# mmp/pbrt-v1

Hardware: AMD Instinct MI355X
Metric: Mrays/s (primary+secondary: every Scene::Intersect + Scene::IntersectP) (higher is better)
Workload: dtype f32

## Files before the change

### include/pbrt_hip.h

```cpp
#ifndef PBRT_HIP_H
#define PBRT_HIP_H
#include <stdint.h>
#include <stddef.h>
#ifdef __cplusplus
extern "C" {
#endif

#define RT_OK 0
#define RT_EINVAL (-1)
#define RT_EDEVICE (-2)
#define RT_ESTATE (-3)
#define RT_ENOMEM (-4)

typedef struct RtScene RtScene;

enum { RT_MAT_MATTE = 0, RT_MAT_MIRROR = 1, RT_MAT_GLASS = 2, RT_MAT_PLASTIC = 3, RT_MAT_UBER = 4, RT_MAT_SHINYMETAL = 5, RT_MAT_TRANSLUCENT = 6 };
typedef struct RtMaterial {
    int32_t type;
    float kd[3];
    float kt[3];
    float sigma;
    float ior;
    float ks[3];
    float roughness;
// ... 130 lines not shown
typedef struct RtAccelInfo {
    uint32_t n_nodes, n_leaf_refs, max_depth, n_tris;
    float bounds[6];
    double build_seconds;
    int32_t kind;
    int32_t grid_nvoxels[3];
    float grid_width[3], grid_inv_width[3];
} RtAccelInfo;

const char *rt_last_error(void);
int rt_device_count(int *count);

int rt_scene_create(const RtSceneDesc *desc, int device, RtScene **out);
typedef struct RtPrebuiltAccel {
    int32_t kind;
    uint32_t n_nodes, n_leaf_refs, max_depth;
    const uint32_t *nodes;
    const uint32_t *leaf_refs;
    float bounds[6];
    int32_t grid_nvoxels[3]; float grid_width[3], grid_inv_width[3];
} RtPrebuiltAccel;
int rt_scene_create_prebuilt(const RtSceneDesc *desc, int device, const RtPrebuiltAccel *accel, RtScene **out);
int rt_scene_set_density(RtScene *s, const RtDensityRegion *region);
int rt_scene_set_light_transforms(RtScene *s, const float *light_to_world, uint32_t n_lights);
struct RtTexture; struct RtMaterialTextures;
int rt_scene_set_textures(RtScene *s, const struct RtTexture *nodes, uint32_t n_nodes, const struct RtMaterialTextures *mats, uint32_t n_mats);
int rt_scene_destroy(RtScene *s);
int rt_scene_set_stream(RtScene *s, void *hip_stream);
int rt_scene_accel_info(const RtScene *s, RtAccelInfo *info);
int rt_scene_accel_copy(const RtScene *s, uint32_t *nodes, uint32_t *leaf_refs);

typedef struct RtKdTree RtAccel;
int rt_accel_build(const float *tri_verts, uint32_t n_tris, const RtAccelParams *params, RtAccel **out);
int rt_accel_info(const RtAccel *t, RtAccelInfo *info);
int rt_accel_copy(const RtAccel *t, uint32_t *nodes, uint32_t *leaf_refs);
typedef struct RtLeafLayoutInfo { uint64_t n_nodes, n_slots, n_entries; uint32_t stride, pad; } RtLeafLayoutInfo;
int rt_accel_leaf_layout(const RtAccel *t, int runs, int copies, uint32_t *tnodes, uint32_t *slot_prim, uint32_t *entries, RtLeafLayoutInfo *info);
int rt_accel_destroy(RtAccel *t);
typedef struct RtKdTree RtKdTree;
int rt_kdtree_build(const float *tri_verts, uint32_t n_tris, const RtAccelParams *params, RtKdTree **out);
int rt_kdtree_info(const RtKdTree *t, RtAccelInfo *info);
int rt_kdtree_copy(const RtKdTree *t, uint32_t *nodes, uint32_t *leaf_refs);
int rt_kdtree_destroy(RtKdTree *t);

int rt_camera_rays(RtScene *s, const RtRenderDesc *rd, uint64_t first, uint32_t count, RtRay *rays_out);
int rt_trace_closest(RtScene *s, const RtRay *rays, uint32_t n, RtHit *hits_out);
int rt_trace_any(RtScene *s, const RtRay *rays, uint32_t n, uint8_t *occluded_out);

int rt_trace_closest_device(RtScene *s, const RtRay *dev_rays, uint32_t n, RtHit *dev_hits);
int rt_trace_any_device(RtScene *s, const RtRay *dev_rays, uint32_t n, uint8_t *dev_occluded);
typedef struct RtHitGeometry {
    float   *p;
    float   *ng;
    float   *ns;
    float   *uv;
    int32_t *material;
    int32_t *light;
} RtHitGeometry;
int rt_hit_geometry_device(RtScene *s, const RtRay *dev_rays, const RtHit *dev_hits, uint32_t n, const RtHitGeometry *out);
int rt_camera_rays_device(RtScene *s, const RtRenderDesc *rd, uint64_t first, uint32_t count, RtRay *dev_rays);
int rt_scene_get_stream(RtScene *s, void **hip_stream_out);

int rt_film_bind(RtScene *s, void *device_accum, int32_t x_pixel_count, int32_t y_pixel_count);
int rt_film_clear(RtScene *s);
int rt_film_read(RtScene *s, float *host_accum);
int rt_film_resolve(RtScene *s, int premultiply_alpha, float *rgb_out, float *alpha_out);

int rt_render(RtScene *s, const RtRenderDesc *rd);
int rt_sync(RtScene *s);
int rt_samples_read(RtScene *s, uint64_t first, uint64_t count, float *out);
int rt_counters(RtScene *s, RtCounters *out);
int rt_counters_reset(RtScene *s);
int rt_set_counting(RtScene *s, int enabled);
int rt_last_render_ms(RtScene *s, float *total_ms, float *kernel_ms);
typedef struct RtRenderStats {
    float total_ms, render_ms, trace_ms, gather_ms;
    int32_t pipeline, iterations, timed_iterations;
    uint32_t slots;
    float shade_ms;
    int32_t bands;
    float march_ms;
    uint64_t weighted_points;
    float weighted_ms[5];
} RtRenderStats;
int rt_film_resolve_device(RtScene *s, const float *dev_accum, uint64_t n, int premultiply, float *dev_rgb, float *dev_alpha);
int rt_film_resolve_device_rgba(RtScene *s, const float *dev_accum, uint64_t n, int premultiply, float *dev_rgba);
int rt_film_pack_parts(RtScene *s, const float *dev_accum, int32_t w, int32_t h, int32_t world, int32_t rows, float *dev_parts);
int rt_last_render_stats(RtScene *s, RtRenderStats *out);

#ifdef __cplusplus
}
#endif
#endif
```

### pbrt-v1_amd/__init__.py

```python
from __future__ import annotations

import ctypes as C
import os
import subprocess
import numpy as np

_HERE = os.path.dirname(os.path.abspath(__file__))
LIB_DIR = os.path.join(_HERE, "lib")
HIP_LIB = os.path.join(LIB_DIR, "libpbrt_hip.so")
if os.environ.get("PBRT_HIP_TUNE") and os.environ.get("PBRT_HIP_LIB_PATH"):
    HIP_LIB = os.environ["PBRT_HIP_LIB_PATH"]
HOST_LIB = os.path.join(LIB_DIR, "libpbrt_host.so")
CSRC = os.path.join(_HERE, "csrc")

HIPCC_FLAGS = ["--offload-arch=gfx950", "-O3", "-std=c++17", "-ffp-contract=off", "-fno-slp-vectorize", "-fPIC", "-shared",
               "-Wno-unused-value"]
HOST_FLAGS = ["-O2", "-std=c++17", "-fPIC", "-shared", "-msse2", "-mfpmath=sse", "-fvisibility=hidden", "-fvisibility-inlines-hidden"]


HIP_UNITS = ("rt_kernels.hip", "rt_scene.hip", "rt_film.hip", "rt_trace.hip", "rt_mega_w.hip", "rt_mega_d.hip", "rt_mega_dw.hip", "rt_mega_p.hip", "rt_mega_b.hip", "rt_mega_g.hip", "rt_pipe_w.hip", "rt_pipe_d.hip",
             "rt_pipe_p.hip", "rt_pipe_v.hip", "rt_march.hip", "rt_rays.hip", "kd_build.cpp", "grid_build.cpp", "leaf_layout.cpp")


def _include_closure(path, seen=None):
    import re
    seen = set() if seen is None else seen
    if path in seen or not os.path.exists(path):
        return seen
    seen.add(path)
    for inc in re.findall(r'^\s*#\s*include\s+"([^"]+)"', open(path).read(), re.M):
        _include_closure(os.path.normpath(os.path.join(os.path.dirname(path), inc)), seen)
    return seen


def _compile_unit(cmd, verbose=False):
    if verbose:
        print(" ".join(cmd))
    if not cmd[-3].endswith(".hip"):
        subprocess.check_call(cmd)
        return
    r = subprocess.run(cmd + ["-Rpass-analysis=kernel-resource-usage"], capture_output=True, text=True)
    keep = [ln for ln in r.stderr.splitlines() if "remark:" in ln and any(k in ln for k in ("Function Name", " VGPRs:", "VGPRs Spill", "Occupancy", "ScratchSize", "LDS Size"))]
    open(cmd[-1][:-2] + ".resources.txt", "w").write("\n".join(keep) + "\n")
    if r.returncode != 0:
        raise RuntimeError("hipcc failed:\n" + r.stderr[-4000:])


def build(force: bool = False, verbose: bool = False, defines=(), jobs: int | None = None) -> None:
    from concurrent.futures import ThreadPoolExecutor
    os.makedirs(LIB_DIR, exist_ok=True)
    obj_dir = os.path.join(LIB_DIR, "obj")
    os.makedirs(obj_dir, exist_ok=True)
    hip_dir = os.path.join(CSRC, "hip")
    hip_dep = [os.path.join(hip_dir, f) for f in os.listdir(hip_dir)] + [os.path.join(_HERE, "..", "include", "pbrt_hip.h")]
    headers = [d for d in hip_dep if d.endswith((".h", ".inc"))]
    host_src = [os.path.join(CSRC, "host", "scene_api.cpp")]
    host_dep = [os.path.join(CSRC, "host", f) for f in os.listdir(os.path.join(CSRC, "host"))] + \
               [os.path.join(_HERE, "..", "include", f) for f in ("pbrt_hip.h", "pbrt_hip_desc.h", "pbrt_hip_plugin.h", "pbrt_hip_material.h", "pbrt_hip_texture.h")]

    def stale(out, deps):
        return force or not os.path.exists(out) or any(os.path.getmtime(d) > os.path.getmtime(out) for d in deps)

    stamp = os.path.join(obj_dir, "defines.txt")
    dtext = " ".join(HIPCC_FLAGS) + " | " + " ".join(HOST_FLAGS) + " | " + " ".join(defines)
    if (open(stamp).read() if os.path.exists(stamp) else "") != dtext:
        force = True
    todo = []
    for u in HIP_UNITS:
        obj = os.path.join(obj_dir, u.rsplit(".", 1)[0] + ".o")
        if stale(obj, sorted(_include_closure(os.path.join(hip_dir, u)))):
            todo.append(["hipcc"] + [f for f in HIPCC_FLAGS if f != "-shared"] + list(defines) + ["-c", os.path.join(hip_dir, u), "-o", obj])
    if todo:
        run = lambda cmd: _compile_unit(cmd, verbose)
        with ThreadPoolExecutor(max_workers=jobs or min(len(todo), os.cpu_count() or 4)) as ex:
            list(ex.map(run, todo))
        open(stamp, "w").write(dtext)
    objs = [os.path.join(obj_dir, u.rsplit(".", 1)[0] + ".o") for u in HIP_UNITS]
    if stale(HIP_LIB, objs):
        cmd = ["hipcc", "--offload-arch=gfx950", "-shared", "-fPIC"] + objs + ["-o", HIP_LIB]
        if verbose:
            print(" ".join(cmd))
        subprocess.check_call(cmd)
    if stale(HOST_LIB, host_dep):
        cmd = ["g++"] + HOST_FLAGS + host_src + ["-Wl,--version-script=" + os.path.join(CSRC, "host", "exports.map"), "-ldl", "-o", HOST_LIB]
        if verbose:
            print(" ".join(cmd))
        subprocess.check_call(cmd)


def build_variant(name: str, defines=(), units=None, arch: str | None = None, verbose: bool = False) -> str:
    from concurrent.futures import ThreadPoolExecutor
    units = list(HIP_UNITS if units is None else units)
    if len(units) < len(HIP_UNITS):
        build()
    obj_dir = os.path.join(LIB_DIR, "obj_" + name)
    os.makedirs(obj_dir, exist_ok=True)
    hip_dir = os.path.join(CSRC, "hip")
    flags = [f for f in HIPCC_FLAGS if f != "-shared"]
    if arch:
        flags = ["--offload-arch=" + arch if f.startswith("--offload-arch=") else f for f in flags]
    out = os.path.join(LIB_DIR, "libpbrt_hip_%s.so" % name)
    stamp = os.path.join(obj_dir, "defines.txt")
    dtext = " ".join(flags) + " | " + " ".join(defines) + " | " + " ".join(units)
    lib_ok = os.path.exists(out) and (open(stamp).read() if os.path.exists(stamp) else "") == dtext
    obj_of = lambda d, u: os.path.join(d, u.rsplit(".", 1)[0] + ".o")

    def stale(u):
        obj = obj_of(obj_dir, u)
        if not lib_ok:
            return True
        t = os.path.getmtime(obj if os.path.exists(obj) else out)
        return any(os.path.getmtime(d) > t for d in _include_closure(os.path.join(hip_dir, u)))
    todo = [u for u in units if stale(u)]
    borrowed = [obj_of(os.path.join(LIB_DIR, "obj"), u) for u in HIP_UNITS if u not in units]
    if not todo and lib_ok and not any(os.path.getmtime(o) > os.path.getmtime(out) for o in borrowed):
        return out
    todo += [u for u in units if u not in todo and not os.path.exists(obj_of(obj_dir, u))]
    cmds = [["hipcc"] + flags + list(defines) + ["-c", os.path.join(hip_dir, u), "-o", obj_of(obj_dir, u)] for u in todo]
    if cmds:
        with ThreadPoolExecutor(max_workers=min(len(cmds), os.cpu_count() or 4)) as ex:
            list(ex.map(lambda cmd: _compile_unit(cmd, verbose), cmds))
    objs = [obj_of(obj_dir if u in units else os.path.join(LIB_DIR, "obj"), u) for u in HIP_UNITS]
    subprocess.check_call(["hipcc", "--offload-arch=" + (arch or "gfx950"), "-shared", "-fPIC"] + objs + ["-o", out])
    open(stamp, "w").write(dtext)
    return out


class RtCounters(C.Structure):
    _fields_ = [(n, C.c_uint64) for n in ("camera_rays", "closest_rays", "any_rays", "nodes_visited", "leaf_refs",
                                          "tri_tests", "bad_samples", "stack_overflows")]

    def as_dict(self):
        return {n: int(getattr(self, n)) for n, _ in self._fields_}


class RtAccelInfo(C.Structure):
    _fields_ = [("n_nodes", C.c_uint32), ("n_leaf_refs", C.c_uint32), ("max_depth", C.c_uint32), ("n_tris", C.c_uint32),
                ("bounds", C.c_float * 6), ("build_seconds", C.c_double), ("kind", C.c_int32),
                ("grid_nvoxels", C.c_int32 * 3), ("grid_width", C.c_float * 3), ("grid_inv_width", C.c_float * 3)]


class RtLeafLayoutInfo(C.Structure):
    _fields_ = [("n_nodes", C.c_uint64), ("n_slots", C.c_uint64), ("n_entries", C.c_uint64), ("stride", C.c_uint32), ("pad", C.c_uint32)]


class RtPrebuiltAccel(C.Structure):
    _fields_ = [("kind", C.c_int32), ("n_nodes", C.c_uint32), ("n_leaf_refs", C.c_uint32), ("max_depth", C.c_uint32),
                ("nodes", C.c_void_p), ("leaf_refs", C.c_void_p), ("bounds", C.c_float * 6),
                ("grid_nvoxels", C.c_int32 * 3), ("grid_width", C.c_float * 3), ("grid_inv_width", C.c_float * 3)]


class RtRenderStats(C.Structure):
    _fields_ = [("total_ms", C.c_float), ("render_ms", C.c_float), ("trace_ms", C.c_float), ("gather_ms", C.c_float),
                ("pipeline", C.c_int32), ("iterations", C.c_int32), ("timed_iterations", C.c_int32), ("slots", C.c_uint32), ("shade_ms", C.c_float), ("bands", C.c_int32), ("march_ms", C.c_float),
                ("weighted_points", C.c_uint64), ("weighted_ms", C.c_float * 5)]

    def as_dict(self):
        return {n: (list(getattr(self, n)) if n == "weighted_ms" else getattr(self, n)) for n, _ in self._fields_}


class RtVolume(C.Structure):
    _fields_ = [("present", C.c_int32), ("world_to_volume", C.c_float * 16), ("p0", C.c_float * 3), ("p1", C.c_float * 3),
                ("sigma_a", C.c_float * 3), ("sigma_s", C.c_float * 3), ("le", C.c_float * 3), ("g", C.c_float)]


class RtDensityRegion(C.Structure):
    _fields_ = [("kind", C.c_int32), ("a", C.c_float), ("b", C.c_float), ("updir", C.c_float * 3),
                ("nx", C.c_int32), ("ny", C.c_int32), ("nz", C.c_int32), ("density", C.POINTER(C.c_float))]


RT_MATERIAL_NAMES = ("matte", "mirror", "glass", "plastic", "uber", "shinymetal", "translucent")


class RtMaterial(C.Structure):
    _fields_ = [("type", C.c_int32), ("kd", C.c_float * 3), ("kt", C.c_float * 3), ("sigma", C.c_float), ("ior", C.c_float),
                ("ks", C.c_float * 3), ("roughness", C.c_float), ("kr", C.c_float * 3)]


class RtMaterialLobes(C.Structure):
    _fields_ = [(n, C.c_float * 3) for n in ("eta_ks", "eta_kr", "r_kd", "t_kd", "r_ks", "t_ks")] + \
               [(n, C.c_int32) for n in ("has_dr", "has_dt", "has_gr", "has_gt")]


class RtMaterialParams(C.Structure):
    _fields_ = [("type", C.c_int32), ("c", (C.c_float * 3) * 4), ("f", C.c_float)]


class RtMaterialTextures(C.Structure):
    _fields_ = [("raw", RtMaterialParams), ("tex", C.c_int32 * 5)]


class RtMaterialResolved(C.Structure):
    _fields_ = [("type", C.c_int32), ("r", C.c_float * 3), ("t", C.c_float * 3), ("on_a", C.c_float), ("on_b", C.c_float), ("ior", C.c_float),
                ("has_r", C.c_int32), ("has_t", C.c_int32), ("ks", C.c_float * 3), ("exponent", C.c_float), ("kr", C.c_float * 3),
                ("has_g", C.c_int32), ("has_kr", C.c_int32)]


class RtTexture(C.Structure):
    _fields_ = [("kind", C.c_int32), ("is_color", C.c_int32), ("mapping", C.c_int32), ("child", C.c_int32 * 3), ("value", C.c_float * 12),
                ("map", C.c_float * 8), ("world_to_texture", C.c_float * 16)]


RT_TEXTURE_NAMES = ("constant", "scale", "mix", "bilerp", "uv", "checkerboard")
RT_TEXMAP_NAMES = ("uv", "spherical", "cylindrical", "planar")
RT_MATERIAL_SLOTS = {"matte": ("Kd", None, None, None, "sigma"), "mirror": ("Kr", None, None, None, None), "glass": ("Kr", "Kt", None, None, "index"),
                     "plastic": ("Kd", "Ks", None, None, "roughness"), "uber": ("Kd", "Ks", "Kr", "opacity", "roughness"),
                     "shinymetal": (None, "Ks", "Kr", None, "roughness"), "translucent": ("Kd", "Ks", "reflect", "transmit", "roughness")}

RT_DENSITY_NAMES = {1: "exponential", 2: "volumegrid"}

RT_LIGHT_NAMES = ("point", "area", "spot", "distant", "infinite")

RT_INTEGRATOR_DEBUG = 0x100
RT_DEBUG_NAMES = ("u", "v", "nx", "ny", "nz", "snx", "sny", "snz", "one", "zero", "hit")
(RT_DEBUG_U, RT_DEBUG_V, RT_DEBUG_NX, RT_DEBUG_NY, RT_DEBUG_NZ, RT_DEBUG_SNX, RT_DEBUG_SNY, RT_DEBUG_SNZ,
 RT_DEBUG_ONE, RT_DEBUG_ZERO, RT_DEBUG_HIT) = range(11)


class RtLight(C.Structure):
    _fields_ = [("type", C.c_int32), ("color", C.c_float * 3), ("pos", C.c_float * 3), ("n_samples", C.c_int32), ("first_tri", C.c_uint32),
                ("n_tris", C.c_uint32), ("reverse_orientation", C.c_int32), ("flip_normal", C.c_int32), ("dir", C.c_float * 3),
                ("world_to_light", C.c_float * 9), ("cos_total_width", C.c_float), ("cos_falloff_start", C.c_float), ("quadric_plus1", C.c_int32)]

class RtRenderDesc(C.Structure):
    _fields_ = [(n, C.c_int32) for n in ("integrator", "max_depth", "strategy", "volume_integrator")] + [("step_size", C.c_float)] + \
               [(n, C.c_int32) for n in ("sampler", "x_samples", "y_samples", "jitter", "pixel_samples")] + [("seed", C.c_uint32)] + \
               [(n, C.c_int32) for n in ("x_res", "y_res", "x_pixel_start", "y_pixel_start", "x_pixel_count", "y_pixel_count", "x_start", "x_end", "y_start", "y_end")] + \
               [("filter_x_width", C.c_float), ("filter_y_width", C.c_float), ("filter_table", C.c_float * 256)] + \
               [(n, C.c_int32) for n in ("shard_index", "shard_count", "tile_pixels")]


class RtHitGeometry(C.Structure):
    _fields_ = [(n, C.c_void_p) for n in ("p", "ng", "ns", "uv", "material", "light")]


HIT_FIELDS = ("p", "ng", "ns", "uv", "material", "light")
_HIT_FIELD_SHAPE = {"p": (3, False), "ng": (3, False), "ns": (3, False), "uv": (2, False), "material": (0, True), "light": (0, True)}

# ... 796 lines not shown
```

### pbrt-v1_amd/csrc/hip/rt_host.h

```cpp
#pragma once
#include "rt_flavour.h"
#include "rt_render_kernel.h"
#include "rt_pipeline.h"
#include "rt_pipe_vertex.h"
#include "rt_pipe_march.h"
#include "rt_bidir.h"
#include "rt_internal.h"
#include "rt_devbuf.h"
#include <cstdio>
#include <cstdlib>
#include <cstring>
#include <string>
#include <vector>
#include <cmath>
#include <chrono>
#include <atomic>
#include <thread>
#include <type_traits>

namespace rt {
const char *knob(const char *name);
int fail(int code, const std::string &msg);
const char *last_error();
void hip_warn(hipError_t e, const char *what);
}
using namespace rt;
#define HIPCHK(expr)                                                                                   \
    do {                                                                                               \
        hipError_t e_ = (expr);                                                                        \
        if (e_ != hipSuccess)                                                                          \
            return rt::fail(RT_EDEVICE, std::string(#expr) + ": " + hipGetErrorString(e_));            \
    } while (0)
#define HIPWARN(expr) rt::hip_warn((expr), #expr)

namespace rt {
extern const flavour::Table<RenderKernelFn, flavour::Mega> g_render_kernels_whitted, g_render_kernels_direct, g_render_kernels_path;
extern const flavour::Table<RenderKernelFn, flavour::Weighted> g_render_kernels_weighted;
extern const flavour::Table<RenderKernelFn, flavour::Bidir> g_render_kernels_bidir;
extern const flavour::Table<RenderKernelFn, flavour::Debug> g_render_kernels_debug;
extern const flavour::Table<PipeShadeFn, flavour::Shade> g_pipe_shade_whitted, g_pipe_shade_direct, g_pipe_shade_path;
extern const flavour::Table<PipeShadeFn, flavour::Vertex> g_pipe_vertex;
extern const flavour::Table<PipeTraceFn, flavour::Trace> g_pipe_trace;
extern const flavour::Table<PipeMarchFn, flavour::March> g_pipe_march;
}
static const flavour::Table<RenderKernelFn, flavour::Mega> *const g_render_kernels[RT_INTEGRATOR_PATH + 1] = {&g_render_kernels_whitted, &g_render_kernels_direct, &g_render_kernels_path};
static const flavour::Table<PipeShadeFn, flavour::Shade> *const g_pipe_shade[RT_INTEGRATOR_PATH + 1] = {&g_pipe_shade_whitted, &g_pipe_shade_direct, &g_pipe_shade_path};
struct ResidentGrids {
    flavour::Table<unsigned, flavour::Mega> mega[RT_INTEGRATOR_PATH + 1];
    flavour::Table<unsigned, flavour::Weighted> weighted;
    flavour::Table<unsigned, flavour::Bidir> bidir;
    flavour::Table<unsigned, flavour::Debug> debug;
    flavour::Table<unsigned, flavour::Trace> trace;
    flavour::Table<unsigned, flavour::March> march;
};

namespace rt { void host_free(void *p); void event_free(void *e); void stream_free(void *st); }
template <class T> using Pinned = rt::DevBuf<T, rt::host_free>;
using Event = rt::DevBuf<std::remove_pointer_t<hipEvent_t>, rt::event_free>;
using OwnedStream = rt::DevBuf<std::remove_pointer_t<hipStream_t>, rt::stream_free>;

struct PipePlanes {
    DevBuf<float4> state, ray_o, hit, q_o; DevBuf<unsigned> q_slot;
    template <class F> void each(F &&f) { f(state, size_t(RT_PIPE_VEC)); f(ray_o, size_t(2)); f(hit, size_t(3)); f(q_o, size_t(4)); f(q_slot, size_t(3)); }
};

struct RtScene {
    int device = 0;
    hipStream_t stream = nullptr;
    OwnedStream own_stream;
    Event ev0, ev1, ev2;
    Event wt_ev[6];
    std::vector<Event> pipe_ev;
    std::vector<Event> pipe_fence;
    KdTree tree;
    GridAccelData gridacc;
    int accel_kind = RT_ACCEL_KDTREE;
    double per_leaf = -1.0;
    bool has_ext = false;
    DevScene dev{};
    std::vector<DevBuf<char>> allocs;
    float *accum = nullptr; DevBuf<float> own_accum; int film_w = 0, film_h = 0;
    DevBuf<float> filter_dev;
    DevBuf<unsigned long long> work_counter, counters;
    DevBuf<uint2> spill;
    DevBuf<float> frames;
    unsigned grid = 0, n_threads = 0;
    ResidentGrids grids{};
    DevBuf<DimReq> light_dims;
    std::vector<DimReq> light_dims_host;
    const unsigned *light_draw_flags = nullptr; unsigned n_drawing_lights = 0;
    DevBuf<unsigned> wt_recbase;
    unsigned n_infinite = 0;
    int light_draws = 0;
    DevBuf<unsigned> wt_base; DevBuf<float> wt_rec; DevBuf<float2> wt_pick;
    DevBuf<unsigned long long> wt_sums;
    Pinned<unsigned long long> wt_total;
    unsigned long long wt_points = 0; bool last_weighted = false;
    DevBuf<DevScene> dev_scene; DevBuf<DevFrame> dev_frame;
    DevBuf<float4> samples;
    int samples_spp = 1;
    unsigned long long samples_last = 0;
    DevBuf<float> resolve_buf;
    DevBuf<float> vol_buf;
    RtVolume volume{};
    int density_kind = RT_DENSITY_NONE;
    double vol_world[6] = {0, 0, 0, 0, 0, 0};
    bool rendered = false;
    std::vector<DevMaterial> materials_host;
    std::vector<DevLight> lights_host;
    std::vector<int> tex_uv_idx_host; std::vector<float> tex_uv_host;
    bool has_textures = false;
    DevBuf<DevMaterial> mat_buf;
    int spill_depth = 0;
    bool have_timing = false;
    bool counting = true;
    uint32_t n_tris = 0;
    PipePlanes pool; DevBuf<unsigned> q_count; DevBuf<unsigned long long> wave_work; DevBuf<PipePool> dev_pool;
    Pinned<unsigned> h_qcount;
    bool last_pipeline = false, last_marches = false; int pipe_iters = 0, pipe_timed = 0; unsigned pipe_slots = 0;
    DevBuf<float4> trace_buf;
    int n_cus = 0;
    DevBuf<unsigned> trace_qc;
    DevBuf<float4> ray_planes, any_hits;
};
#define RT_PIPE_QN 4096
#define RT_PIPE_TIMED 256
#define RT_PIPE_BATCH 4

static inline int scene_alloc(RtScene *s, size_t bytes, void **p) {
    DevBuf<char> b;
    if (int rc = b.grow(bytes)) return rc;
    *p = b.p; s->allocs.push_back(std::move(b));
    return RT_OK;
}
template <class T>
static inline int upload(RtScene *s, const T *host, size_t n, const T **dev) {
    void *p = nullptr;
    if (int rc = scene_alloc(s, (n ? n : 1) * sizeof(T), &p)) return rc;
    if (n) HIPCHK(hipMemcpy(p, host, n * sizeof(T), hipMemcpyHostToDevice));
    *dev = static_cast<const T *>(p);
    return RT_OK;
}

int upload_tex_uv(RtScene *s);
int ensure_material_pool(RtScene *s, rt::DevFrame &fr, size_t levels, size_t n_slots);

template <class T>
static inline int ensure(RtScene *s, DevBuf<T> &b, size_t need) {
    if (need <= b.cap) return RT_OK;
    if (b.p) HIPCHK(hipStreamSynchronize(s->stream));
    return b.grow(need);
}

template <class F> static inline int guarded(const char *what, F &&f) {
    try { return f(); }
    catch (const std::bad_alloc &) { return rt::fail(RT_ENOMEM, std::string(what) + ": out of host memory"); }
    catch (const std::exception &e) { return rt::fail(RT_ESTATE, std::string(what) + ": " + e.what()); }
}

struct FilmGather { int which = 0, grx = 0, gry = 0, cols = 0, rows = 0, slot_ncs = 0; size_t slot_lds = 0, col_bytes = 0; };
int film_gather_plan(RtScene *s, const rt::DevFrame &fr, FilmGather &g);
int film_gather_launch(RtScene *s, const rt::DevFrame &fr, const FilmGather &g, const rt::DevFrame *dfr, int row0, int row_end);
```

### pbrt-v1_amd/csrc/hip/rt_integrate.h

```cpp
#pragma once
#include "rt_shade.h"
#include "rt_texture.h"

namespace rt {

enum Stage {
    ST_FETCH = 0, ST_VERTEX, ST_DIRECT_NEXT, ST_SHADOW_DONE, ST_MIS_DONE, ST_ED_BSDF, ST_ED_DONE,
    ST_BOUNCE, ST_SPECULAR, ST_SPEC_TRANS, ST_RETURN, ST_VOL_BEGIN, ST_VOL_STEP, ST_POP, ST_FINISH, ST_EXIT
};

struct Rng {
    uint32_t base, ctr;
    RT_DEV float next_float() { return rng_f32(base, ctr++); }
    RT_DEV uint32_t next_u32() { return rng_u32(base, ctr++); }
};

#define RT_FRAME_WORDS 25

struct Lane {
    uint32_t sample_index;
    uint32_t work;
    float image_x, image_y;
    uint32_t dim_base;
    Rng rng;
    V3 L;
    V3 thr;
    float alpha;
    int depth;
    int fsp;
    bool specular;
    Vertex v;
    int li, lj;
    int cur_light;
    V3 Ld;
    V3 Ld_light;
    V3 L_all;
    V3 pend;
    float bs1, bs2, bcs;
    uint32_t ord;
    uint32_t ctr0;
    float wt_w;
    unsigned vf;
    V3 dM, dB;
    V3 pendS, pendM, thr_old;
    int stage;
    bool has_ray;
    Trav tv;
};

RT_DEV float lhs_value(const Lane &ln, const DimReq &r, int j, int d) {
    const uint32_t fb = ln.dim_base + r.f_base, ub = ln.dim_base + r.u_base;
    if (r.n == 1) return (0 + rng_f32(ln.rng.base, fb + d)) * 1.f;
    int pos = j;
    const int n = r.n;
    for (int k = n - 1; k >= 0; --k) {
        int other = int(rng_u32(ln.rng.base, ub + d * n + k) % uint32_t(n));
        if (pos == k) pos = other; else if (pos == other) pos = k;
    }
    float delta = 1.f / n;
    return (pos + rng_f32(ln.rng.base, fb + pos * r.dims + d)) * delta;
}

RT_DEV float van_der_corput(uint32_t n, uint32_t scramble) {
    n = (n << 16) | (n >> 16);
    n = ((n & 0x00ff00ffu) << 8) | ((n & 0xff00ff00u) >> 8);
    n = ((n & 0x0f0f0f0fu) << 4) | ((n & 0xf0f0f0f0u) >> 4);
    n = ((n & 0x33333333u) << 2) | ((n & 0xccccccccu) >> 2);
    n = ((n & 0x55555555u) << 1) | ((n & 0xaaaaaaaau) >> 1);
    n ^= scramble;
    return (float)n / (float)0x100000000LL;
}
RT_DEV float sobol2(uint32_t n, uint32_t scramble) {
    for (uint32_t v = 1u << 31; n != 0; n >>= 1, v ^= v >> 1)
        if (n & 0x1) scramble ^= v;
    return (float)scramble / (float)0x100000000LL;
}
RT_DEV int shuffle_origin(uint32_t base, uint32_t off, int count, int pos) {
    for (int k = count - 1; k >= 0; --k) {
        const int other = int(rng_u32(base, off + k) % uint32_t(count));
        if (pos == k) pos = other; else if (pos == other) pos = k;
    }
    return pos;
}
RT_DEV uint32_t pixel_stream(const DevFrame &fr, const Lane &ln) {
    const uint32_t n0 = ln.sample_index - (ln.work % uint32_t(fr.spp));
    if (n0 == 0 && fr.sampler != RT_SAMPLER_LOWDISCREPANCY) return rng_base(0xFFFFFFFFu, fr.seed);
    return rng_base(n0, fr.seed);
}
RT_DEV float dim_value(const DevFrame &fr, const Lane &ln, const DimReq &r, int j, int d) {
    if (fr.sampler == RT_SAMPLER_STRATIFIED) return lhs_value(ln, r, j, d);
    if (fr.sampler == RT_SAMPLER_RANDOM) return rng_f32(ln.rng.base, ln.dim_base + r.f_base + j * r.dims + d);
    const uint32_t pb = pixel_stream(fr, ln);
    const int P = fr.spp, n = r.n, s = int(ln.work % uint32_t(P));
    const uint32_t nscr = r.dims;
    const int blk = shuffle_origin(pb, r.f_base + nscr + uint32_t(n) * P, P, s);
    const int jb = (n == 1) ? 0 : shuffle_origin(pb, r.f_base + nscr + uint32_t(blk) * n, n, j);
    const uint32_t idx = uint32_t(blk) * n + jb;
    if (r.dims == 1) return van_der_corput(idx, rng_u32(pb, r.f_base));
    return d == 0 ? van_der_corput(idx, rng_u32(pb, r.f_base)) : sobol2(idx, rng_u32(pb, r.f_base + 1));
}

#ifndef RT_SAMPLE_NT
#define RT_SAMPLE_NT 1
#endif
RT_DEV void sample_write(const DevFrame &fr, const Lane &ln, V3 Ls, float alpha, unsigned &bad) {
    const float y = lum_y(Ls);
    if (Ls.x != Ls.x || Ls.y != Ls.y || Ls.z != Ls.z) { Ls = mk3(0.f); ++bad; }
    else if (y < -1e-5) { Ls = mk3(0.f); ++bad; }
    else if (isinf(y)) { Ls = mk3(0.f); ++bad; }
    const uint32_t lp = fastdiv(ln.work, fr.div.spp);
    float4 RT_G *rec = RT_GPTR(float4, fr.samples) + sample_slot(lp, ln.work - lp * uint32_t(fr.spp), fr.spp);
#if RT_SAMPLE_NT
    typedef float nt_f4 __attribute__((ext_vector_type(4)));
    const nt_f4 r0 = {Ls.x, Ls.y, Ls.z, alpha}, r1 = {ln.image_x, ln.image_y, 0.f, 0.f};
    __builtin_nontemporal_store(r0, (nt_f4 RT_G *)rec);
    __builtin_nontemporal_store(r1, (nt_f4 RT_G *)(rec + RT_SAMPLE_XY));
#else
    rec[0] = make_float4(Ls.x, Ls.y, Ls.z, alpha);
    rec[RT_SAMPLE_XY] = make_float4(ln.image_x, ln.image_y, 0.f, 0.f);
#endif
}

RT_DEV void stratified_camera_sample(const DevFrame &fr, uint32_t pixel_index, int s, int px, int py,
                                     uint32_t pix_base, float &ix, float &iy, float &lu, float &lv, bool need_lens) {
    const int n = fr.spp;
    const int sy = int(fastdiv(unsigned(s), fr.div.xs)), sx = s - sy * fr.xs;
    const float dx = 1.f / fr.xs, dy = 1.f / fr.ys;
    float jx = 0.5f, jy = 0.5f;
    if (fr.jitter) { jx = rng_f32(pix_base, 2 * s); jy = rng_f32(pix_base, 2 * s + 1); }
    ix = (sx + jx) * dx; iy = (sy + jy) * dy;
    ix += px; iy += py;
    lu = lv = 0.5f;
    if (need_lens) {
        const uint32_t ub = fr.jitter ? 5u * n : 0u;
        int pos = s;
        for (int k = n - 1; k >= 0; --k) {
            int other = int(rng_u32(pix_base, ub + k) % uint32_t(n));
            if (pos == k) pos = other; else if (pos == other) pos = k;
        }
        const int lx = pos % fr.xs, ly = pos / fr.xs;
        float kx = 0.5f, ky = 0.5f;
        if (fr.jitter) { kx = rng_f32(pix_base, 2 * n + 2 * pos); ky = rng_f32(pix_base, 2 * n + 2 * pos + 1); }
        lu = (lx + kx) * dx; lv = (ly + ky) * dy;
    }
    (void)pixel_index;
}

RT_DEV Ray camera_ray(const RtCamera &cam, float ix, float iy, float lensU, float lensV) {
    Ray r;
    if (cam.type == RT_CAMERA_ENVIRONMENT) {
        r.o = xform_point(cam.camera_to_world, mk3(0.f, 0.f, 0.f));
        const float theta = RT_PI * iy / cam.y_res;
        const float phi = 2 * RT_PI * ix / cam.x_res;
        const V3 dir = mk3(rt_sinf(theta) * rt_cosf(phi), rt_cosf(theta), rt_sinf(theta) * rt_sinf(phi));
        r.d = xform_vector(cam.camera_to_world, dir);
        r.mint = cam.hither; r.maxt = cam.yon;
        return r;
    }
    V3 Pcamera = xform_point(cam.raster_to_camera, mk3(ix, iy, 0.f));
    r.o = Pcamera;
    r.d = cam.type == RT_CAMERA_ORTHOGRAPHIC ? mk3(0.f, 0.f, 1.f) : Pcamera;
    if (cam.lens_radius > 0.f) {
        float lu, lv; concentric_disk(lensU, lensV, lu, lv);
        lu *= cam.lens_radius; lv *= cam.lens_radius;
        float ft = (cam.focal_distance - cam.hither) / r.d.z;
        V3 Pfocus = r.o + r.d * ft;
        r.o.x += lu * (cam.focal_distance - cam.hither) / cam.focal_distance;
        r.o.y += lv * (cam.focal_distance - cam.hither) / cam.focal_distance;
        r.d = Pfocus - r.o;
    }
    r.d = normalize3(r.d);
    r.mint = 0.f;
    r.maxt = cam.type == RT_CAMERA_ORTHOGRAPHIC ? cam.yon - cam.hither : (cam.yon - cam.hither) / r.d.z;
    r.o = xform_point(cam.camera_to_world, r.o);
    r.d = xform_vector(cam.camera_to_world, r.d);
    return r;
}

RT_DEV bool work_to_sample(const DevFrame &fr, unsigned long long w, unsigned long long &pixel, int &s) {
    const unsigned long long per_tile = (unsigned long long)fr.tile_pixels * fr.spp;
    if (fr.tile_w > 0) {
        const unsigned w32 = unsigned(w), pt = unsigned(per_tile);
        const unsigned lt = fastdiv(w32, fr.div.per_tile), rem = w32 - lt * pt;
        const unsigned tile = lt * unsigned(fr.shard_count) + unsigned(fr.shard_index);
        const unsigned q = fastdiv(rem, fr.div.spp);
        s = int(rem - q * unsigned(fr.spp));
        const unsigned ty = fastdiv(tile, fr.div.tiles_x), tx = tile - ty * unsigned(fr.tiles_x);
        const unsigned qy = fastdiv(q, fr.div.tile_w), qx = q - qy * unsigned(fr.tile_w);
        const unsigned px = tx * unsigned(fr.tile_w) + qx, py = ty * unsigned(fr.tile_h) + qy;
        const unsigned ew = unsigned(fr.x_end - fr.x_start), eh = unsigned(fr.y_end - fr.y_start);
        pixel = (unsigned long long)py * ew + px;
        return px < ew && py < eh;
    }
    if (fr.total_work <= 0xffffffffull && per_tile <= 0xffffffffull) {
        const unsigned w32 = unsigned(w), pt = unsigned(per_tile);
        const unsigned lt = fastdiv(w32, fr.div.per_tile), rem = w32 - lt * pt;
        const unsigned long long tile = (unsigned long long)lt * unsigned(fr.shard_count) + unsigned(fr.shard_index);
        const unsigned q = fastdiv(rem, fr.div.spp);
        pixel = tile * unsigned(fr.tile_pixels) + q;
        s = int(rem - q * unsigned(fr.spp));
        return pixel < fr.total_pixels;
    }
    const unsigned long long lt = w / per_tile, rem = w % per_tile;
    const unsigned long long tile = lt * fr.shard_count + fr.shard_index;
    pixel = tile * fr.tile_pixels + rem / fr.spp;
    s = int(rem % fr.spp);
    return pixel < fr.total_pixels;
}

RT_DEV void tile_order_to_sample(const DevFrame &fr, unsigned w, unsigned &pixel, int &s) {
    const unsigned spp = unsigned(fr.spp), T = unsigned(fr.mega_tile);
    const unsigned W = unsigned(fr.x_end - fr.x_start), H = unsigned(fr.y_end - fr.y_start);
    const FrameDiv &dv = fr.div;
    const unsigned wp = fastdiv(w, dv.spp); s = int(w - wp * spp);
    const unsigned row_px = W * T, ty = fastdiv(wp, dv.row_px), rem = wp - ty * row_px;
    const unsigned h_t = min(T, H - ty * T), full = T * h_t, tiles_x = dv.blocks_x;
    const FastDiv &df = h_t < T ? dv.block[1] : dv.block[0];
    unsigned tx = fastdiv(rem, df); tx = tx < tiles_x ? tx : tiles_x - 1u;
    const unsigned rem2 = rem - tx * full, w_t = min(T, W - tx * T);
    const FastDiv &dw = w_t < T ? dv.block_w[1] : dv.block_w[0];
    const unsigned qy = fastdiv(rem2, dw), qx = rem2 - qy * w_t;
    pixel = (ty * T + qy) * W + tx * T + qx;
}

RT_DEV void setup_sample(const DevScene &sc, const DevFrame &fr, Lane &ln, unsigned long long pixel, int s, Ray &ray) {
    const int w = fr.x_end - fr.x_start;
    int px, py;
    if (fr.total_pixels <= 0xffffffffull) { const unsigned row = fastdiv(unsigned(pixel), fr.div.width); px = fr.x_start + int(unsigned(pixel) - row * unsigned(w)); py = fr.y_start + int(row); }
    else { px = fr.x_start + int(pixel % w); py = fr.y_start + int(pixel / w); }
    const uint32_t n0 = uint32_t(pixel * fr.spp);
    ln.sample_index = n0 + uint32_t(s);
    ln.rng.base = rng_base(ln.sample_index, fr.seed);
    float lu = 0.5f, lv = 0.5f;
    const bool need_lens = sc.cam.lens_radius > 0.f;
    if (fr.sampler == RT_SAMPLER_STRATIFIED) {
        const uint32_t pix_base = (pixel == 0) ? rng_base(0xFFFFFFFFu, fr.seed) : rng_base(n0, fr.seed);
        ln.dim_base = (s == 0 && pixel != 0) ? fr.pixgen_draws : 0u;
        stratified_camera_sample(fr, uint32_t(pixel), s, px, py, pix_base, ln.image_x, ln.image_y, lu, lv, need_lens);
    } else if (fr.sampler == RT_SAMPLER_RANDOM) {
        const uint32_t pix_base = (pixel == 0) ? rng_base(0xFFFFFFFFu, fr.seed) : rng_base(n0, fr.seed);
        ln.dim_base = (s == 0 && pixel != 0) ? fr.pixgen_draws : 0u;
        ln.image_x = rng_f32(pix_base, 2 * s); ln.image_y = rng_f32(pix_base, 2 * s + 1);
        ln.image_x += px; ln.image_y += py;
        if (need_lens) { lu = rng_f32(pix_base, 2 * fr.spp + 2 * s); lv = rng_f32(pix_base, 2 * fr.spp + 2 * s + 1); }
    } else {
        const uint32_t pix_base = rng_base(n0, fr.seed);
        const uint32_t P = uint32_t(fr.spp);
        ln.dim_base = (s == 0) ? fr.pixgen_draws : 0u;
        const int pos = shuffle_origin(pix_base, 2 + P, int(P), s);
        ln.image_x = px + van_der_corput(uint32_t(pos), rng_u32(pix_base, 0));
        ln.image_y = py + sobol2(uint32_t(pos), rng_u32(pix_base, 1));
        if (need_lens) {
            const uint32_t lb = 2 + 2 * P;
            const int lp = shuffle_origin(pix_base, lb + 2 + P, int(P), s);
            lu = van_der_corput(uint32_t(lp), rng_u32(pix_base, lb)); lv = sobol2(uint32_t(lp), rng_u32(pix_base, lb + 1));
        }
    }
    ln.rng.ctr = ln.dim_base + ((fr.sampler == RT_SAMPLER_LOWDISCREPANCY) ? 0u : fr.lhs_total);
    ray = camera_ray(sc.cam, ln.image_x, ln.image_y, lu, lv);
    ln.image_x = (ln.image_x + 1.f) - 1.f; ln.image_y = (ln.image_y + 1.f) - 1.f;
}

RT_DEV float RT_G *frame_ptr(const DevFrame &fr, int frame, unsigned gtid) {
    return RT_GPTR(float, fr.frames) + (size_t(frame) * RT_FRAME_WORDS) * fr.n_threads + gtid;
}
template <bool EXT>
RT_DEV void frame_push(const DevFrame &fr, Lane &ln, unsigned gtid, V3 f, float absdot, int after) {
    float RT_G *q = frame_ptr(fr, ln.fsp, gtid); const size_t st = fr.n_threads;
    q[0 * st] = ln.L.x; q[1 * st] = ln.L.y; q[2 * st] = ln.L.z;
    q[3 * st] = f.x; q[4 * st] = f.y; q[5 * st] = f.z; q[6 * st] = absdot;
    q[7 * st] = __int_as_float(after); q[8 * st] = __int_as_float(ln.depth);
    q[9 * st] = ln.v.p.x; q[10 * st] = ln.v.p.y; q[11 * st] = ln.v.p.z;
    q[12 * st] = ln.v.nn.x; q[13 * st] = ln.v.nn.y; q[14 * st] = ln.v.nn.z;
    q[15 * st] = ln.v.sn.x; q[16 * st] = ln.v.sn.y; q[17 * st] = ln.v.sn.z;
    q[18 * st] = ln.v.wo.x; q[19 * st] = ln.v.wo.y; q[20 * st] = ln.v.wo.z;
    q[21 * st] = __int_as_float(ln.v.mat);
    if (EXT) { q[22 * st] = ln.v.ng.x; q[23 * st] = ln.v.ng.y; q[24 * st] = ln.v.ng.z; }
    ++ln.fsp;
}
template <bool EXT>
RT_DEV int frame_pop(const DevFrame &fr, Lane &ln, unsigned gtid, V3 child) {
    --ln.fsp;
    const float RT_G *q = frame_ptr(fr, ln.fsp, gtid); const size_t st = fr.n_threads;
    V3 Lp = mk3(q[0 * st], q[1 * st], q[2 * st]);
    V3 f = mk3(q[3 * st], q[4 * st], q[5 * st]);
    float absdot = q[6 * st];
    ln.L = Lp + (child * f) * absdot;
    int after = __float_as_int(q[7 * st]);
    ln.depth = __float_as_int(q[8 * st]);
    ln.v.p = mk3(q[9 * st], q[10 * st], q[11 * st]);
    ln.v.nn = mk3(q[12 * st], q[13 * st], q[14 * st]);
    ln.v.sn = mk3(q[15 * st], q[16 * st], q[17 * st]);
    ln.v.tn = cross3(ln.v.nn, ln.v.sn);
    ln.v.wo = mk3(q[18 * st], q[19 * st], q[20 * st]);
    ln.v.mat = __float_as_int(q[21 * st]);
    if (EXT) ln.v.ng = mk3(q[22 * st], q[23 * st], q[24 * st]);
    return after;
}

RT_DEV void all_lights_done(Lane &ln) {
    ln.L = ln.L + ln.L_all;
    ln.stage = ST_SPECULAR;
}

template <bool DEFER = false>
RT_DEV void launch_ray(Lane &ln, const DevScene &sc, V3 o, V3 d, float mint, float maxt, bool any, int next_stage) {
    Ray r; r.o = o; r.d = d; r.mint = mint; r.maxt = maxt;
    if (DEFER) { ln.tv.o = o; ln.tv.d = d; ln.tv.mint = mint; ln.tv.maxt = maxt; ln.tv.any = any; ln.tv.hit_prim = -1; ln.tv.b1 = 0.f; ln.tv.b2 = 0.f; }
    else if (sc.accel_kind == RT_ACCEL_GRID) grid_begin(ln.tv, sc, r, any); else trav_begin(ln.tv, sc, r, any);
    ln.has_ray = true;
    ln.stage = next_stage;
}

RT_DEV float RT_G *vol_ray_ptr(const DevFrame &fr, int level, unsigned gtid) { return RT_GPTR(float, fr.vol_rays) + size_t(level) * 8 * fr.n_threads + gtid; }
RT_DEV void vol_store_ray(const DevFrame &fr, int level, unsigned gtid, const Ray &r) {
    float RT_G *q = vol_ray_ptr(fr, level, gtid); const size_t st = fr.n_threads;
    q[0] = r.o.x; q[st] = r.o.y; q[2 * st] = r.o.z; q[3 * st] = r.d.x; q[4 * st] = r.d.y; q[5 * st] = r.d.z; q[6 * st] = r.mint; q[7 * st] = r.maxt;
}
RT_DEV Ray vol_load_ray(const DevFrame &fr, int level, unsigned gtid) {
    const float RT_G *q = vol_ray_ptr(fr, level, gtid); const size_t st = fr.n_threads;
    Ray r; r.o = mk3(q[0], q[st], q[2 * st]); r.d = mk3(q[3 * st], q[4 * st], q[5 * st]); r.mint = q[6 * st]; r.maxt = q[7 * st];
    return r;
}
RT_DEV bool vol_intersect(const RtVolume &v, V3 o, V3 d, float mint, float maxt, float &t0, float &t1) {
    const V3 vo = xform_point(v.world_to_volume, o), vd = xform_vector(v.world_to_volume, d);
    float a = mint, b = maxt; bool ok = true;
#pragma unroll
    for (int i = 0; i < 3; ++i) {
        float invRayDir = 1.f / comp(vd, i);
        float tNear = (v.p0[i] - comp(vo, i)) * invRayDir, tFar = (v.p1[i] - comp(vo, i)) * invRayDir;
        if (tNear > tFar) { float tmp = tNear; tNear = tFar; tFar = tmp; }
        a = tNear > a ? tNear : a; b = tFar < b ? tFar : b;
        if (a > b) ok = false;
    }
    t0 = a; t1 = b; return ok;
}
RT_DEV bool vol_inside(const RtVolume &v, V3 p) {
    const V3 q = xform_point(v.world_to_volume, p);
    return q.x >= v.p0[0] && q.x <= v.p1[0] && q.y >= v.p0[1] && q.y <= v.p1[1] && q.z >= v.p0[2] && q.z <= v.p1[2];
}
RT_DEV V3 vol_transmittance(const RtVolume &v, V3 o, V3 d, float mint, float maxt) {
    float t0, t1;
// ... 194 lines not shown
            const V3 ss = dens ? D * mat_color(vol.sigma_s) : (in ? mat_color(vol.sigma_s) : mk3(0.f));
            const int nLights = int(sc.n_lights);
            if (!is_black(ss) && nLights > 0) {
                const float r0 = have_row ? m.s0 : samp[size_t(3 * i) * st], u1 = have_row ? m.s1 : samp[size_t(3 * i + 1) * st], u2 = have_row ? m.s2 : samp[size_t(3 * i + 2) * st];
                const int lightNum = min(int(floorf(r0 * nLights)), nLights - 1);
                LightRef Lt = RT_LIGHT(sc, lightNum);
                V3 wo, L, sd; float pdf, smax;
                if (light_is_delta<EXT>(Lt)) { L = delta_light_sample(Lt, p, wo, sd, smax); pdf = 1.f; }
                else if constexpr (EXT) {
                    if (light_is_infinite<EXT>(Lt)) { wo = infinite_sample_sphere(u1, u2, pdf); L = mat_color(Lt.color); sd = wo; smax = RT_INF; }
                    else {
                        V3 ns; V3 ps = area_sample_point<EXT>(sc, Lt, p, u1, u2, ln.rng, ns);
                        wo = normalize3(ps - p); pdf = area_light_pdf<EXT>(sc, Lt, p, wo); L = area_L(Lt, ns, -wo);
                        sd = ps - p; smax = 1.f - RT_RAY_EPSILON;
                    }
                } else {
                    V3 ns; V3 ps = area_sample_point<EXT>(sc, Lt, p, u1, u2, ln.rng, ns);
                    wo = normalize3(ps - p); pdf = area_light_pdf<EXT>(sc, Lt, p, wo); L = area_L(Lt, ns, -wo);
                    sd = ps - p; smax = 1.f - RT_RAY_EPSILON;
                }
                if (!is_black(L) && pdf > 0.f) {
                    const float costheta = dot3(w, -wo);
                    const float phase = in ? 1.f / (4.f * RT_PI) * (1.f - vol.g * vol.g) / rt_powf(1.f + vol.g * vol.g - 2.f * vol.g * costheta, 1.5f) : 0.f;
                    ln.pend = div_s((((Tr * ss) * phase) * L) * float(nLights), pdf);
                    m.i = i; m.t0 = t0; m.Tr = Tr; m.p = p; m.Lv = Lv;
                    if (PREFETCH) {
                        const int j = i + 1 < N ? i + 1 : i;
                        m.s0 = samp[size_t(3 * j) * st]; m.s1 = samp[size_t(3 * j + 1) * st]; m.s2 = samp[size_t(3 * j + 2) * st];
                    }
                    launch_ray<DEFER>(ln, sc, p, sd, RT_RAY_EPSILON, smax, true, ST_VOL_STEP);
                    return true;
                }
            }
        }
        ++i; t0 += step; have_row = false;
    }
    Lv = Lv * step;
    if (EXT && sc.dens_kind != RT_DENSITY_NONE) ln.L = ln.L + Lv;
    else {
        const V3 T = vol_transmittance(vol, ray.o, ray.d, ray.mint, ray.maxt);
        ln.L = T * ln.L + Lv;
    }
    ln.stage = ST_POP;
    return false;
}

RT_DEV float debug_value(int code, bool hit, float u, float v, V3 ng, V3 ns) {
    switch (code) {
        case RT_DEBUG_U: return u;
        case RT_DEBUG_V: return v;
        case RT_DEBUG_NX: return fabsf(ng.x);
        case RT_DEBUG_NY: return fabsf(ng.y);
        case RT_DEBUG_NZ: return fabsf(ng.z);
        case RT_DEBUG_SNX: return fabsf(ns.x);
        case RT_DEBUG_SNY: return fabsf(ns.y);
        case RT_DEBUG_SNZ: return fabsf(ns.z);
        case RT_DEBUG_ONE: return 1.f;
        case RT_DEBUG_HIT: return hit ? 1.f : 0.f;
        default: return 0.f;
    }
}
template <bool COUNT, bool VOL>
RT_DEV void debug_vertex(const DevScene &sc, const DevFrame &fr, Lane &ln, unsigned gtid, unsigned *c_closest) {
    if (COUNT) ++*c_closest;
    const bool hit = ln.tv.hit_prim >= 0;
    const int cr = fr.strategy & 0xff, cg = (fr.strategy >> 8) & 0xff, cb = (fr.strategy >> 16) & 0xff;
    const bool want_uv = cr <= RT_DEBUG_V || cg <= RT_DEBUG_V || cb <= RT_DEBUG_V;
    const bool want_n = (cr >= RT_DEBUG_NX && cr <= RT_DEBUG_SNZ) || (cg >= RT_DEBUG_NX && cg <= RT_DEBUG_SNZ) || (cb >= RT_DEBUG_NX && cb <= RT_DEBUG_SNZ);
    float u = 0.f, v = 0.f; V3 ng = mk3(0.f), ns = mk3(0.f);
    if (hit) {
        if (want_uv) {
            RtTexHit h;
            hit_point_uv(sc, ln.tv, __float_as_uint(RT_GPTR(const float4, sc.tri_shade)[size_t(2) * unsigned(ln.tv.hit_prim)].w), h);
            u = h.u; v = h.v;
        }
        if (want_n) { make_vertex<true>(sc, ln.tv, ln.v); ng = ln.v.ng; ns = ln.v.nn; }
        if (VOL) vol_ray_ptr(fr, 0, gtid)[7 * size_t(fr.n_threads)] = ln.tv.maxt;
    }
    ln.L = mk3(debug_value(cr, hit, u, v, ng, ns), debug_value(cg, hit, u, v, ng, ns), debug_value(cb, hit, u, v, ng, ns));
    ln.alpha = 1.f;
    ln.stage = ST_RETURN;
}

template <bool COUNT, int INTEG_, bool VOL, bool EXT, int STAGE, bool DEFER = false, bool PARK = false>
RT_DEV void stage_body(const DevScene &sc, const DevFrame &fr, Lane &ln, unsigned gtid,
                       unsigned *c_closest, unsigned *c_any, unsigned *c_bad) {
    constexpr bool WEIGHTED = INTEG_ == RT_INTEG_DIRECT_WEIGHTED;
    constexpr int INTEG = WEIGHTED ? int(RT_INTEGRATOR_DIRECT) : INTEG_;
    if constexpr (STAGE == ST_VERTEX && INTEG_ == RT_INTEGRATOR_DEBUG) {
        debug_vertex<COUNT, VOL>(sc, fr, ln, gtid, c_closest);
        return;
    } else if constexpr (STAGE == ST_VERTEX) {
        if (COUNT) ++*c_closest;
        const bool hit = ln.tv.hit_prim >= 0;
        if (INTEG == RT_INTEGRATOR_PATH) {
            if (!hit) {
                if (EXT && ln.depth == 0) ln.L = infinite_le_sum(sc, ln.L, mk3(1.f), false);
                if (ln.depth == 0) ln.alpha = (ln.L.x != 0.f || ln.L.y != 0.f || ln.L.z != 0.f) ? 1.f : 0.f;
                else if (EXT && ln.specular) ln.L = infinite_le_sum(sc, ln.L, ln.thr, true);
                ln.stage = ST_RETURN; return;
            }
            int resolved = -1;
            if constexpr (EXT) resolved = resolve_hit_material(sc, fr, ln.tv, 0, gtid);
            make_vertex<EXT>(sc, ln.tv, ln.v);
            if (EXT && resolved >= 0) ln.v.mat = resolved;
#ifdef RT_DEBUG_PIXEL
            if (int(floorf(ln.image_x)) == fr.dbg_x && int(floorf(ln.image_y)) == fr.dbg_y)
                printf("DEV depth %d prim %d t %.9g o %.9g %.9g %.9g d %.9g %.9g %.9g p %.9g %.9g %.9g nn %.9g %.9g %.9g sn %.9g %.9g %.9g\n", ln.depth, ln.tv.hit_prim, ln.tv.maxt,
                       ln.tv.o.x, ln.tv.o.y, ln.tv.o.z, ln.tv.d.x, ln.tv.d.y, ln.tv.d.z, ln.v.p.x, ln.v.p.y, ln.v.p.z, ln.v.nn.x, ln.v.nn.y, ln.v.nn.z, ln.v.sn.x, ln.v.sn.y, ln.v.sn.z);
#endif
            if (ln.depth == 0) { ln.alpha = 1.f; if (VOL) vol_ray_ptr(fr, 0, gtid)[7 * size_t(fr.n_threads)] = ln.tv.maxt; }
            else if (VOL) ln.thr = ln.thr * scene_transmittance<VOL, EXT>(sc, fr, ln, ln.tv.o, ln.tv.d, ln.tv.mint, ln.tv.maxt);
            if ((ln.depth == 0 || ln.specular) && ln.v.light >= 0)
                ln.L = ln.L + ln.thr * area_L(RT_LIGHT(sc, ln.v.light), vertex_ng<EXT>(ln.v), ln.v.wo);
        } else {
            if (!hit) {
                ln.L = mk3(0.f);
                if (ln.depth == 0) ln.alpha = 0.f;
                if (EXT) {
                    ln.L = infinite_le_sum(sc, ln.L, mk3(1.f), false);
                    if (ln.depth == 0 && !is_black(ln.L)) ln.alpha = 1.f;
                }
                ln.stage = ST_RETURN; return;
            }
            int resolved = -1;
            if constexpr (EXT) resolved = resolve_hit_material(sc, fr, ln.tv, ln.fsp, gtid);
            make_vertex<EXT>(sc, ln.tv, ln.v);
            if (EXT && resolved >= 0) ln.v.mat = resolved;
            if (ln.depth == 0) ln.alpha = 1.f;
            if (VOL) vol_ray_ptr(fr, ln.fsp, gtid)[7 * size_t(fr.n_threads)] = ln.tv.maxt;
            ln.L = mk3(0.f);
            if (ln.v.light >= 0) ln.L = ln.L + area_L(RT_LIGHT(sc, ln.v.light), vertex_ng<EXT>(ln.v), ln.v.wo);
        }
        ln.li = 0; ln.lj = 0; ln.L_all = mk3(0.f); ln.Ld_light = mk3(0.f);
        ln.stage = ST_DIRECT_NEXT;
        return;
    }
    if constexpr (STAGE == ST_DIRECT_NEXT) {
        const int nLights = int(sc.n_lights);
        if constexpr (WEIGHTED) {
            if (nLights == 0) { ln.stage = ST_SPECULAR; return; }
            if (fr.weighted_phase == 1) { ++ln.ord; ln.stage = ST_SPECULAR; return; }
            if (fr.weighted_phase == 3 && ln.li > 0) { ln.stage = ST_SPECULAR; return; }
            if (fr.weighted_phase == 2 && fr.wt_mixed) {
                if (ln.li == 0 && ln.lj == 0) { ln.ctr0 = ln.rng.ctr; ln.wt_w = __uint_as_float(1u); }
                if (ln.li >= nLights) { ++ln.ord; ln.rng.ctr = ln.ctr0; ln.lj = 0; ln.stage = ST_SPECULAR; return; }
                ln.rng.ctr = ln.ctr0 + uint32_t(ln.lj);
            } else if (fr.weighted_phase == 2) {
                if (ln.li == 0) ln.ctr0 = ln.rng.ctr;
                if (ln.li >= nLights) { ++ln.ord; ln.stage = ST_SPECULAR; return; }
                ln.rng.ctr = ln.ctr0;
            }
            const float ls1 = dim_value(fr, ln, fr.two_d[0], 0, 0), ls2 = dim_value(fr, ln, fr.two_d[0], 0, 1);
            ln.bs1 = dim_value(fr, ln, fr.two_d[1], 0, 0); ln.bs2 = dim_value(fr, ln, fr.two_d[1], 0, 1);
            ln.bcs = dim_value(fr, ln, fr.one_d[1], 0, 0);
            if (fr.weighted_phase == 2) {
                if (ln.li == 0 && ln.lj == 0) RT_GPTR(float, fr.wt_rec)[weighted_record(fr, ln, nLights)] = dim_value(fr, ln, fr.one_d[0], 0, 0);
                estimate_direct_begin<EXT, DEFER>(sc, ln, ln.li, ls1, ls2);
            } else {
                const float2 pick = RT_GPTR(const float2, fr.wt_pick)[ln.ord++];
                ln.li = 1; ln.wt_w = pick.y;
                estimate_direct_begin<EXT, DEFER>(sc, ln, __float_as_int(pick.x), ls1, ls2);
            }
            return;
        }
        if (INTEG == RT_INTEGRATOR_PATH || (INTEG == RT_INTEGRATOR_DIRECT && fr.strategy == RT_STRATEGY_ONE)) {
            if (nLights == 0 || ln.li > 0) { ln.stage = (INTEG == RT_INTEGRATOR_PATH) ? ST_BOUNCE : ST_SPECULAR; return; }
            ln.li = 1;
            const int k = (INTEG == RT_INTEGRATOR_PATH) ? ln.depth : 0;
            const bool from_sampler = (INTEG == RT_INTEGRATOR_DIRECT) || k < 3;
            float un, ls1, ls2;
            if (from_sampler) {
                const int i1 = (INTEG == RT_INTEGRATOR_PATH) ? 3 * k : 0;
                const int i2 = (INTEG == RT_INTEGRATOR_PATH) ? 3 * k : 0;
                un = dim_value(fr, ln, fr.one_d[i1], 0, 0);
                ls1 = dim_value(fr, ln, fr.two_d[i2], 0, 0); ls2 = dim_value(fr, ln, fr.two_d[i2], 0, 1);
                ln.bs1 = dim_value(fr, ln, fr.two_d[i2 + 1], 0, 0); ln.bs2 = dim_value(fr, ln, fr.two_d[i2 + 1], 0, 1);
                ln.bcs = dim_value(fr, ln, fr.one_d[i1 + 1], 0, 0);
            } else {
                un = ln.rng.next_float();
                ls1 = ln.rng.next_float(); ls2 = ln.rng.next_float();
                ln.bs1 = ln.rng.next_float(); ln.bs2 = ln.rng.next_float(); ln.bcs = ln.rng.next_float();
            }
            int lightNum = min(int(floorf(un * nLights)), nLights - 1);
            estimate_direct_begin<EXT, DEFER>(sc, ln, lightNum, ls1, ls2);
            return;
        }
        if (INTEG == RT_INTEGRATOR_DIRECT) {
            if (ln.li >= nLights) { all_lights_done(ln); return; }
            const DimReq RT_G *ld = RT_GPTR(const DimReq, fr.light_dims) + 3 * ln.li;
            const DimReq rl = ld[0], rb = ld[1], rc = ld[2];
            if (ln.lj == 0) ln.Ld_light = mk3(0.f);
            const float ls1 = dim_value(fr, ln, rl, ln.lj, 0), ls2 = dim_value(fr, ln, rl, ln.lj, 1);
            ln.bs1 = dim_value(fr, ln, rb, ln.lj, 0); ln.bs2 = dim_value(fr, ln, rb, ln.lj, 1);
            ln.bcs = dim_value(fr, ln, rc, ln.lj, 0);
            estimate_direct_begin<EXT, DEFER>(sc, ln, ln.li, ls1, ls2);
            return;
        }
        if (ln.li >= nLights) { ln.stage = ST_SPECULAR; return; }
        {
            LightRef Lt = RT_LIGHT(sc, ln.li);
            MatRef m = RT_MAT(sc, ln.v.mat);
            const int cur = ln.li++;
            V3 wi, Li, sd; float smax;
            if (light_is_delta<EXT>(Lt)) Li = delta_light_sample(Lt, ln.v.p, wi, sd, smax);
            else if constexpr (EXT) {
                if (light_is_infinite<EXT>(Lt)) {
                    float u2 = ln.rng.next_float();
                    float u1 = ln.rng.next_float();
                    float pdf; wi = infinite_sample_sphere(u1, u2, pdf);
                    Li = (pdf == 0.f) ? mk3(0.f) : div_s(mat_color(Lt.color), pdf);
                    sd = wi; smax = RT_INF;
                } else {
                    float u2 = ln.rng.next_float();
                    float u1 = ln.rng.next_float();
                    V3 ns; V3 ps = area_sample_point<EXT>(sc, Lt, ln.v.p, u1, u2, ln.rng, ns);
                    wi = normalize3(ps - ln.v.p);
                    float pdf = area_light_pdf<EXT>(sc, Lt, ln.v.p, wi);
                    Li = (pdf == 0.f) ? mk3(0.f) : div_s(area_L(Lt, ns, -wi), pdf);
                    sd = ps - ln.v.p; smax = 1.f - RT_RAY_EPSILON;
                }
            } else {
                float u2 = ln.rng.next_float();
                float u1 = ln.rng.next_float();
                V3 ns; V3 ps = area_sample_point<EXT>(sc, Lt, ln.v.p, u1, u2, ln.rng, ns);
                wi = normalize3(ps - ln.v.p);
                float pdf = area_light_pdf<EXT>(sc, Lt, ln.v.p, wi);
                Li = (pdf == 0.f) ? mk3(0.f) : div_s(area_L(Lt, ns, -wi), pdf);
                sd = ps - ln.v.p; smax = 1.f - RT_RAY_EPSILON;
            }
            (void)cur;
            if (is_black(Li)) return;
            V3 f = bsdf_f<EXT>(m, ln.v, ln.v.wo, wi);
            if (is_black(f)) return;
            ln.pend = (f * Li) * absdot3(wi, ln.v.nn);
            launch_ray<DEFER>(ln, sc, ln.v.p, sd, RT_RAY_EPSILON, smax, true, ST_SHADOW_DONE);
        }
        return;
    }
    if constexpr (STAGE == ST_SHADOW_DONE) {
        if (COUNT) ++*c_any;
        const bool occluded = ln.tv.hit_prim >= 0;
        if (INTEG == RT_INTEGRATOR_WHITTED) {
            if (!occluded) ln.L = ln.L + ln.pend * scene_transmittance<VOL, EXT>(sc, fr, ln, ln.tv.o, ln.tv.d, ln.tv.mint, ln.tv.maxt);
            ln.stage = ST_DIRECT_NEXT;
            return;
        }
        if (!occluded) ln.Ld = ln.Ld + ln.pend * scene_transmittance<VOL, EXT>(sc, fr, ln, ln.tv.o, ln.tv.d, ln.tv.mint, ln.tv.maxt);
        ln.stage = ST_ED_BSDF;
        return;
    }
    if constexpr (STAGE == ST_ED_BSDF) {
        estimate_direct_bsdf<EXT, DEFER>(sc, ln);
        return;
    }
    if constexpr (STAGE == ST_MIS_DONE) {
        if (COUNT) ++*c_closest;
        if (ln.tv.hit_prim >= 0) {
            V3 nh; int light;
            prim_normal_light<EXT>(sc, ln.tv, nh, light);
            if (light == ln.cur_light) {
                if (dot3(nh, -ln.tv.d) > 0)
                    ln.Ld = ln.Ld + ln.pend * scene_transmittance<VOL, EXT>(sc, fr, ln, ln.tv.o, ln.tv.d, ln.tv.mint, ln.tv.maxt);
            }
        } else if (EXT) {
            LightRef Lt = RT_LIGHT(sc, ln.cur_light);
            if (Lt.type == RT_LIGHT_INFINITE && !is_black(mat_color(Lt.color)))
                ln.Ld = ln.Ld + ln.pend * scene_transmittance<VOL, EXT>(sc, fr, ln, ln.tv.o, ln.tv.d, ln.tv.mint, ln.tv.maxt);
        }
        ln.stage = ST_ED_DONE;
        return;
    }
    if constexpr (STAGE == ST_ED_DONE) {
        const int nLights = int(sc.n_lights);
        if constexpr (WEIGHTED) {
            if (fr.weighted_phase == 2) {
                const unsigned at = fr.wt_mixed ? __float_as_uint(ln.wt_w) : 1u + 2u * unsigned(ln.li);
                float RT_G *rec = RT_GPTR(float, fr.wt_rec) + weighted_record(fr, ln, nLights) + at;
                rec[0] = lum_y(ln.Ld);
                rec[1] = lum_y(ln.Ld * float(nLights));
                if (fr.wt_mixed) {
                    ln.wt_w = __uint_as_float(at + 2u);
                    const unsigned j = ln.ord - RT_GPTR(const unsigned, fr.wt_base)[ln.work];
                    if (light_draws_rng(RT_LIGHT(sc, ln.li)) && unsigned(ln.lj) < j) ++ln.lj; else { ln.lj = 0; ++ln.li; }
                } else ++ln.li;
                ln.stage = ST_DIRECT_NEXT;
            } else {
                if (ln.wt_w == 0.f) ln.L = ln.L + ln.Ld * float(nLights);
                else ln.L = ln.L + div_s(ln.Ld, ln.wt_w);
                ln.stage = ST_SPECULAR;
            }
            return;
        }
        if (INTEG == RT_INTEGRATOR_PATH) {
            ln.L = ln.L + ln.thr * (ln.Ld * float(nLights));
            ln.stage = ST_BOUNCE;
        } else if (fr.strategy == RT_STRATEGY_ONE) {
            ln.L = ln.L + ln.Ld * float(nLights);
            ln.stage = ST_SPECULAR;
        } else {
            ln.Ld_light = ln.Ld_light + ln.Ld;
            const int ns = RT_GPTR(const DimReq, fr.light_dims)[3 * ln.li].n;
            if (++ln.lj >= ns) {
                ln.L_all = ln.L_all + ln.Ld_light * (1.f / float(ns));
                ln.lj = 0; ++ln.li;
            }
            ln.stage = ST_DIRECT_NEXT;
            if (ln.li >= nLights) all_lights_done(ln);
        }
        return;
    }
    if constexpr (STAGE == ST_BOUNCE) {
        MatRef m = RT_MAT(sc, ln.v.mat);
        const int k = ln.depth;
        float bs1, bs2, bcs;
        if (k < 3) {
            bs1 = dim_value(fr, ln, fr.two_d[3 * k + 2], 0, 0); bs2 = dim_value(fr, ln, fr.two_d[3 * k + 2], 0, 1);
            bcs = dim_value(fr, ln, fr.one_d[3 * k + 2], 0, 0);
        } else { bs1 = ln.rng.next_float(); bs2 = ln.rng.next_float(); bcs = ln.rng.next_float(); }
        V3 wi; float pdf; int flags;
        V3 f = bsdf_sample_f<EXT>(m, ln.v, ln.v.wo, wi, bs1, bs2, bcs, pdf, BX_ALL, flags);
        if (is_black(f) || pdf == 0.f) { ln.stage = ST_RETURN; return; }
        ln.specular = (flags & BX_SPECULAR) != 0;
        ln.thr = ln.thr * div_s(f * absdot3(wi, ln.v.nn), pdf);
        if (k > 3) {
            if (ln.rng.next_float() > .5f) { ln.stage = ST_RETURN; return; }
            ln.thr = div_s(ln.thr, .5f);
        }
        if (k == fr.max_depth) { ln.stage = ST_RETURN; return; }
        ++ln.depth;
        launch_ray<DEFER>(ln, sc, ln.v.p, wi, RT_RAY_EPSILON, RT_INF, false, ST_VERTEX);
        return;
    }
    if constexpr (STAGE == ST_SPECULAR) {
        if (!(ln.depth < fr.max_depth)) { ln.stage = ST_RETURN; return; }
        MatRef m = RT_MAT(sc, ln.v.mat);
        float u3 = ln.rng.next_float(), u2 = ln.rng.next_float(), u1 = ln.rng.next_float();
        V3 wi; float pdf; int flags;
        V3 f = bsdf_sample_f<EXT>(m, ln.v, ln.v.wo, wi, u1, u2, u3, pdf, BX_REFLECTION | BX_SPECULAR, flags);
        if (!is_black(f) && pdf > 0.f) f = div_s(f, pdf);
        const float ad = absdot3(wi, ln.v.nn);
        if (!is_black(f) && ad > 0.f) {
            frame_push<EXT>(fr, ln, gtid, f, ad, ST_SPEC_TRANS);
            ++ln.depth;
            launch_ray<DEFER>(ln, sc, ln.v.p, wi, RT_RAY_EPSILON, RT_INF, false, ST_VERTEX);
            if (VOL) { Ray cr; cr.o = ln.v.p; cr.d = wi; cr.mint = RT_RAY_EPSILON; cr.maxt = RT_INF; vol_store_ray(fr, ln.fsp, gtid, cr); }
            return;
        }
        ln.stage = ST_SPEC_TRANS;
        return;
    }
    if constexpr (STAGE == ST_SPEC_TRANS) {
        MatRef m = RT_MAT(sc, ln.v.mat);
        float u3 = ln.rng.next_float(), u2 = ln.rng.next_float(), u1 = ln.rng.next_float();
        V3 wi; float pdf; int flags;
        V3 f = bsdf_sample_f<EXT>(m, ln.v, ln.v.wo, wi, u1, u2, u3, pdf, BX_TRANSMISSION | BX_SPECULAR, flags);
        if (!is_black(f) && pdf > 0.f) f = div_s(f, pdf);
        const float ad = absdot3(wi, ln.v.nn);
        if (!is_black(f) && ad > 0.f) {
            frame_push<EXT>(fr, ln, gtid, f, ad, ST_RETURN);
            ++ln.depth;
            launch_ray<DEFER>(ln, sc, ln.v.p, wi, RT_RAY_EPSILON, RT_INF, false, ST_VERTEX);
            if (VOL) { Ray cr; cr.o = ln.v.p; cr.d = wi; cr.mint = RT_RAY_EPSILON; cr.maxt = RT_INF; vol_store_ray(fr, ln.fsp, gtid, cr); }
            return;
        }
        ln.stage = ST_RETURN;
        return;
    }
    if constexpr (STAGE == ST_RETURN) {
        ln.stage = VOL ? ST_VOL_BEGIN : ST_POP;
        return;
    }
    if constexpr (VOL && (STAGE == ST_VOL_BEGIN || STAGE == ST_VOL_STEP)) {
        const Ray ray = vol_load_ray(fr, ln.fsp, gtid);
        const size_t st = fr.n_threads;
        float RT_G *vs = RT_GPTR(float, fr.vol_state) + gtid;
        float RT_G *samp = RT_GPTR(float, fr.vol_samp) + gtid;
        March m;
        bool park;
        if (STAGE == ST_VOL_BEGIN) {
            march_begin<EXT>(sc, fr, ln, ray, m, samp, st);
            if (PARK) { ln.stage = ST_VOL_STEP; park = true; }
            else park = march_steps<COUNT, EXT, DEFER>(sc, fr, ln, ray, m, samp, st, false, c_any);
        } else {
            m.i = __float_as_int(vs[0]); m.N = __float_as_int(vs[st]); m.t0 = vs[2 * st]; m.step = vs[3 * st];
            m.Tr = mk3(vs[4 * st], vs[5 * st], vs[6 * st]); m.p = mk3(vs[7 * st], vs[8 * st], vs[9 * st]); m.Lv = mk3(vs[10 * st], vs[11 * st], vs[12 * st]);
            park = march_steps<COUNT, EXT, DEFER>(sc, fr, ln, ray, m, samp, st, true, c_any);
        }
        if (park) {
            vs[0] = __int_as_float(m.i); vs[st] = __int_as_float(m.N); vs[2 * st] = m.t0; vs[3 * st] = m.step;
            vs[4 * st] = m.Tr.x; vs[5 * st] = m.Tr.y; vs[6 * st] = m.Tr.z; vs[7 * st] = m.p.x; vs[8 * st] = m.p.y; vs[9 * st] = m.p.z;
            vs[10 * st] = m.Lv.x; vs[11 * st] = m.Lv.y; vs[12 * st] = m.Lv.z;
        }
        return;
    }
    if constexpr (STAGE == ST_POP) {
        if (ln.fsp == 0) { ln.stage = ST_FINISH; return; }
        ln.stage = frame_pop<EXT>(fr, ln, gtid, ln.L);
        return;
    }
    if constexpr (STAGE == ST_FINISH) {
        if (WEIGHTED && fr.weighted_phase == 1) RT_GPTR(unsigned, fr.wt_base)[ln.work] = ln.ord;
        if (!WEIGHTED || fr.weighted_phase == 3) sample_write(fr, ln, ln.L, ln.alpha, *c_bad);
        ln.stage = ST_FETCH;
        return;
    }
    (void)gtid; (void)c_closest; (void)c_any; (void)c_bad;
}

enum { BV_S = 1u, BV_M = 2u, BV_B = 4u, BV_ED = 8u,
       BV_QM = 16u, BV_QB = 32u,
       BV_CUR_S = 64u, BV_CUR_M = 128u, BV_CUR_B = 256u,
       BV_S_CLEAR = 512u, BV_M_LIT = 1024u };
template <bool COUNT, bool EXT>
RT_DEV void byv_ray_result(const DevScene &sc, Lane &ln, unsigned *c_closest, unsigned *c_any) {
    if (ln.vf & BV_CUR_S) {
        if (COUNT) ++*c_any;
        if (ln.tv.hit_prim < 0) ln.vf |= BV_S_CLEAR;
    } else if (ln.vf & BV_CUR_M) {
        if (COUNT) ++*c_closest;
        if (ln.tv.hit_prim >= 0) {
            V3 nh; int light;
            prim_normal_light<EXT>(sc, ln.tv, nh, light);
            if (light == ln.cur_light && dot3(nh, -ln.tv.d) > 0) ln.vf |= BV_M_LIT;
        }
    }
    ln.vf &= ~(BV_CUR_S | BV_CUR_M | BV_CUR_B);
}
template <bool COUNT, int ACCEL, bool EXT>
RT_DEV void byv_ray_advance(const DevScene &sc, Lane &ln, unsigned *c_closest, unsigned *c_any) {
    byv_ray_result<COUNT, EXT>(sc, ln, c_closest, c_any);
    Ray r; r.o = ln.tv.o; r.mint = RT_RAY_EPSILON; r.maxt = RT_INF;
    if (ln.vf & BV_QM) { r.d = ln.dM; ln.vf = (ln.vf & ~BV_QM) | BV_CUR_M; }
    else { r.d = ln.dB; ln.vf = (ln.vf & ~BV_QB) | BV_CUR_B; }
    if (ACCEL == RT_ACCEL_GRID) grid_begin(ln.tv, sc, r, false); else trav_begin(ln.tv, sc, r, false);
}
template <bool COUNT, int ACCEL, bool EXT>
RT_DEV void advance_pass_byv(const DevScene &sc, const DevFrame &fr, Lane &ln, unsigned gtid, unsigned *c_closest, unsigned *c_any, unsigned *c_bad) {
    constexpr int INTEG = RT_INTEGRATOR_PATH;
#define RT_BV_BODY(S) stage_body<COUNT, INTEG, false, EXT, S, true>(sc, fr, ln, gtid, c_closest, c_any, c_bad)
    const int nLights = int(sc.n_lights);
    if (!ln.has_ray && (ln.stage == ST_VERTEX || ln.stage == ST_ED_DONE)) {
        byv_ray_result<COUNT, EXT>(sc, ln, c_closest, c_any);
        if (ln.vf & BV_ED) {
            V3 Ld = mk3(0.f);
            if (ln.vf & BV_S_CLEAR) Ld = Ld + ln.pendS * mk3(1.f);
            if (ln.vf & BV_M_LIT) Ld = Ld + ln.pendM * mk3(1.f);
            ln.L = ln.L + ln.thr_old * (Ld * float(nLights));
        }
        ln.vf = 0u;
        if (ln.stage == ST_ED_DONE) ln.stage = ST_RETURN;
    }
    unsigned flags = 0;
    V3 o = mk3(0.f), dS = mk3(0.f); float maxtS = 0.f;
    if (!ln.has_ray && ln.stage == ST_VERTEX) RT_BV_BODY(ST_VERTEX);
    if (!ln.has_ray && ln.stage == ST_DIRECT_NEXT) {
        RT_BV_BODY(ST_DIRECT_NEXT);
        if (ln.has_ray) { ln.has_ray = false; ln.stage = ST_ED_BSDF; flags |= BV_S; ln.pendS = ln.pend; o = ln.tv.o; dS = ln.tv.d; maxtS = ln.tv.maxt; }
        if (ln.stage == ST_ED_BSDF) {
            RT_BV_BODY(ST_ED_BSDF);
            if (ln.has_ray) { ln.has_ray = false; flags |= BV_M | BV_QM; ln.pendM = ln.pend; o = ln.tv.o; ln.dM = ln.tv.d; }
            if (flags & (BV_S | BV_M)) { flags |= BV_ED; ln.thr_old = ln.thr; }
            else { ln.stage = ST_ED_DONE; RT_BV_BODY(ST_ED_DONE); }
            ln.stage = ST_BOUNCE;
        }
    }
    if (!ln.has_ray && ln.stage == ST_BOUNCE) {
        RT_BV_BODY(ST_BOUNCE);
        if (ln.has_ray) { ln.has_ray = false; flags |= BV_B | BV_QB; o = ln.tv.o; ln.dB = ln.tv.d; }
    }
    if (!ln.has_ray && ln.stage == ST_RETURN && !(flags & BV_ED)) { RT_BV_BODY(ST_RETURN); RT_BV_BODY(ST_POP); RT_BV_BODY(ST_FINISH); }
    if (flags & (BV_S | BV_M | BV_B)) {
        Ray r; r.o = o; r.mint = RT_RAY_EPSILON;
        bool any = false;
        if (flags & BV_S) { r.d = dS; r.maxt = maxtS; any = true; flags |= BV_CUR_S; }
        else if (flags & BV_M) { r.d = ln.dM; r.maxt = RT_INF; flags = (flags & ~BV_QM) | BV_CUR_M; }
        else { r.d = ln.dB; r.maxt = RT_INF; flags = (flags & ~BV_QB) | BV_CUR_B; }
        if (ACCEL == RT_ACCEL_GRID) grid_begin(ln.tv, sc, r, any); else trav_begin(ln.tv, sc, r, any);
        ln.vf = flags;
        ln.has_ray = true;
        ln.stage = (flags & BV_B) ? ST_VERTEX : ST_ED_DONE;
    }
#undef RT_BV_BODY
}


RT_DEV bool stage_in_phase(int stage, int phase) {
    if (stage == ST_EXIT) return false;
    if (phase < 0) return true;
    const bool first = stage == ST_VERTEX || stage == ST_DIRECT_NEXT;
    return phase == 0 ? first : !first;
}
template <bool COUNT, int INTEG_, bool VOL, bool EXT, bool DEFER = false, bool PARK = false>
RT_DEV void advance_pass(const DevScene &sc, const DevFrame &fr, Lane &ln, unsigned gtid,
                         unsigned *c_closest, unsigned *c_any, unsigned *c_bad, int phase) {
    constexpr int INTEG = INTEG_ == RT_INTEG_DIRECT_WEIGHTED ? int(RT_INTEGRATOR_DIRECT) : INTEG_;
#ifdef RT_PROFILE_STAGES
#define RT_RUN(S) { const unsigned long long m_ = __ballot(!ln.has_ray && ln.stage == S); if (m_) { const unsigned long long t_ = __builtin_readcyclecounter(); \
        if (!ln.has_ray && ln.stage == S) stage_body<COUNT, INTEG_, VOL, EXT, S, DEFER, PARK>(sc, fr, ln, gtid, c_closest, c_any, c_bad); \
        if (__lane_id() == 0) { atomicAdd(fr.counters + 24 + 2 * S, __builtin_readcyclecounter() - t_); atomicAdd(fr.counters + 24 + 2 * S + 1, (unsigned long long)__popcll(m_) | (1ull << 40)); } } }
#else
#define RT_RUN(S) if (!ln.has_ray && ln.stage == S) stage_body<COUNT, INTEG_, VOL, EXT, S, DEFER, PARK>(sc, fr, ln, gtid, c_closest, c_any, c_bad)
#endif
    if constexpr (INTEG_ == RT_INTEGRATOR_DEBUG) {
        RT_RUN(ST_VERTEX);
        RT_RUN(ST_RETURN);
        if (VOL) { RT_RUN(ST_VOL_STEP); RT_RUN(ST_VOL_BEGIN); }
        RT_RUN(ST_POP);
        RT_RUN(ST_FINISH);
    } else {
    if (phase != 0) {
        RT_RUN(ST_MIS_DONE);
        RT_RUN(ST_SHADOW_DONE);
    }
    if (phase != 1) {
        RT_RUN(ST_VERTEX);
        RT_RUN(ST_DIRECT_NEXT);
    }
    if (phase != 0) {
        if (INTEG != RT_INTEGRATOR_WHITTED) { RT_RUN(ST_ED_BSDF); RT_RUN(ST_ED_DONE); }
        if (INTEG == RT_INTEGRATOR_PATH) { RT_RUN(ST_BOUNCE); }
        else { RT_RUN(ST_SPECULAR); RT_RUN(ST_SPEC_TRANS); }
        RT_RUN(ST_RETURN);
        if (VOL) { if (!PARK) RT_RUN(ST_VOL_STEP); RT_RUN(ST_VOL_BEGIN); }
        RT_RUN(ST_POP);
        RT_RUN(ST_FINISH);
    }
    }
#undef RT_RUN
}

}
```

### pbrt-v1_amd/csrc/hip/rt_kernels.hip

```cpp
#include "rt_host.h"
#include "rt_weighted.h"

namespace rt {
__global__ void camera_kernel(DevScene sc, DevFrame fr, unsigned long long first, unsigned count, RtRay *out) {
    const unsigned i = blockIdx.x * blockDim.x + threadIdx.x;
    if (i >= count) return;
    const unsigned long long n = first + i;
    Lane ln; Ray r;
    setup_sample(sc, fr, ln, n / fr.spp, int(n % fr.spp), r);
    out[i].o[0] = r.o.x; out[i].o[1] = r.o.y; out[i].o[2] = r.o.z;
    out[i].d[0] = r.d.x; out[i].d[1] = r.d.y; out[i].d[2] = r.d.z;
    out[i].mint = r.mint; out[i].maxt = r.maxt;
}

}

namespace rt {
const char *knob(const char *name) {
#ifdef RT_NO_TUNABLES
    (void)name; return nullptr;
#else
    static const bool on = std::getenv("PBRT_HIP_TUNE") != nullptr;
    return on ? std::getenv(name) : nullptr;
#endif
// ... 78 lines not shown
        s->pipe_ev.resize(6 * RT_PIPE_TIMED); s->pipe_fence.resize(RT_PIPE_QN / RT_PIPE_BATCH);
        for (auto &e : s->pipe_ev) HIPCHK(hipEventCreate(&e.p));
        for (auto &e : s->pipe_fence) HIPCHK(hipEventCreateWithFlags(&e.p, hipEventDisableTiming));
    }
    const flavour::Request rq = request_of(s, rd, &fr);
    const PipeShadeFn shade = by_vertex ? g_pipe_vertex[flavour::Vertex::index(rq)] : (*g_pipe_shade[integ])[flavour::Shade::index(rq)];
    const int tk = flavour::Trace::index(rq);
    const PipeTraceFn trace = g_pipe_trace[tk];
    const unsigned trace_grid = s->grids.trace[tk];
    const bool marches = s->volume.present;
    const int mk = flavour::March::index(rq);
    const unsigned march_grid = s->grids.march[mk];
    HIPCHK(hipMemcpyAsync(s->dev_frame, &fr, sizeof(DevFrame), hipMemcpyHostToDevice, s->stream));
    HIPCHK(hipMemcpyAsync(s->dev_pool, &pl, sizeof(PipePool), hipMemcpyHostToDevice, s->stream));
    HIPCHK(hipMemsetAsync(s->work_counter, 0, sizeof(unsigned long long), s->stream));
    HIPCHK(hipMemsetAsync(pl.state + n_slots, 0, size_t(n_slots) * sizeof(float4), s->stream));
    HIPCHK(hipMemsetAsync(pl.wave_work, 0, size_t(n_slots / 64 + 1) * 2 * sizeof(unsigned long long), s->stream));
    HIPCHK(hipEventRecord(s->ev0, s->stream));
    int iter = 0, checked = 0, batch = 0;
    bool done = false;
    const int max_iters = 1 << 20;
    while (!done) {
        for (int k = 0; k < RT_PIPE_BATCH; ++k, ++iter) {
            const unsigned qi = unsigned(iter % RT_PIPE_QN);
            PipeLaunch pk{}; pk.qi = qi; pk.slot_base = 0; pk.q_base = 0;
            HIPCHK(hipMemsetAsync(pl.q_count + size_t(RT_QC_STRIDE) * qi, 0, RT_QC_STRIDE * sizeof(unsigned), s->stream));
            if (iter < RT_PIPE_TIMED) HIPCHK(hipEventRecord(s->pipe_ev[6 * iter + 2], s->stream));
            hipLaunchKernelGGL(shade, dim3(n_slots / RT_BLOCK), dim3(RT_BLOCK), 0, s->stream, (const DevScene *)s->dev_scene,
                               (const DevFrame *)s->dev_frame, (const PipePool *)s->dev_pool, pk);
            if (iter < RT_PIPE_TIMED) HIPCHK(hipEventRecord(s->pipe_ev[6 * iter + 3], s->stream));
            TraceJob job{};
            job.q_o = pl.q_o; job.q_d = pl.q_d; job.q_slot = pl.q_slot; job.q_count = pl.q_count + size_t(RT_QC_STRIDE) * qi; job.hit = pl.hit;
            job.n_slots = n_slots; job.q_base = pk.q_base; job.spill = s->spill; job.n_threads = s->n_threads; job.counters = s->counters;
            if (by_vertex) { job.by_slot = 1; job.q_o = pl.ray_o; job.q_d = pl.ray_d; }
            if (iter < RT_PIPE_TIMED) HIPCHK(hipEventRecord(s->pipe_ev[6 * iter], s->stream));
            hipLaunchKernelGGL(trace, dim3(trace_grid), dim3(RT_BLOCK), 0, s->stream, (const DevScene *)s->dev_scene, job);
            if (iter < RT_PIPE_TIMED) HIPCHK(hipEventRecord(s->pipe_ev[6 * iter + 1], s->stream));
            if (marches) {
                MarchJob mj{};
                mj.q_march = pl.q_march; mj.q_count = pl.q_count + size_t(RT_QC_STRIDE) * qi;
                mj.spill = s->spill; mj.n_threads = s->n_threads; mj.counters = s->counters;
                if (iter < RT_PIPE_TIMED) HIPCHK(hipEventRecord(s->pipe_ev[6 * iter + 4], s->stream));
                hipLaunchKernelGGL(g_pipe_march[mk], dim3(march_grid), dim3(RT_BLOCK), 0, s->stream, (const DevScene *)s->dev_scene, (const DevFrame *)s->dev_frame,
                                   (const PipePool *)s->dev_pool, mj);
                if (iter < RT_PIPE_TIMED) HIPCHK(hipEventRecord(s->pipe_ev[6 * iter + 5], s->stream));
            }
            HIPCHK(hipMemcpyAsync(s->h_qcount + size_t(RT_QC_STRIDE) * qi, pl.q_count + size_t(RT_QC_STRIDE) * qi, (RT_QC_MARCH + 1) * sizeof(unsigned), hipMemcpyDeviceToHost, s->stream));
        }
        HIPCHK(hipGetLastError());
        HIPCHK(hipEventRecord(s->pipe_fence[batch % (RT_PIPE_QN / RT_PIPE_BATCH)], s->stream));
        if (batch >= 1) {
            HIPCHK(hipEventSynchronize(s->pipe_fence[(batch - 1) % (RT_PIPE_QN / RT_PIPE_BATCH)]));
            for (int k = 0; k < RT_PIPE_BATCH; ++k, ++checked) {
                const unsigned *q = s->h_qcount + size_t(RT_QC_STRIDE) * (checked % RT_PIPE_QN);
                if (q[0] + q[RT_QC_ANY] + q[RT_QC_MARCH] == 0) { done = true; break; }
            }
        }
        ++batch;
        if (iter > max_iters) return fail(RT_ESTATE, "rt_render: the queue pipeline did not terminate");
    }
    s->last_marches = marches;
    s->pipe_slots = n_slots; s->pipe_iters = checked + 1; s->pipe_timed = std::min(s->pipe_iters, RT_PIPE_TIMED);
    HIPCHK(hipEventRecord(s->ev1, s->stream));
    return RT_OK;
}

static int render_bidir(RtScene *s, const RtRenderDesc *rd, DevFrame &fr) {
    int rc = bind_scratch(s, rd, fr, s->n_threads); if (rc) return rc;
    const int k = flavour::Bidir::index(request_of(s, rd, &fr));
    const unsigned grid = s->grids.bidir[k];
    if (grid == 0) return fail(RT_ESTATE, "render kernel variant has no resident grid");
    HIPCHK(hipMemcpyAsync(s->dev_frame, &fr, sizeof(DevFrame), hipMemcpyHostToDevice, s->stream));
    HIPCHK(hipMemsetAsync(s->work_counter, 0, 64 * sizeof(unsigned long long), s->stream));
    HIPCHK(hipEventRecord(s->ev0, s->stream));
    hipLaunchKernelGGL(g_render_kernels_bidir[k], dim3(grid), dim3(RT_BLOCK), 0, s->stream, (const DevScene *)s->dev_scene, (const DevFrame *)s->dev_frame);
    HIPCHK(hipGetLastError());
    HIPCHK(hipEventRecord(s->ev1, s->stream));
    return RT_OK;
}

static int render_mega(RtScene *s, const RtRenderDesc *rd, DevFrame &fr) {
    int rc = bind_scratch(s, rd, fr, s->n_threads); if (rc) return rc;
    const bool debug = rd->integrator == RT_INTEGRATOR_DEBUG;
    const int k = debug ? flavour::Debug::index(request_of(s, rd, &fr)) : flavour::Mega::index(request_of(s, rd, &fr));
    const unsigned grid = debug ? s->grids.debug[k] : s->grids.mega[rd->integrator][k];
    const RenderKernelFn kernel = debug ? g_render_kernels_debug[k] : (*g_render_kernels[rd->integrator])[k];
    if (grid == 0) return fail(RT_ESTATE, "render kernel variant has no resident grid");
#ifdef RT_TAIL_PROBE
    static unsigned long long *probe = nullptr;
    const size_t n_waves = size_t(grid) * (RT_BLOCK / 64);
    if (!probe) HIPCHK(hipMalloc((void **)&probe, size_t(s->n_threads / 64 + 64) * 4 * sizeof(unsigned long long)));
    HIPCHK(hipMemsetAsync(probe, 0, n_waves * 4 * sizeof(unsigned long long), s->stream));
    fr.probe = probe;
#endif
    HIPCHK(hipMemcpyAsync(s->dev_frame, &fr, sizeof(DevFrame), hipMemcpyHostToDevice, s->stream));
    HIPCHK(hipMemsetAsync(s->work_counter, 0, 64 * sizeof(unsigned long long), s->stream));
    HIPCHK(hipEventRecord(s->ev0, s->stream));
    hipLaunchKernelGGL(kernel, dim3(grid), dim3(RT_BLOCK), 0, s->stream, (const DevScene *)s->dev_scene, (const DevFrame *)s->dev_frame);
    HIPCHK(hipGetLastError());
    HIPCHK(hipEventRecord(s->ev1, s->stream));
#ifdef RT_TAIL_PROBE
    {
        std::vector<unsigned long long> h(n_waves * 4);
        HIPCHK(hipStreamSynchronize(s->stream));
        HIPCHK(hipMemcpy(h.data(), probe, h.size() * sizeof(unsigned long long), hipMemcpyDeviceToHost));
        unsigned long long t0 = ~0ull, t0max = 0, e0 = ~0ull, e1 = 0, x1 = 0, smin = ~0ull, smax = 0, stot = 0;
        std::vector<double> ends, drain;
        for (size_t w = 0; w < n_waves; ++w) {
            const unsigned long long *r = &h[4 * w];
            if (!r[2]) continue;
            t0 = std::min(t0, r[0]); t0max = std::max(t0max, r[0]); x1 = std::max(x1, r[2]);
            if (r[1]) { e0 = std::min(e0, r[1]); e1 = std::max(e1, r[1]); drain.push_back(double(r[2] - r[1]) * 1e-2); }
            smin = std::min(smin, r[3]); smax = std::max(smax, r[3]); stot += r[3];
            ends.push_back(double(r[2]));
        }
        std::sort(ends.begin(), ends.end()); std::sort(drain.begin(), drain.end());
        auto q = [&](const std::vector<double> &v, double f) { return v.empty() ? 0.0 : v[size_t(f * (v.size() - 1))]; };
        std::fprintf(stderr, "RT_TAIL_PROBE waves=%zu span=%.1f us | starts spread %.1f us | list first seen empty at %.1f us, last at %.1f us | wave ends (us after start): p1 %.1f p10 %.1f p50 %.1f p90 %.1f p99 %.1f max %.1f | "
                             "drain per wave (end - empty, us): p10 %.1f p50 %.1f p90 %.1f p99 %.1f max %.1f | samples per wave min %llu mean %.1f max %llu\n",
                     ends.size(), double(x1 - t0) * 1e-2, double(t0max - t0) * 1e-2, double(e0 - t0) * 1e-2, double(e1 - t0) * 1e-2,
                     (q(ends, .01) - double(t0)) * 1e-2, (q(ends, .1) - double(t0)) * 1e-2, (q(ends, .5) - double(t0)) * 1e-2, (q(ends, .9) - double(t0)) * 1e-2, (q(ends, .99) - double(t0)) * 1e-2, (q(ends, 1.) - double(t0)) * 1e-2,
                     q(drain, .1), q(drain, .5), q(drain, .9), q(drain, .99), q(drain, 1.), smin, double(stot) / double(std::max<size_t>(ends.size(), 1)), smax);
    }
#endif
    return RT_OK;
}

static int render_weighted(RtScene *s, const RtRenderDesc *rd, DevFrame &fr) {
    int rc = bind_scratch(s, rd, fr, s->n_threads); if (rc) return rc;
    const int k = flavour::Weighted::index(request_of(s, rd, &fr));
    const unsigned grid = s->grids.weighted[k];
    if (grid == 0) return fail(RT_ESTATE, "render kernel variant has no resident grid");
    const int nL = int(s->dev.n_lights), R = 1 + 2 * nL;
    if (!s->wt_total) HIPCHK(hipHostMalloc((void **)&s->wt_total.p, sizeof(unsigned long long), hipHostMallocDefault));
    if ((rc = s->wt_sums.grow(RT_WSCAN_BLOCKS))) return rc;
    for (Event &e : s->wt_ev) if (!e) HIPCHK(hipEventCreate(&e.p));
    rc = ensure(s, s->wt_base, size_t(fr.total_work) + 1); if (rc) return rc;
    fr.wt_base = s->wt_base;
    auto pass = [&](int phase) -> int {
        fr.weighted_phase = phase;
        HIPCHK(hipMemcpyAsync(s->dev_frame, &fr, sizeof(DevFrame), hipMemcpyHostToDevice, s->stream));
        HIPCHK(hipMemsetAsync(s->work_counter, 0, 64 * sizeof(unsigned long long), s->stream));
        hipLaunchKernelGGL(g_render_kernels_weighted[k], dim3(grid), dim3(RT_BLOCK), 0, s->stream, (const DevScene *)s->dev_scene, (const DevFrame *)s->dev_frame);
        HIPCHK(hipGetLastError());
        return RT_OK;
    };
    HIPCHK(hipEventRecord(s->ev0, s->stream));
    if ((rc = pass(1))) return rc;
    HIPCHK(hipEventRecord(s->wt_ev[0], s->stream));
    hipLaunchKernelGGL(weighted_scan_sums_kernel, dim3(RT_WSCAN_BLOCKS), dim3(RT_WSCAN_THREADS), 0, s->stream, (const unsigned *)s->wt_base, (unsigned long long)fr.total_work, s->wt_sums);
    hipLaunchKernelGGL(weighted_scan_top_kernel, dim3(1), dim3(RT_WSCAN_THREADS), 0, s->stream, s->wt_base, (unsigned long long)fr.total_work, s->wt_sums, s->wt_total);
    hipLaunchKernelGGL(weighted_scan_apply_kernel, dim3(RT_WSCAN_BLOCKS), dim3(RT_WSCAN_THREADS), 0, s->stream, s->wt_base, (unsigned long long)fr.total_work, (const unsigned long long *)s->wt_sums);
    HIPCHK(hipGetLastError());
    HIPCHK(hipEventRecord(s->wt_ev[1], s->stream));
    HIPCHK(hipStreamSynchronize(s->stream));
    const unsigned long long n_points = *s->wt_total;
    auto late_fail = [&](int code, const char *msg) { s->last_weighted = false; s->last_pipeline = false; s->have_timing = false; s->wt_points = 0; return fail(code, msg); };
    if (n_points >= 0xffffffffull) return late_fail(RT_EINVAL, "rt_render: strategy \"weighted\": more than 2^32 - 2 shading points in the frame");
    s->wt_points = n_points;
    const bool mixed = s->light_draws < 0;
    const int nD = int(s->n_drawing_lights);
    size_t rec_floats = size_t(n_points) * size_t(R);
    fr.wt_mixed = mixed ? 1 : 0; fr.wt_nd = unsigned(nD); fr.wt_recbase = nullptr;
    if (mixed) {
        {
            const double W = double(fr.total_work ? fr.total_work : 1), Pavg = double(n_points) / W;
            const double at_least = double(n_points) * double(1 + 2 * (nL - nD)) + double(nD) * W * Pavg * (Pavg + 1.0);
            if (at_least >= 4294967295.0) return late_fail(RT_EINVAL, "rt_render: strategy \"weighted\" with lights of mixed RNG use: the survey's records exceed 2^32 floats (quadratic in a sample's shading points)");
        }
// ... 187 lines not shown
        if (const char *e = knob("PBRT_HIP_EXIT_THRESH")) fr.exit_thresh = std::atoi(e);
        fr.dbg_x = fr.dbg_y = -1000000;
        if (const char *e = knob("PBRT_HIP_DEBUG_PIXEL")) std::sscanf(e, "%d,%d", &fr.dbg_x, &fr.dbg_y);
        fr.phase_sync = tiny ? 1 : 0;
        if (const char *e = knob("PBRT_HIP_PHASE_SYNC")) fr.phase_sync = std::atoi(e);
        fr.pipeline = (!tiny && s->volume.present) ? 1 : 0;
        if (const char *e = knob("PBRT_HIP_PIPELINE")) fr.pipeline = std::atoi(e) != 0;
        if (fr.max_depth > 250 || fr.max_depth < 0) fr.pipeline = 0;
        if (fr.dims_max_n >= 65535) fr.pipeline = 0;
        if (s->dev.n_lights >= 65535u) fr.pipeline = 0;
        if (rd->integrator == RT_INTEGRATOR_DIRECT && rd->strategy == RT_STRATEGY_WEIGHTED) fr.pipeline = 0;
        if (bidir) { fr.pipeline = 0; fr.xcd_bands = 0; }
        if (rd->integrator == RT_INTEGRATOR_DEBUG) { fr.pipeline = 0; fr.high_occupancy = 0; }
        if (fr.shard_count == 1 && !fr.pipeline) {
            fr.tile_w = fr.tile_h = fr.tiles_x = 0; fr.tile_pixels = 1;
            fr.total_work = fr.total_pixels * fr.spp;
            fr.mega_tile = 32;
            if (const char *e = knob("PBRT_HIP_MEGA_TILE")) fr.mega_tile = std::max(0, std::atoi(e));
            if (fr.mega_tile > 4096 || fr.total_work > 0xffffffffull) fr.mega_tile = 0;
        }
        if (fr.trav_mode != 3 || fr.high_occupancy) fr.trav_mode = 2;
    }
    fr.div = framediv_make(unsigned(fr.spp), unsigned(fr.xs), unsigned(fr.x_end - fr.x_start), unsigned(fr.y_end - fr.y_start), unsigned(fr.mega_tile),
                           (unsigned long long)fr.tile_pixels * fr.spp, unsigned(fr.tile_w), unsigned(fr.tiles_x));
    fr.work_counter = s->work_counter; fr.counters = s->counters; fr.spill = s->spill; fr.n_threads = s->n_threads;
    fr.frames = s->frames;
    if (need_film && !s->accum) return fail(RT_ESTATE, "rt_render: no film bound (call rt_film_bind first)");
    if (need_film && (fr.x_pixel_count != s->film_w || fr.y_pixel_count != s->film_h))
        return fail(RT_EINVAL, "rt_render: film size does not match the bound film");
    return RT_OK;
}

int rt_camera_rays(RtScene *s, const RtRenderDesc *rd, uint64_t first, uint32_t count, RtRay *rays_out) {
    if (!s || !rd || !rays_out) return fail(RT_EINVAL, "null argument");
    HIPCHK(hipSetDevice(s->device));
    DevFrame fr; int rc = make_frame(s, rd, fr, false); if (rc) return rc;
    DevBuf<RtRay> dev;
    if ((rc = dev.grow(count ? count : 1))) return rc;
    hipLaunchKernelGGL(camera_kernel, dim3((count + 255) / 256), dim3(256), 0, s->stream, s->dev, fr,
                       (unsigned long long)first, count, dev.p);
    HIPCHK(hipGetLastError());
    HIPCHK(hipStreamSynchronize(s->stream));
    HIPCHK(hipMemcpy(rays_out, dev, size_t(count) * sizeof(RtRay), hipMemcpyDeviceToHost));
    return RT_OK;
}
int rt_camera_rays_device(RtScene *s, const RtRenderDesc *rd, uint64_t first, uint32_t count, RtRay *dev_rays) {
    if (!s) return fail(RT_EINVAL, "rt_camera_rays_device: null scene");
    if (!rd) return fail(RT_EINVAL, "rt_camera_rays_device: null render description");
    if (!dev_rays) return fail(RT_EINVAL, "rt_camera_rays_device: null ray pointer");
    if ((reinterpret_cast<uintptr_t>(dev_rays) & 15u) != 0) return fail(RT_EINVAL, "rt_camera_rays_device: dev_rays is not 16-byte aligned");
    if (count > (1u << 30)) return fail(RT_EINVAL, "rt_camera_rays_device: count = " + std::to_string(count) + " is above 2^30");
    HIPCHK(hipSetDevice(s->device));
    RtRenderDesc d = *rd;
    if (d.integrator == RT_INTEGRATOR_BIDIRECTIONAL || (d.integrator == RT_INTEGRATOR_DIRECT && d.strategy == RT_STRATEGY_ALL)) d.integrator = RT_INTEGRATOR_WHITTED;
    DevFrame fr; int rc = make_frame(s, &d, fr, false); if (rc) return rc;
    if (count == 0) return RT_OK;
    hipLaunchKernelGGL(camera_kernel, dim3((count + 255) / 256), dim3(256), 0, s->stream, s->dev, fr, (unsigned long long)first, count, dev_rays);
    HIPCHK(hipGetLastError());
    return RT_OK;
}

static int trace_common(RtScene *s, const RtRay *rays, uint32_t n, int any, RtHit *hits, uint8_t *occ) {
    if (!s || !rays || (!hits && !occ)) return fail(RT_EINVAL, "null argument");
    HIPCHK(hipSetDevice(s->device));
    if (n == 0) return RT_OK;
    if (int rc = ensure(s, s->trace_buf, size_t(n) * 3)) return rc;
    std::vector<float4> host(size_t(n) * 2);
    for (uint32_t i = 0; i < n; ++i) {
        host[i] = make_float4(rays[i].o[0], rays[i].o[1], rays[i].o[2], rays[i].mint);
        host[size_t(n) + i] = make_float4(rays[i].d[0], rays[i].d[1], rays[i].d[2], rays[i].maxt);
    }
    unsigned qc[RT_QC_STRIDE] = {0};
    qc[0] = any ? 0u : n; qc[RT_QC_ANY] = any ? n : 0u;
    HIPCHK(hipMemcpyAsync(s->trace_buf, host.data(), host.size() * sizeof(float4), hipMemcpyHostToDevice, s->stream));
    HIPCHK(hipMemcpyAsync(s->trace_qc, qc, sizeof qc, hipMemcpyHostToDevice, s->stream));
    TraceJob job{};
    job.q_o = s->trace_buf; job.q_d = s->trace_buf + n; job.q_slot = nullptr; job.q_count = s->trace_qc; job.hit = s->trace_buf + 2 * size_t(n);
    job.n_slots = 0; job.spill = s->spill; job.n_threads = s->n_threads; job.counters = s->counters;
    flavour::Request rq = request_of(s);
    rq.count = true;
    const int k = flavour::Trace::index(rq);
    HIPWARN(hipEventRecord(s->ev0, s->stream));
    hipLaunchKernelGGL(g_pipe_trace[k], dim3(s->grids.trace[k]), dim3(RT_BLOCK), 0, s->stream, (const DevScene *)s->dev_scene, job);
    HIPWARN(hipEventRecord(s->ev1, s->stream)); HIPWARN(hipEventRecord(s->ev2, s->stream)); s->have_timing = true; s->last_pipeline = false;
    HIPCHK(hipGetLastError());
    HIPCHK(hipMemcpyAsync(host.data(), s->trace_buf + 2 * size_t(n), size_t(n) * sizeof(float4), hipMemcpyDeviceToHost, s->stream));
    HIPCHK(hipStreamSynchronize(s->stream));
    for (uint32_t i = 0; i < n; ++i) {
        int prim; std::memcpy(&prim, &host[i].x, 4);
        if (any) occ[i] = prim >= 0 ? 1 : 0;
        else { hits[i].prim = prim; hits[i].t = host[i].y; hits[i].b1 = host[i].z; hits[i].b2 = host[i].w; }
    }
    return RT_OK;
}
int rt_trace_closest(RtScene *s, const RtRay *rays, uint32_t n, RtHit *hits_out) { return trace_common(s, rays, n, 0, hits_out, nullptr); }
int rt_trace_any(RtScene *s, const RtRay *rays, uint32_t n, uint8_t *occluded_out) { return trace_common(s, rays, n, 1, nullptr, occluded_out); }
int rt_render(RtScene *s, const RtRenderDesc *rd) {
    if (!s || !rd) return fail(RT_EINVAL, "null argument");
    HIPCHK(hipSetDevice(s->device));
    const bool debug = rd->integrator == RT_INTEGRATOR_DEBUG;
    if ((rd->integrator < RT_INTEGRATOR_WHITTED || rd->integrator > RT_INTEGRATOR_BIDIRECTIONAL) && !debug) return fail(RT_EINVAL, "unknown integrator");
    const bool bidir = rd->integrator == RT_INTEGRATOR_BIDIRECTIONAL;
    if (rd->max_depth < 0 && !bidir && !debug) return fail(RT_EINVAL, "rt_render: negative maxdepth");
    if (debug) {
        const unsigned codes = unsigned(rd->strategy);
        if ((codes >> 24) != 0u || (codes & 0xffu) > unsigned(RT_DEBUG_HIT) || ((codes >> 8) & 0xffu) > unsigned(RT_DEBUG_HIT) || ((codes >> 16) & 0xffu) > unsigned(RT_DEBUG_HIT))
            return fail(RT_EINVAL, "rt_render: unknown debug channel code (the debug integrator's strategy holds three RT_DEBUG_* codes, red | green << 8 | blue << 16)");
    }
    if (bidir) {
        if (s->volume.present) return fail(RT_EINVAL, "rt_render: the bidirectional integrator in a participating medium is not supported");
        if (s->dev.n_lights == 0) return fail(RT_EINVAL, "rt_render: the bidirectional integrator needs at least one light (the reference indexes lights[-1] in a scene with no lights)");
    }
    if (!rd->filter_table) return fail(RT_EINVAL, "rt_render: no filter table");
    DevFrame fr; int rc = make_frame(s, rd, fr, true); if (rc) return rc;
    const bool weighted = rd->integrator == RT_INTEGRATOR_DIRECT && rd->strategy == RT_STRATEGY_WEIGHTED;
    if (rd->integrator == RT_INTEGRATOR_DIRECT && (rd->strategy < RT_STRATEGY_ALL || rd->strategy > RT_STRATEGY_WEIGHTED)) return fail(RT_EINVAL, "rt_render: unknown direct lighting strategy");
    if (weighted) {
        if (fr.shard_count != 1) return fail(RT_EINVAL, "rt_render: strategy \"weighted\" is a recurrence over the whole frame in the sampler's order (transport.cpp:71-122): one shard only");
        if (s->volume.present && s->light_draws != 0) return fail(RT_EINVAL, "rt_render: strategy \"weighted\" in a participating medium needs lights whose estimates draw no random numbers "
                                                                            "(point / spot / distant / single-triangle / quadric lights): an emitter of several triangles draws its triangle, and the medium makes "
                                                                            "the draw's position in the stream depend on occlusion");
        if (s->n_infinite != 0) return fail(RT_EINVAL, "rt_render: strategy \"weighted\" with an infinite light is not supported (the light draws a random number per estimate); "
                                                       "use strategy \"one\" or \"all\"");
        if (s->dev.n_lights > 2048u) return fail(RT_EINVAL, "rt_render: strategy \"weighted\" holds the per-light tables of its recurrence in LDS: at most 2048 lights");
        if (fr.total_work >= 0xffffffffull) return fail(RT_EINVAL, "rt_render: strategy \"weighted\": more than 2^32 - 2 camera samples in the frame");
    }
    const bool skip_film = knob("PBRT_HIP_DEBUG_NOFILM") != nullptr;
    FilmGather fg; rc = film_gather_plan(s, fr, fg); if (rc) return rc;
    int vol_nmax = 0;
    fr.dens_cap = 0;
    if (s->volume.present) {
        if (!(rd->step_size > 0.f)) return fail(RT_EINVAL, "rt_render: volume integrator stepsize must be positive");
        if (rd->volume_integrator != RT_VOLUME_EMISSION && rd->volume_integrator != RT_VOLUME_SINGLE) return fail(RT_EINVAL, "rt_render: unknown volume integrator");
        const float ex = s->volume.p1[0] - s->volume.p0[0], ey = s->volume.p1[1] - s->volume.p0[1], ez = s->volume.p1[2] - s->volume.p0[2];
        const double diag = std::sqrt(double(ex) * ex + double(ey) * ey + double(ez) * ez);
        const double nsteps = std::ceil(diag / rd->step_size) + 2;
        if (nsteps > 65536) return fail(RT_EINVAL, "rt_render: stepsize too small for the medium (more than 65536 march steps)");
        vol_nmax = int(nsteps);
        if (s->density_kind != RT_DENSITY_NONE) {
            const double *wb = s->vol_world;
            const double wx = wb[3] - wb[0], wy = wb[4] - wb[1], wz = wb[5] - wb[2];
            const double wdiag = std::sqrt(wx * wx + wy * wy + wz * wz);
            const float half = .5f * rd->step_size;
            const double taus = std::ceil(wdiag / double(half)) + 2;
            if (taus > double(1 << 20)) return fail(RT_EINVAL, "rt_render: stepsize too small for the density region (an optical-depth march would take more than 2^20 samples)");
            double u[6] = {wb[0], wb[1], wb[2], wb[3], wb[4], wb[5]};
            const float *c2w = s->dev.cam.camera_to_world;
            const double cam[3] = {c2w[3], c2w[7], c2w[11]};
            for (int i = 0; i < 3; ++i) { u[i] = std::min(u[i], cam[i]); u[3 + i] = std::max(u[3 + i], cam[i]); }
            const float *sb = s->dev.bounds;
            if (sb[0] <= sb[3] && sb[1] <= sb[4] && sb[2] <= sb[5])
                for (int i = 0; i < 3; ++i) { u[i] = std::min(u[i], double(sb[i])); u[3 + i] = std::max(u[3 + i], double(sb[3 + i])); }
            const double ux = u[3] - u[0], uy = u[4] - u[1], uz = u[5] - u[2];
            const float tmax = std::nextafter(float(std::sqrt(ux * ux + uy * uy + uz * uz)), INFINITY);
            volatile float tv = tmax;
            const float adv = tv + half;
            if (!std::isfinite(tmax) || !(adv > tmax))
                return fail(RT_EINVAL, "rt_render: stepsize too small for the density region: at the scene's ray parameters t + .5 * stepsize == t, the optical-depth march would not advance");
            fr.dens_cap = int(taus);
            vol_nmax = std::max(vol_nmax, int(std::ceil(wdiag / rd->step_size)) + 2);
            if (vol_nmax > 65536) return fail(RT_EINVAL, "rt_render: stepsize too small for the medium (more than 65536 march steps)");
        }
        fr.vol_nmax = vol_nmax;
    }
    {
        const size_t cap = s->samples.cap;
        const size_t local_pixels = size_t(fr.total_work / fr.spp);
        const size_t need = ((local_pixels + 63) / 64 * 64 + 64) * size_t(fr.spp) * 2;
        rc = ensure(s, s->samples, need); if (rc) return rc;
        if (cap != s->samples.cap) HIPCHK(hipMemsetAsync(s->samples, 0, s->samples.bytes(), s->stream));
    }
    fr.samples = s->samples; s->samples_last = fr.total_work; s->samples_spp = fr.spp;
    HIPCHK(hipMemcpyAsync(s->filter_dev, rd->filter_table, 256 * sizeof(float), hipMemcpyHostToDevice, s->stream));
    if (debug) { rc = upload_tex_uv(s); if (rc) return rc; }
    { hipError_t pre = hipGetLastError(); if (pre != hipSuccess) return fail(RT_EDEVICE, std::string("pending HIP error before launch: ") + hipGetErrorString(pre)); }
    s->rendered = true;
    rc = fr.pipeline ? render_pipeline(s, rd, fr) : bidir ? render_bidir(s, rd, fr) : weighted ? render_weighted(s, rd, fr) : render_mega(s, rd, fr);
    if (rc) return rc;
    s->last_pipeline = fr.pipeline != 0; s->last_weighted = weighted;
    if (!skip_film) { rc = film_gather_launch(s, fr, fg, (const DevFrame *)s->dev_frame, 0, fr.y_pixel_count); if (rc) return rc; }
    HIPCHK(hipEventRecord(s->ev2, s->stream));
    s->have_timing = true;
#ifdef RT_PROFILE
    {
        unsigned long long v[24];
        HIPCHK(hipStreamSynchronize(s->stream));
        HIPCHK(hipMemcpy(v, s->counters, sizeof v, hipMemcpyDeviceToHost));
        std::fprintf(stderr, "RT_PROFILE shade_cyc=%llu trav_cyc=%llu outer=%llu inner=%llu rounds=%llu act_lane_rounds=%llu rays_at_trav_start=%llu desc_cyc=%llu leaf_cyc=%llu chunks=%llu pooled_rounds=%llu leaf_iters=%llu\n",
                     v[8], v[9], v[10], v[11], v[12], v[13], v[14], v[15], v[16], v[17], v[18], v[19]);
#ifdef RT_PROFILE_STAGES
        {
            unsigned long long st[32];
            HIPCHK(hipMemcpy(st, s->counters + 24, sizeof st, hipMemcpyDeviceToHost));
            static const char *names[16] = {"FETCH", "VERTEX", "DIRECT_NEXT", "SHADOW_DONE", "MIS_DONE", "ED_BSDF", "ED_DONE", "BOUNCE", "SPECULAR", "SPEC_TRANS", "RETURN", "VOL_BEGIN", "VOL_STEP", "POP", "FINISH", "EXIT"};
            for (int i = 0; i < 16; ++i) if (st[2 * i + 1])
                std::fprintf(stderr, "RT_PROFILE_STAGE %-12s cycles=%llu passes=%llu lane_visits=%llu\n", names[i], st[2 * i], st[2 * i + 1] >> 40, st[2 * i + 1] & ((1ull << 40) - 1));
            HIPCHK(hipMemsetAsync(s->counters + 24, 0, 32 * sizeof(unsigned long long), s->stream));
        }
#endif
        HIPCHK(hipMemsetAsync(s->counters + 8, 0, 16 * sizeof(unsigned long long), s->stream));
    }
#endif
    return RT_OK;
}
int rt_sync(RtScene *s) {
    if (!s) return fail(RT_EINVAL, "null scene");
    HIPCHK(hipSetDevice(s->device));
    HIPCHK(hipStreamSynchronize(s->stream));
    return RT_OK;
}

int rt_counters(RtScene *s, RtCounters *out) {
    if (!s || !out) return fail(RT_EINVAL, "null argument");
    HIPCHK(hipSetDevice(s->device));
    HIPCHK(hipStreamSynchronize(s->stream));
    unsigned long long v[8];
    HIPCHK(hipMemcpy(v, s->counters, sizeof v, hipMemcpyDeviceToHost));
    out->camera_rays = v[0]; out->closest_rays = v[1]; out->any_rays = v[2]; out->nodes_visited = v[3];
    out->leaf_refs = v[4]; out->tri_tests = v[5]; out->bad_samples = v[6]; out->stack_overflows = v[7];
    return RT_OK;
}
int rt_counters_reset(RtScene *s) {
    if (!s) return fail(RT_EINVAL, "null scene");
    HIPCHK(hipSetDevice(s->device));
    HIPCHK(hipMemsetAsync(s->counters, 0, 24 * sizeof(unsigned long long), s->stream));
    return RT_OK;
}
int rt_set_counting(RtScene *s, int enabled) {
    if (!s) return fail(RT_EINVAL, "null scene");
    s->counting = enabled != 0;
    return RT_OK;
}
int rt_last_render_ms(RtScene *s, float *total_ms, float *kernel_ms) {
    if (!s || !s->have_timing) return fail(RT_ESTATE, "no timed launch yet");
    HIPCHK(hipSetDevice(s->device));
    HIPCHK(hipEventSynchronize(s->ev2));
    float k = 0.f, t = 0.f;
    HIPCHK(hipEventElapsedTime(&k, s->ev0, s->ev1));
    HIPCHK(hipEventElapsedTime(&t, s->ev0, s->ev2));
    if (total_ms) *total_ms = t;
    if (kernel_ms) *kernel_ms = k;
    return RT_OK;
}
int rt_last_render_stats(RtScene *s, RtRenderStats *out) {
    if (!s || !out) return fail(RT_EINVAL, "null argument");
    if (!s->have_timing) return fail(RT_ESTATE, "no timed launch yet");
    HIPCHK(hipSetDevice(s->device));
    HIPCHK(hipEventSynchronize(s->ev2));
    std::memset(out, 0, sizeof *out);
    HIPCHK(hipEventElapsedTime(&out->render_ms, s->ev0, s->ev1));
    HIPCHK(hipEventElapsedTime(&out->total_ms, s->ev0, s->ev2));
    out->gather_ms = out->total_ms - out->render_ms;
    out->pipeline = s->last_pipeline ? 1 : 0;
    if (s->last_pipeline) {
        out->iterations = s->pipe_iters; out->timed_iterations = s->pipe_timed;
        float sum = 0.f;
        float sum2 = 0.f, sum3 = 0.f;
        for (int i = 0; i < s->pipe_timed; ++i) {
            float ms = 0.f; HIPCHK(hipEventElapsedTime(&ms, s->pipe_ev[6 * i], s->pipe_ev[6 * i + 1])); sum += ms;
            HIPCHK(hipEventElapsedTime(&ms, s->pipe_ev[6 * i + 2], s->pipe_ev[6 * i + 3])); sum2 += ms;
            if (s->last_marches) { HIPCHK(hipEventElapsedTime(&ms, s->pipe_ev[6 * i + 4], s->pipe_ev[6 * i + 5])); sum3 += ms; }
        }
        out->trace_ms = sum; out->shade_ms = sum2; out->march_ms = sum3;
        out->slots = s->pipe_slots;
    } else out->trace_ms = out->render_ms;
    out->bands = s->last_pipeline ? 0 : 1;
    if (s->last_weighted) {
        out->weighted_points = s->wt_points;
        hipEvent_t seq[6] = {s->ev0, s->wt_ev[0], s->wt_ev[1], s->wt_ev[2], s->wt_ev[3], s->ev1};
        for (int i = 0; i < 5; ++i) HIPCHK(hipEventElapsedTime(&out->weighted_ms[i], seq[i], seq[i + 1]));
    }
    return RT_OK;
}

}
```

### pbrt-v1_amd/csrc/hip/rt_render_kernel.h

```cpp
#pragma once
#include "rt_integrate.h"

namespace rt {

#ifndef RT_MEGA_CHUNK
#define RT_MEGA_CHUNK 64
#endif
static_assert(RT_MEGA_CHUNK >= 64, "one fresh chunk must cover a whole wave's fetch");
RT_DEV unsigned long long uniform64(unsigned long long v) {
    const unsigned lo = __builtin_amdgcn_readfirstlane(unsigned(v)), hi = __builtin_amdgcn_readfirstlane(unsigned(v >> 32));
    return (unsigned long long)hi << 32 | lo;
}


RT_DEV unsigned long long band_lo(unsigned long long total, unsigned r, unsigned n) {
    if (r >= n) return total;
    return (total / RT_MEGA_CHUNK) * r / n * RT_MEGA_CHUNK;
}

#ifndef RT_MIN_WAVES
#define RT_MIN_WAVES 1
#endif
#ifndef RT_MEGA_BYV
#define RT_MEGA_BYV 1
#endif


#ifndef RT_HIGH_OCC_WAVES
#define RT_HIGH_OCC_WAVES 4
#endif
template <bool COUNT, int INTEG, int ACCEL, bool VOL, int MINW, bool EXT>
__global__ __launch_bounds__(RT_BLOCK, (EXT && COUNT && INTEG == RT_INTEGRATOR_PATH && ACCEL == RT_ACCEL_GRID && !VOL && MINW < 3) ? 3 : MINW) void render_kernel(const DevScene *__restrict__ scp,
                                                                       const DevFrame *__restrict__ frp) {
    __shared__ uint2 lds_stack[RT_STACK_LDS * RT_BLOCK];
    constexpr bool POOL = MINW < RT_HIGH_OCC_WAVES;
    constexpr int PN = POOL ? RT_BLOCK : 64;
    __shared__ unsigned long long pool_key[PN];
    __shared__ float4 pool_res[PN];
    __shared__ unsigned pool_head[PN];
    __shared__ float4 pool_ray[3 * PN];
    __shared__ float lds_tm_own[POOL ? 1 : RT_STACK_LDS * RT_BLOCK];
    float RT_L *lds_tm = (float RT_L *)lds_tm_own;
    const DevScene &sc = *scp;
    const DevFrame &fr = *frp;
    const unsigned wave0 = POOL ? (threadIdx.x & ~63u) : 0u;
    const PoolLds pool = {(unsigned long long RT_L *)pool_key + wave0, (float4 RT_L *)pool_res + wave0, (unsigned RT_L *)pool_head + wave0,
                          (float4 RT_L *)pool_ray + 3 * wave0};
    const unsigned gtid = blockIdx.x * RT_BLOCK + threadIdx.x;
    const int lane = threadIdx.x & 63;
    constexpr bool BYV = RT_MEGA_BYV != 0 && !POOL && INTEG == RT_INTEGRATOR_PATH && !VOL && !EXT && !COUNT;
    Lane ln;
    ln.vf = 0u;
    ln.stage = ST_FETCH; ln.has_ray = false; ln.fsp = 0; ln.tv.active = false; ln.tv.hit_prim = -1;
    ln.L = mk3(0.f); ln.thr = mk3(1.f); ln.alpha = 0.f; ln.depth = 0; ln.specular = false;
    TravCounters tc; tc.nodes = tc.leaf_refs = tc.tris = tc.spills = 0;
    RT_PFT(tc.c_desc = tc.c_leaf = tc.n_chunks = tc.n_pooled = tc.n_iter = 0;)
    unsigned c_cam = 0, c_closest = 0, c_any = 0, c_bad = 0;

#ifdef RT_PROFILE
    unsigned long long pf_shade = 0, pf_trav = 0, pf_outer = 0, pf_inner = 0, pf_rounds = 0, pf_act = 0, pf_rays = 0, pf_t0 = 0;
#define RT_PF(x) x
#else
#define RT_PF(x)
#endif
#ifdef RT_TAIL_PROBE
    const unsigned long long tp_start = __builtin_amdgcn_s_memrealtime();
    unsigned long long tp_empty = 0, tp_taken = 0;
#endif
    unsigned long long w_next = 0, w_end = 0;
    const unsigned n_bands = fr.xcd_bands ? 8u : 1u, home = fr.xcd_bands ? (blockIdx.x & 7u) : 0u;
    unsigned band_shift = 0;

    int phase = (INTEG == RT_INTEGRATOR_PATH && fr.phase_sync && !BYV) ? 1 : -1;
    for (;;) {
        RT_PF(pf_t0 = __builtin_readcyclecounter(); ++pf_outer;)
        do {
            RT_PF(++pf_inner;)
            if constexpr (BYV) advance_pass_byv<COUNT, ACCEL, EXT>(sc, fr, ln, gtid, &c_closest, &c_any, &c_bad);
            else advance_pass<COUNT, INTEG, VOL, EXT>(sc, fr, ln, gtid, &c_closest, &c_any, &c_bad, phase);
            const unsigned long long want = phase == 0 ? 0ull : __ballot(!ln.has_ray && ln.stage == ST_FETCH);
            if (want) {
                const unsigned n_want = unsigned(__popcll(want));
                const unsigned long long have = w_end - w_next;
                unsigned long long fresh = 0, fresh_end = 0;
                if (have < n_want) {
                    const int leader = __ffsll((long long)want) - 1;
#pragma unroll 1
                    while (band_shift < n_bands) {
                        const unsigned r = (home + band_shift) % n_bands;
                        const unsigned long long lo = band_lo(fr.total_work, r, n_bands), hi = band_lo(fr.total_work, r + 1u, n_bands);
                        unsigned long long base = 0;
                        if (lane == leader) base = atomicAdd(fr.work_counter + 8u * r, (unsigned long long)RT_MEGA_CHUNK);
                        base = uniform64(__shfl(base, leader));
                        if (lo + base < hi) { fresh = lo + base; fresh_end = fresh + RT_MEGA_CHUNK < hi ? fresh + RT_MEGA_CHUNK : hi; break; }
                        ++band_shift;
                    }
                }
                const bool none_left = band_shift >= n_bands;
#ifdef RT_TAIL_PROBE
                if (none_left && !tp_empty) tp_empty = __builtin_amdgcn_s_memrealtime();
#endif
                const unsigned long long rk = __popcll(want & ((1ull << lane) - 1ull));
                const unsigned long long w_mine = rk < have ? w_next + rk : fresh + (rk - have);
                const bool got = rk < have || w_mine < fresh_end;
                if (have < n_want) {
                    const unsigned long long took = n_want - have < fresh_end - fresh ? n_want - have : fresh_end - fresh;
                    w_next = fresh + took; w_end = fresh_end;
                } else w_next += n_want;
                if (!ln.has_ray && ln.stage == ST_FETCH && !got) { if (none_left) ln.stage = ST_EXIT; }
                else if (!ln.has_ray && ln.stage == ST_FETCH) {
                    const unsigned long long w = w_mine;
#ifdef RT_TAIL_PROBE
                    tp_taken += 1;
#endif
                    {
                        unsigned long long pixel; int s;
                        bool ok;
                        if (fr.mega_tile > 0) { unsigned px; tile_order_to_sample(fr, unsigned(w), px, s); pixel = px; ok = true; }
                        else ok = work_to_sample(fr, w, pixel, s);
                        if (ok) {
                            Ray ray;
                            setup_sample(sc, fr, ln, pixel, s, ray);
                            ln.work = fr.mega_tile > 0 ? uint32_t(pixel * unsigned(fr.spp) + unsigned(s)) : uint32_t(w);
                            if (INTEG == RT_INTEG_DIRECT_WEIGHTED) ln.ord = fr.weighted_phase == 1 ? 0u : RT_GPTR(const unsigned, fr.wt_base)[ln.work];
                            ln.L = mk3(0.f); ln.thr = mk3(1.f); ln.alpha = 0.f; ln.depth = 0; ln.fsp = 0;
                            ln.specular = false;
                            if (COUNT) ++c_cam;
                            accel_begin<ACCEL>(ln.tv, sc, ray, false);
                            if (VOL) vol_store_ray(fr, 0, gtid, ray);
                            ln.has_ray = true; ln.stage = ST_VERTEX;
                            if (BYV) ln.vf = BV_B | BV_CUR_B;
                        }
                    }
                }
            }
        } while (__any(!ln.has_ray && stage_in_phase(ln.stage, phase)));
        if (phase >= 0) phase ^= 1;
        RT_PF({ unsigned long long t1 = __builtin_readcyclecounter(); pf_shade += t1 - pf_t0; pf_t0 = t1; pf_rays += __popcll(__ballot(ln.has_ray && ln.tv.active)); })
        if (!__any(ln.has_ray)) {
            if (!__any(ln.stage != ST_EXIT)) break;
            continue;
        }
        for (;;) {
            if constexpr (BYV) {
                const bool next = ln.has_ray && !ln.tv.active && (ln.vf & (BV_QM | BV_QB)) != 0u;
                if (__any(next)) { if (next) byv_ray_advance<COUNT, ACCEL, EXT>(sc, ln, &c_closest, &c_any); }
            }
            const bool act = ln.has_ray && ln.tv.active;
            const unsigned long long am = __ballot(act);
            if (!am) break;
            RT_PF(++pf_rounds; pf_act += __popcll(am);)
            if (fr.exit_thresh > 0 && __popcll(am) <= fr.exit_thresh && __any(!act && ln.stage != ST_EXIT)) break;
            if (POOL && fr.trav_mode == 3) accel_round_pooled<COUNT, ACCEL, EXT>(ln.tv, ln.has_ray, sc, (uint2 RT_L *)lds_stack, RT_GPTR(uint2, fr.spill), fr.n_threads, gtid, tc, pool);
            else trace_round<COUNT, ACCEL, EXT, RT_STACK_LDS, !POOL>(ln.tv, ln.has_ray, sc, (uint2 RT_L *)lds_stack, lds_tm, RT_GPTR(uint2, fr.spill), fr.n_threads, gtid, tc, fr.leaf_min);
        }
        if (ln.has_ray && !ln.tv.active && !(BYV && (ln.vf & (BV_QM | BV_QB)) != 0u)) ln.has_ray = false;
        RT_PF(pf_trav += __builtin_readcyclecounter() - pf_t0;)
    }
#ifdef RT_PROFILE
    if (lane == 0) {
        unsigned long long v[12] = {pf_shade, pf_trav, pf_outer, pf_inner, pf_rounds, pf_act, pf_rays, tc.c_desc, tc.c_leaf, tc.n_chunks, tc.n_pooled, tc.n_iter};
        for (int k = 0; k < 12; ++k) atomicAdd(fr.counters + 8 + k, v[k]);
    }
#endif

#ifdef RT_TAIL_PROBE
    {
        for (int off = 32; off > 0; off >>= 1) tp_taken += __shfl_down(tp_taken, off);
        if (lane == 0 && fr.probe) {
            unsigned long long *o = fr.probe + size_t(gtid >> 6) * 4u;
            o[0] = tp_start; o[1] = tp_empty; o[2] = __builtin_amdgcn_s_memrealtime(); o[3] = tp_taken;
        }
    }
#endif
    if (COUNT && !(INTEG == RT_INTEG_DIRECT_WEIGHTED && fr.weighted_phase != 3)) {
        unsigned long long v[8] = {c_cam, c_closest, c_any, tc.nodes, tc.leaf_refs, tc.tris, c_bad, tc.spills};
#pragma unroll
        for (int k = 0; k < 8; ++k) {
            unsigned long long x = v[k];
            for (int off = 32; off > 0; off >>= 1) x += __shfl_down(x, off);
            if (lane == 0 && x) atomicAdd(fr.counters + k, x);
        }
    }
}

typedef void (*RenderKernelFn)(const DevScene *, const DevFrame *);

}
```

### pbrt-v1_amd/csrc/hip/rt_scene.hip

```cpp
#include "rt_host.h"
#include "../../../include/pbrt_hip_material.h"

static void host_tri_frame(const float *v, bool flip, float nn[3], float sn[3]) {
    const float du1 = 0.f - 1.f, du2 = 1.f - 1.f, dv1 = 0.f - 1.f, dv2 = 0.f - 1.f;
    const float determinant = du1 * dv2 - dv1 * du2;
    const float invdet = 1.f / determinant;
    float dpdu[3], dpdv[3];
    for (int a = 0; a < 3; ++a) {
        const float dp1 = v[a] - v[6 + a], dp2 = v[3 + a] - v[6 + a];
        dpdu[a] = invdet * ((dv2 * dp1) - (dv1 * dp2));
        dpdv[a] = invdet * ((-du2 * dp1) + (du1 * dp2));
    }
    float c[3] = {(dpdu[1] * dpdv[2]) - (dpdu[2] * dpdv[1]), (dpdu[2] * dpdv[0]) - (dpdu[0] * dpdv[2]), (dpdu[0] * dpdv[1]) - (dpdu[1] * dpdv[0])};
    float inv = 1.f / sqrtf(c[0] * c[0] + c[1] * c[1] + c[2] * c[2]);
    for (int a = 0; a < 3; ++a) { nn[a] = c[a] * inv; if (flip) nn[a] = -1.f * nn[a]; }
    inv = 1.f / sqrtf(dpdu[0] * dpdu[0] + dpdu[1] * dpdu[1] + dpdu[2] * dpdu[2]);
    for (int a = 0; a < 3; ++a) sn[a] = dpdu[a] * inv;
}

static void leaf_records_fill_host(const RefVec &slot_prim, const std::vector<DevTri> &tris, std::vector<float4> &ltris) {
    ltris.assign(slot_prim.size() * RT_TRI_STRIDE + 4, make_float4(0.f, 0.f, 0.f, 0.f));
    for (size_t i = 0; i < slot_prim.size(); ++i) {
        const uint32_t prim = slot_prim[i];
        float4 q2 = tris[prim].q2; std::memcpy(&q2.w, &prim, 4);
// ... 393 lines not shown
    s->materials_host = mats;
    if ((rc = upload(s, mats.data(), mats.size(), &s->dev.materials))) return rc;

    std::vector<float> ltris(size_t(d->n_light_tris) * 16, 0.f);
    std::vector<DevLight> lights(d->n_lights);
    for (uint32_t i = 0; i < d->n_lights; ++i) {
        const RtLight &L = d->lights[i]; DevLight &o = lights[i];
        o.type = L.type; o.n_samples = L.n_samples < 1 ? 1 : L.n_samples;
        for (int c = 0; c < 3; ++c) { o.color[c] = L.color[c]; o.pos[c] = L.pos[c]; }
        o.first_tri = L.first_tri; o.n_tris = L.n_tris; o.reverse_orientation = L.reverse_orientation;
        o.flip_normal = L.flip_normal; o.area = 0.f;
        for (int c = 0; c < 3; ++c) o.dir[c] = L.dir[c];
        for (int c = 0; c < 9; ++c) o.w2l[c] = L.world_to_light[c];
        o.cos_total = L.cos_total_width; o.cos_falloff = L.cos_falloff_start;
        {
            const float a = o.w2l[0], b = o.w2l[1], c = o.w2l[2], d3 = o.w2l[3], e = o.w2l[4], f = o.w2l[5], g = o.w2l[6], h = o.w2l[7], i9 = o.w2l[8];
            const float cof[9] = {e * i9 - f * h, c * h - b * i9, b * f - c * e, f * g - d3 * i9, a * i9 - c * g, c * d3 - a * f, d3 * h - e * g, b * g - a * h, a * e - b * d3};
            for (int k = 0; k < 9; ++k) o.l2w[k] = cof[k];
            o.l2w_scale = L.type == RT_LIGHT_SPOT ? 1.f / (a * cof[0] + b * cof[3] + c * cof[6]) : 0.f;
        }
        o.quadric = L.quadric_plus1 - 1;
        if (L.quadric_plus1 < 0 || uint32_t(L.quadric_plus1) > d->n_quadrics) return fail(RT_EINVAL, "rt_scene_create: light refers to a quadric out of range");
        if (L.type < RT_LIGHT_POINT || L.type > RT_LIGHT_INFINITE) return fail(RT_EINVAL, "rt_scene_create: unknown light type");
        if (L.type == RT_LIGHT_INFINITE) { s->has_ext = true; ++s->n_infinite; }
        if (L.type != RT_LIGHT_AREA) continue;
        if (size_t(L.first_tri) + L.n_tris > d->n_light_tris) return fail(RT_EINVAL, "rt_scene_create: light triangle range out of bounds");
        float area = 0.f; std::vector<float> areas;
        for (uint32_t k = 0; k < L.n_tris; ++k) {
            const float *v = d->light_tris + size_t(L.first_tri + k) * 9;
            float *q = &ltris[size_t(L.first_tri + k) * 16];
            std::memcpy(q, v, 9 * sizeof(float));
            { float nl[3], sn_unused[3]; host_tri_frame(v, L.flip_normal != 0, nl, sn_unused); q[12] = nl[0]; q[13] = nl[1]; q[14] = nl[2]; }
            float ax = v[3] - v[0], ay = v[4] - v[1], az = v[5] - v[2];
            float bx = v[6] - v[0], by = v[7] - v[1], bz = v[8] - v[2];
            float cx = (ay * bz) - (az * by), cy = (az * bx) - (ax * bz), cz = (ax * by) - (ay * bx);
            float a = 0.5f * sqrtf(cx * cx + cy * cy + cz * cz);
            q[9] = a; area += a; areas.push_back(a);
        }
        float prev = 0.f;
        for (uint32_t k = 0; k < L.n_tris; ++k) {
            float c = prev + areas[k] / area;
            ltris[size_t(L.first_tri + k) * 16 + 10] = c; prev = c;
        }
        o.area = (L.n_tris == 1) ? areas[0] : area;
    }
    if ((rc = upload(s, lights.data(), lights.size(), &s->dev.lights))) return rc;
    s->lights_host = lights;
    if ((rc = upload(s, ltris.data(), ltris.size(), &s->dev.light_tris))) return rc;
    {
        std::vector<unsigned> flags(d->n_lights ? d->n_lights : 1, 0u);
        s->n_drawing_lights = 0;
        for (uint32_t i = 0; i < d->n_lights; ++i) {
            const int draws = (d->lights[i].type == RT_LIGHT_AREA && d->lights[i].quadric_plus1 == 0 && d->lights[i].n_tris > 1) ? 1 : 0;
            if (i == 0) s->light_draws = draws; else if (draws != s->light_draws) s->light_draws = -1;
            flags[i] = unsigned(draws); s->n_drawing_lights += unsigned(draws);
        }
        if ((rc = upload(s, flags.data(), flags.size(), &s->light_draw_flags))) return rc;
    }

    s->dev.n_tris = d->n_tris; s->dev.n_lights = d->n_lights; s->dev.n_infinite = int(s->n_infinite);
    s->dev.accel_kind = s->accel_kind;
    for (int a = 0; a < 3; ++a) { s->dev.nvox[a] = s->gridacc.nvox[a]; s->dev.gwidth[a] = s->gridacc.width[a]; s->dev.ginv_width[a] = s->gridacc.inv_width[a]; }
    std::memcpy(s->dev.bounds, s->tree.bounds, sizeof s->dev.bounds);
    s->dev.cam = d->camera; s->dev.vol = d->volume; s->volume = d->volume;

    hipDeviceProp_t prop;
    HIPCHK(hipGetDeviceProperties(&prop, s->device));
    s->n_cus = prop.multiProcessorCount;
    unsigned trace_per_cu = ~0u;
    if (const char *e = knob("PBRT_HIP_TRACE_BLOCKS_PER_CU")) trace_per_cu = unsigned(std::max(1, std::atoi(e)));
    unsigned mx = 0;
    auto resident = [&](const auto &kernels, auto &grids, unsigned at_most = ~0u) -> int {
        static_assert(sizeof kernels / sizeof kernels[0] == sizeof grids / sizeof grids[0], "a grid per table entry");
        for (size_t k = 0; k < kernels.size(); ++k) {
            int per_cu = 0;
            HIPCHK(hipOccupancyMaxActiveBlocksPerMultiprocessor(&per_cu, (const void *)kernels[k], RT_BLOCK, 0));
            grids[k] = unsigned(prop.multiProcessorCount) * std::max(1u, std::min(unsigned(std::max(per_cu, 0)), at_most));
            mx = std::max(mx, grids[k]);
        }
        return RT_OK;
    };
    ResidentGrids &g = s->grids;
    for (int i = 0; i <= RT_INTEGRATOR_PATH; ++i) if ((rc = resident(*g_render_kernels[i], g.mega[i]))) return rc;
    if ((rc = resident(g_render_kernels_weighted, g.weighted)) || (rc = resident(g_render_kernels_bidir, g.bidir))) return rc;
    s->grid = mx;
    {
        const unsigned others = mx;
        if ((rc = resident(g_render_kernels_debug, g.debug))) return rc;
        for (unsigned &n : g.debug) n = std::min(n, others);
        mx = others;
    }
    if ((rc = resident(g_pipe_trace, g.trace, trace_per_cu)) || (rc = resident(g_pipe_march, g.march))) return rc;
    s->n_threads = mx * RT_BLOCK;
    s->spill_depth = s->tree.max_depth > RT_TRACE_STACK ? s->tree.max_depth - RT_TRACE_STACK + 1 : 1;
    if ((rc = s->work_counter.grow(64))) return rc;
    if ((rc = s->counters.grow(64))) return rc;
    HIPCHK(hipMemsetAsync(s->counters, 0, 64 * sizeof(unsigned long long), s->stream));
    if ((rc = s->filter_dev.grow(256)) || (rc = s->dev_scene.grow(1)) || (rc = s->dev_frame.grow(1))) return rc;
    HIPCHK(hipMemcpy(s->dev_scene, &s->dev, sizeof(DevScene), hipMemcpyHostToDevice));
    HIPCHK(hipEventCreate(&s->ev2.p));
    if ((rc = s->spill.grow(size_t(s->spill_depth) * s->n_threads * 2))) return rc;
    if ((rc = s->dev_pool.grow(1)) || (rc = s->trace_qc.grow(RT_QC_STRIDE))) return rc;
    HIPCHK(hipHostMalloc((void **)&s->h_qcount.p, size_t(RT_PIPE_QN) * RT_QC_STRIDE * sizeof(unsigned), hipHostMallocDefault));
    HIPCHK(hipStreamSynchronize(s->stream));
    guard.p = nullptr;
    *out = s;
    return RT_OK;
}

int rt_scene_destroy(RtScene *s) {
    if (!s) return RT_OK;
    HIPWARN(hipSetDevice(s->device));
    if (s->stream) hipStreamSynchronize(s->stream);
    delete s;
    return RT_OK;
}

int rt_scene_set_stream(RtScene *s, void *hip_stream) {
    if (!s) return fail(RT_EINVAL, "null scene");
    if (s->own_stream) { HIPWARN(hipStreamSynchronize(s->own_stream)); s->own_stream.reset(); }
    s->stream = static_cast<hipStream_t>(hip_stream);
    return RT_OK;
}
int rt_scene_get_stream(RtScene *s, void **hip_stream_out) {
    if (!s || !hip_stream_out) return fail(RT_EINVAL, "rt_scene_get_stream: null argument");
    *hip_stream_out = s->stream;
    return RT_OK;
}

int rt_scene_set_density(RtScene *s, const RtDensityRegion *r) {
    if (!s || !r) return fail(RT_EINVAL, "rt_scene_set_density: null argument");
    if (s->rendered) return fail(RT_ESTATE, "rt_scene_set_density: the scene has rendered a frame already");
    if (s->density_kind != RT_DENSITY_NONE) return fail(RT_ESTATE, "rt_scene_set_density: the scene has a density region already");
    if (!s->volume.present) return fail(RT_EINVAL, "rt_scene_set_density: the scene has no medium (RtSceneDesc.volume.present == 0)");
    if (r->kind != RT_DENSITY_EXPONENTIAL && r->kind != RT_DENSITY_GRID) return fail(RT_EINVAL, "rt_scene_set_density: unknown density kind");
    double a[4][8];
    for (int i = 0; i < 4; ++i) for (int j = 0; j < 4; ++j) { a[i][j] = s->volume.world_to_volume[4 * i + j]; a[i][4 + j] = i == j ? 1.0 : 0.0; }
    for (int c = 0; c < 4; ++c) {
        int piv = c;
        for (int i = c + 1; i < 4; ++i) if (std::fabs(a[i][c]) > std::fabs(a[piv][c])) piv = i;
        if (!(std::fabs(a[piv][c]) > 0.0)) return fail(RT_EINVAL, "rt_scene_set_density: singular world_to_volume");
        for (int j = 0; j < 8; ++j) std::swap(a[c][j], a[piv][j]);
        const double inv = 1.0 / a[c][c];
        for (int j = 0; j < 8; ++j) a[c][j] *= inv;
        for (int i = 0; i < 4; ++i) if (i != c) { const double f = a[i][c]; for (int j = 0; j < 8; ++j) a[i][j] -= f * a[c][j]; }
    }
    double wb[6] = {INFINITY, INFINITY, INFINITY, -INFINITY, -INFINITY, -INFINITY};
    for (int k = 0; k < 8; ++k) {
        const double q[3] = {(k & 1) ? s->volume.p1[0] : s->volume.p0[0], (k & 2) ? s->volume.p1[1] : s->volume.p0[1], (k & 4) ? s->volume.p1[2] : s->volume.p0[2]};
        double w[4];
        for (int i = 0; i < 4; ++i) w[i] = a[i][4] * q[0] + a[i][5] * q[1] + a[i][6] * q[2] + a[i][7];
        for (int i = 0; i < 3; ++i) { const double v = w[3] != 1.0 ? w[i] / w[3] : w[i]; wb[i] = std::min(wb[i], v); wb[3 + i] = std::max(wb[3 + i], v); }
    }
    for (double v : wb) if (!std::isfinite(v)) return fail(RT_EINVAL, "rt_scene_set_density: the volume's world bound is not finite");
    HIPCHK(hipSetDevice(s->device));
    const float *grid = nullptr;
    if (r->kind == RT_DENSITY_GRID) {
        const long long total = (long long)r->nx * r->ny * r->nz;
        if (r->nx <= 0 || r->ny <= 0 || r->nz <= 0 || total > 0x7fffffffLL) return fail(RT_EINVAL, "rt_scene_set_density: grid counts must be positive with nx*ny*nz < 2^31");
        if (!r->density) return fail(RT_EINVAL, "rt_scene_set_density: null density grid");
        int rc = upload(s, r->density, size_t(total), &grid); if (rc) return rc;
    }
    DevScene &d = s->dev;
    d.dens_kind = r->kind; d.dens_a = r->a; d.dens_b = r->b;
    for (int i = 0; i < 3; ++i) d.dens_up[i] = r->updir[i];
    d.dens_n[0] = r->nx; d.dens_n[1] = r->ny; d.dens_n[2] = r->nz; d.dens_grid = grid;
// ... 218 lines not shown
```

Baseline: 3488.

## Add fixed-frame specialized render kernels with compile-time sampler and camera facts

Adds a 'Fixed' flavour of the megakernel, templated on a traits class that bakes in the stratified sampler, a pinhole non-environment camera, tile-order pixel indexing and one sample per light. Under these facts, per-sample runtime branches and the light_dims lookups are folded away, and dim_value shortcuts to a direct RNG draw. The kernel body moves into a shared include so the generic and fixed kernels share code. Host code computes resident grids for the new table, capped at the matching generic kernel's grid. The fixed path is only selected when a qualifies() check passes, and the dim_value shortcut assumes the stratified value with n=1 reduces to a plain RNG draw.

```diff
diff --git a/include/pbrt_hip.h b/include/pbrt_hip.h
--- a/include/pbrt_hip.h
+++ b/include/pbrt_hip.h
@@ -236,6 +236,7 @@
     float march_ms;
     uint64_t weighted_points;
     float weighted_ms[5];
+    int32_t fixed_frame;
 } RtRenderStats;
 int rt_film_resolve_device(RtScene *s, const float *dev_accum, uint64_t n, int premultiply, float *dev_rgb, float *dev_alpha);
 int rt_film_resolve_device_rgba(RtScene *s, const float *dev_accum, uint64_t n, int premultiply, float *dev_rgba);
diff --git a/pbrt-v1_amd/__init__.py b/pbrt-v1_amd/__init__.py
--- a/pbrt-v1_amd/__init__.py
+++ b/pbrt-v1_amd/__init__.py
@@ -18,7 +18,7 @@
 HOST_FLAGS = ["-O2", "-std=c++17", "-fPIC", "-shared", "-msse2", "-mfpmath=sse", "-fvisibility=hidden", "-fvisibility-inlines-hidden"]
 
 
-HIP_UNITS = ("rt_kernels.hip", "rt_scene.hip", "rt_film.hip", "rt_trace.hip", "rt_mega_w.hip", "rt_mega_d.hip", "rt_mega_dw.hip", "rt_mega_p.hip", "rt_mega_b.hip", "rt_mega_g.hip", "rt_pipe_w.hip", "rt_pipe_d.hip",
+HIP_UNITS = ("rt_kernels.hip", "rt_scene.hip", "rt_film.hip", "rt_trace.hip", "rt_mega_w.hip", "rt_mega_d.hip", "rt_mega_dw.hip", "rt_mega_p.hip", "rt_mega_b.hip", "rt_mega_g.hip", "rt_mega_f.hip", "rt_pipe_w.hip", "rt_pipe_d.hip",
              "rt_pipe_p.hip", "rt_pipe_v.hip", "rt_march.hip", "rt_rays.hip", "kd_build.cpp", "grid_build.cpp", "leaf_layout.cpp")
 
 
@@ -153,7 +153,7 @@
 class RtRenderStats(C.Structure):
     _fields_ = [("total_ms", C.c_float), ("render_ms", C.c_float), ("trace_ms", C.c_float), ("gather_ms", C.c_float),
                 ("pipeline", C.c_int32), ("iterations", C.c_int32), ("timed_iterations", C.c_int32), ("slots", C.c_uint32), ("shade_ms", C.c_float), ("bands", C.c_int32), ("march_ms", C.c_float),
-                ("weighted_points", C.c_uint64), ("weighted_ms", C.c_float * 5)]
+                ("weighted_points", C.c_uint64), ("weighted_ms", C.c_float * 5), ("fixed_frame", C.c_int32)]
 
     def as_dict(self):
         return {n: (list(getattr(self, n)) if n == "weighted_ms" else getattr(self, n)) for n, _ in self._fields_}
diff --git a/pbrt-v1_amd/csrc/hip/rt_fixed_frame.h b/pbrt-v1_amd/csrc/hip/rt_fixed_frame.h
--- /dev/null
+++ b/pbrt-v1_amd/csrc/hip/rt_fixed_frame.h
@@ -0,0 +1,78 @@
+#pragma once
+#include "rt_flavour.h"
+
+#ifndef RT_FIXED_SAMPLER
+#define RT_FIXED_SAMPLER 1
+#endif
+#ifndef RT_FIXED_N1
+#define RT_FIXED_N1 1
+#endif
+#ifndef RT_FIXED_CAMERA
+#define RT_FIXED_CAMERA 1
+#endif
+#ifndef RT_FIXED_TILE_ORDER
+#define RT_FIXED_TILE_ORDER 1
+#endif
+
+namespace rt {
+namespace fixed {
+
+struct Any {
+    static constexpr int sampler = -1;
+    static constexpr bool no_lens = false;
+    static constexpr bool no_env_camera = false;
+    static constexpr bool tile_order = false;
+    static constexpr bool all_n1 = false;
+};
+struct Frame {
+    static constexpr int sampler = RT_FIXED_SAMPLER ? int(RT_SAMPLER_STRATIFIED) : -1;
+    static constexpr bool no_lens = RT_FIXED_CAMERA != 0;
+    static constexpr bool no_env_camera = RT_FIXED_CAMERA != 0;
+    static constexpr bool tile_order = RT_FIXED_TILE_ORDER != 0;
+    static constexpr bool all_n1 = RT_FIXED_N1 != 0;
+};
+
+struct Facts {
+    int integrator;
+    int sampler;
+    bool weighted;
+    float lens_radius;
+    int camera_type;
+    int shard_count;
+    int mega_tile;
+    int dims_max_n;
+    bool counting, ext, vol;
+    bool high_occ;
+};
+constexpr bool qualifies(const Facts &f) {
+    return f.integrator >= RT_INTEGRATOR_WHITTED && f.integrator <= RT_INTEGRATOR_PATH && !f.weighted &&
+           f.sampler == RT_SAMPLER_STRATIFIED &&
+           f.lens_radius == 0.f &&
+           (f.camera_type == RT_CAMERA_PERSPECTIVE || f.camera_type == RT_CAMERA_ORTHOGRAPHIC) &&
+           f.shard_count == 1 && f.mega_tile > 0 &&
+           f.dims_max_n <= 1 &&
+           !f.counting && !f.ext && !f.vol && f.high_occ;
+}
+
+}
+
+namespace flavour {
+struct Fixed {
+    static constexpr int N = 6;
+    static constexpr int index(const Request &r) { return 2 * r.integ + (r.grid ? 1 : 0); }
+    static constexpr int integrator(int k) { return k >> 1; }
+    static constexpr Flavour flavour(int k) { return Flavour{false, k & 1, false, false, RT_HIGH_OCC_WAVES, true}; }
+    static constexpr Request request(int k) { Request r = flavour(k).request(); r.integ = integrator(k); return r; }
+    static constexpr int generic(int k) { return Mega::index(request(k)); }
+};
+constexpr bool fixed_round_trips() {
+    for (int k = 0; k < Fixed::N; ++k) {
+        if (Fixed::index(Fixed::request(k)) != k) return false;
+        const Flavour g = Mega::flavour(Fixed::generic(k), Fixed::integrator(k)), f = Fixed::flavour(k);
+        if (g.count != f.count || g.accel != f.accel || g.vol != f.vol || g.ext != f.ext || g.waves != f.waves || g.high_occ != f.high_occ) return false;
+    }
+    return true;
+}
+static_assert(fixed_round_trips(), "Fixed: index(request(k)) != k, or entry k is not the twin of a Mega entry");
+}
+}
diff --git a/pbrt-v1_amd/csrc/hip/rt_host.h b/pbrt-v1_amd/csrc/hip/rt_host.h
--- a/pbrt-v1_amd/csrc/hip/rt_host.h
+++ b/pbrt-v1_amd/csrc/hip/rt_host.h
@@ -35,6 +35,7 @@
 
 namespace rt {
 extern const flavour::Table<RenderKernelFn, flavour::Mega> g_render_kernels_whitted, g_render_kernels_direct, g_render_kernels_path;
+extern const flavour::Table<RenderKernelFn, flavour::Fixed> g_render_kernels_fixed;
 extern const flavour::Table<RenderKernelFn, flavour::Weighted> g_render_kernels_weighted;
 extern const flavour::Table<RenderKernelFn, flavour::Bidir> g_render_kernels_bidir;
 extern const flavour::Table<RenderKernelFn, flavour::Debug> g_render_kernels_debug;
@@ -47,6 +48,7 @@
 static const flavour::Table<PipeShadeFn, flavour::Shade> *const g_pipe_shade[RT_INTEGRATOR_PATH + 1] = {&g_pipe_shade_whitted, &g_pipe_shade_direct, &g_pipe_shade_path};
 struct ResidentGrids {
     flavour::Table<unsigned, flavour::Mega> mega[RT_INTEGRATOR_PATH + 1];
+    flavour::Table<unsigned, flavour::Fixed> fixed;
     flavour::Table<unsigned, flavour::Weighted> weighted;
     flavour::Table<unsigned, flavour::Bidir> bidir;
     flavour::Table<unsigned, flavour::Debug> debug;
@@ -117,6 +119,7 @@
     uint32_t n_tris = 0;
     PipePlanes pool; DevBuf<unsigned> q_count; DevBuf<unsigned long long> wave_work; DevBuf<PipePool> dev_pool;
     Pinned<unsigned> h_qcount;
+    bool last_fixed = false;
     bool last_pipeline = false, last_marches = false; int pipe_iters = 0, pipe_timed = 0; unsigned pipe_slots = 0;
     DevBuf<float4> trace_buf;
     int n_cus = 0;
diff --git a/pbrt-v1_amd/csrc/hip/rt_integrate.h b/pbrt-v1_amd/csrc/hip/rt_integrate.h
--- a/pbrt-v1_amd/csrc/hip/rt_integrate.h
+++ b/pbrt-v1_amd/csrc/hip/rt_integrate.h
@@ -1,6 +1,7 @@
 #pragma once
 #include "rt_shade.h"
 #include "rt_texture.h"
+#include "rt_fixed_frame.h"
 
 namespace rt {
 
@@ -87,8 +88,10 @@
     if (n0 == 0 && fr.sampler != RT_SAMPLER_LOWDISCREPANCY) return rng_base(0xFFFFFFFFu, fr.seed);
     return rng_base(n0, fr.seed);
 }
+template <class FX = fixed::Any>
 RT_DEV float dim_value(const DevFrame &fr, const Lane &ln, const DimReq &r, int j, int d) {
-    if (fr.sampler == RT_SAMPLER_STRATIFIED) return lhs_value(ln, r, j, d);
+    if constexpr (FX::sampler == RT_SAMPLER_STRATIFIED && FX::all_n1) return (0 + rng_f32(ln.rng.base, ln.dim_base + r.f_base + d)) * 1.f;
+    if (FX::sampler == RT_SAMPLER_STRATIFIED || fr.sampler == RT_SAMPLER_STRATIFIED) return lhs_value(ln, r, j, d);
     if (fr.sampler == RT_SAMPLER_RANDOM) return rng_f32(ln.rng.base, ln.dim_base + r.f_base + j * r.dims + d);
     const uint32_t pb = pixel_stream(fr, ln);
     const int P = fr.spp, n = r.n, s = int(ln.work % uint32_t(P));
@@ -146,9 +149,10 @@
     (void)pixel_index;
 }
 
+template <class FX = fixed::Any>
 RT_DEV Ray camera_ray(const RtCamera &cam, float ix, float iy, float lensU, float lensV) {
     Ray r;
-    if (cam.type == RT_CAMERA_ENVIRONMENT) {
+    if (!FX::no_env_camera && cam.type == RT_CAMERA_ENVIRONMENT) {
         r.o = xform_point(cam.camera_to_world, mk3(0.f, 0.f, 0.f));
         const float theta = RT_PI * iy / cam.y_res;
         const float phi = 2 * RT_PI * ix / cam.x_res;
@@ -160,7 +164,7 @@
     V3 Pcamera = xform_point(cam.raster_to_camera, mk3(ix, iy, 0.f));
     r.o = Pcamera;
     r.d = cam.type == RT_CAMERA_ORTHOGRAPHIC ? mk3(0.f, 0.f, 1.f) : Pcamera;
-    if (cam.lens_radius > 0.f) {
+    if (!FX::no_lens && cam.lens_radius > 0.f) {
         float lu, lv; concentric_disk(lensU, lensV, lu, lv);
         lu *= cam.lens_radius; lv *= cam.lens_radius;
         float ft = (cam.focal_distance - cam.hither) / r.d.z;
@@ -223,17 +227,18 @@
     pixel = (ty * T + qy) * W + tx * T + qx;
 }
 
+template <class FX = fixed::Any>
 RT_DEV void setup_sample(const DevScene &sc, const DevFrame &fr, Lane &ln, unsigned long long pixel, int s, Ray &ray) {
     const int w = fr.x_end - fr.x_start;
     int px, py;
-    if (fr.total_pixels <= 0xffffffffull) { const unsigned row = fastdiv(unsigned(pixel), fr.div.width); px = fr.x_start + int(unsigned(pixel) - row * unsigned(w)); py = fr.y_start + int(row); }
+    if (FX::tile_order || fr.total_pixels <= 0xffffffffull) { const unsigned row = fastdiv(unsigned(pixel), fr.div.width); px = fr.x_start + int(unsigned(pixel) - row * unsigned(w)); py = fr.y_start + int(row); }
     else { px = fr.x_start + int(pixel % w); py = fr.y_start + int(pixel / w); }
     const uint32_t n0 = uint32_t(pixel * fr.spp);
     ln.sample_index = n0 + uint32_t(s);
     ln.rng.base = rng_base(ln.sample_index, fr.seed);
     float lu = 0.5f, lv = 0.5f;
-    const bool need_lens = sc.cam.lens_radius > 0.f;
-    if (fr.sampler == RT_SAMPLER_STRATIFIED) {
+    const bool need_lens = !FX::no_lens && sc.cam.lens_radius > 0.f;
+    if (FX::sampler == RT_SAMPLER_STRATIFIED || fr.sampler == RT_SAMPLER_STRATIFIED) {
         const uint32_t pix_base = (pixel == 0) ? rng_base(0xFFFFFFFFu, fr.seed) : rng_base(n0, fr.seed);
         ln.dim_base = (s == 0 && pixel != 0) ? fr.pixgen_draws : 0u;
         stratified_camera_sample(fr, uint32_t(pixel), s, px, py, pix_base, ln.image_x, ln.image_y, lu, lv, need_lens);
@@ -256,8 +261,8 @@
             lu = van_der_corput(uint32_t(lp), rng_u32(pix_base, lb)); lv = sobol2(uint32_t(lp), rng_u32(pix_base, lb + 1));
         }
     }
-    ln.rng.ctr = ln.dim_base + ((fr.sampler == RT_SAMPLER_LOWDISCREPANCY) ? 0u : fr.lhs_total);
-    ray = camera_ray(sc.cam, ln.image_x, ln.image_y, lu, lv);
+    ln.rng.ctr = ln.dim_base + ((FX::sampler != RT_SAMPLER_STRATIFIED && fr.sampler == RT_SAMPLER_LOWDISCREPANCY) ? 0u : fr.lhs_total);
+    ray = camera_ray<FX>(sc.cam, ln.image_x, ln.image_y, lu, lv);
     ln.image_x = (ln.image_x + 1.f) - 1.f; ln.image_y = (ln.image_y + 1.f) - 1.f;
 }
 
@@ -618,7 +623,7 @@
     ln.stage = ST_RETURN;
 }
 
-template <bool COUNT, int INTEG_, bool VOL, bool EXT, int STAGE, bool DEFER = false, bool PARK = false>
+template <bool COUNT, int INTEG_, bool VOL, bool EXT, int STAGE, bool DEFER = false, bool PARK = false, class FX = fixed::Any>
 RT_DEV void stage_body(const DevScene &sc, const DevFrame &fr, Lane &ln, unsigned gtid,
                        unsigned *c_closest, unsigned *c_any, unsigned *c_bad) {
     constexpr bool WEIGHTED = INTEG_ == RT_INTEG_DIRECT_WEIGHTED;
@@ -687,11 +692,11 @@
                 if (ln.li >= nLights) { ++ln.ord; ln.stage = ST_SPECULAR; return; }
                 ln.rng.ctr = ln.ctr0;
             }
-            const float ls1 = dim_value(fr, ln, fr.two_d[0], 0, 0), ls2 = dim_value(fr, ln, fr.two_d[0], 0, 1);
-            ln.bs1 = dim_value(fr, ln, fr.two_d[1], 0, 0); ln.bs2 = dim_value(fr, ln, fr.two_d[1], 0, 1);
-            ln.bcs = dim_value(fr, ln, fr.one_d[1], 0, 0);
+            const float ls1 = dim_value<FX>(fr, ln, fr.two_d[0], 0, 0), ls2 = dim_value<FX>(fr, ln, fr.two_d[0], 0, 1);
+            ln.bs1 = dim_value<FX>(fr, ln, fr.two_d[1], 0, 0); ln.bs2 = dim_value<FX>(fr, ln, fr.two_d[1], 0, 1);
+            ln.bcs = dim_value<FX>(fr, ln, fr.one_d[1], 0, 0);
             if (fr.weighted_phase == 2) {
-                if (ln.li == 0 && ln.lj == 0) RT_GPTR(float, fr.wt_rec)[weighted_record(fr, ln, nLights)] = dim_value(fr, ln, fr.one_d[0], 0, 0);
+                if (ln.li == 0 && ln.lj == 0) RT_GPTR(float, fr.wt_rec)[weighted_record(fr, ln, nLights)] = dim_value<FX>(fr, ln, fr.one_d[0], 0, 0);
                 estimate_direct_begin<EXT, DEFER>(sc, ln, ln.li, ls1, ls2);
             } else {
                 const float2 pick = RT_GPTR(const float2, fr.wt_pick)[ln.ord++];
@@ -709,10 +714,10 @@
             if (from_sampler) {
                 const int i1 = (INTEG == RT_INTEGRATOR_PATH) ? 3 * k : 0;
                 const int i2 = (INTEG == RT_INTEGRATOR_PATH) ? 3 * k : 0;
-                un = dim_value(fr, ln, fr.one_d[i1], 0, 0);
-                ls1 = dim_value(fr, ln, fr.two_d[i2], 0, 0); ls2 = dim_value(fr, ln, fr.two_d[i2], 0, 1);
-                ln.bs1 = dim_value(fr, ln, fr.two_d[i2 + 1], 0, 0); ln.bs2 = dim_value(fr, ln, fr.two_d[i2 + 1], 0, 1);
-                ln.bcs = dim_value(fr, ln, fr.one_d[i1 + 1], 0, 0);
+                un = dim_value<FX>(fr, ln, fr.one_d[i1], 0, 0);
+                ls1 = dim_value<FX>(fr, ln, fr.two_d[i2], 0, 0); ls2 = dim_value<FX>(fr, ln, fr.two_d[i2], 0, 1);
+                ln.bs1 = dim_value<FX>(fr, ln, fr.two_d[i2 + 1], 0, 0); ln.bs2 = dim_value<FX>(fr, ln, fr.two_d[i2 + 1], 0, 1);
+                ln.bcs = dim_value<FX>(fr, ln, fr.one_d[i1 + 1], 0, 0);
             } else {
                 un = ln.rng.next_float();
                 ls1 = ln.rng.next_float(); ls2 = ln.rng.next_float();
@@ -727,9 +732,9 @@
             const DimReq RT_G *ld = RT_GPTR(const DimReq, fr.light_dims) + 3 * ln.li;
             const DimReq rl = ld[0], rb = ld[1], rc = ld[2];
             if (ln.lj == 0) ln.Ld_light = mk3(0.f);
-            const float ls1 = dim_value(fr, ln, rl, ln.lj, 0), ls2 = dim_value(fr, ln, rl, ln.lj, 1);
-            ln.bs1 = dim_value(fr, ln, rb, ln.lj, 0); ln.bs2 = dim_value(fr, ln, rb, ln.lj, 1);
-            ln.bcs = dim_value(fr, ln, rc, ln.lj, 0);
+            const float ls1 = dim_value<FX>(fr, ln, rl, ln.lj, 0), ls2 = dim_value<FX>(fr, ln, rl, ln.lj, 1);
+            ln.bs1 = dim_value<FX>(fr, ln, rb, ln.lj, 0); ln.bs2 = dim_value<FX>(fr, ln, rb, ln.lj, 1);
+            ln.bcs = dim_value<FX>(fr, ln, rc, ln.lj, 0);
             estimate_direct_begin<EXT, DEFER>(sc, ln, ln.li, ls1, ls2);
             return;
         }
@@ -836,7 +841,7 @@
             ln.stage = ST_SPECULAR;
         } else {
             ln.Ld_light = ln.Ld_light + ln.Ld;
-            const int ns = RT_GPTR(const DimReq, fr.light_dims)[3 * ln.li].n;
+            const int ns = FX::all_n1 ? 1 : int(RT_GPTR(const DimReq, fr.light_dims)[3 * ln.li].n);
             if (++ln.lj >= ns) {
                 ln.L_all = ln.L_all + ln.Ld_light * (1.f / float(ns));
                 ln.lj = 0; ++ln.li;
@@ -851,8 +856,8 @@
         const int k = ln.depth;
         float bs1, bs2, bcs;
         if (k < 3) {
-            bs1 = dim_value(fr, ln, fr.two_d[3 * k + 2], 0, 0); bs2 = dim_value(fr, ln, fr.two_d[3 * k + 2], 0, 1);
-            bcs = dim_value(fr, ln, fr.one_d[3 * k + 2], 0, 0);
+            bs1 = dim_value<FX>(fr, ln, fr.two_d[3 * k + 2], 0, 0); bs2 = dim_value<FX>(fr, ln, fr.two_d[3 * k + 2], 0, 1);
+            bcs = dim_value<FX>(fr, ln, fr.one_d[3 * k + 2], 0, 0);
         } else { bs1 = ln.rng.next_float(); bs2 = ln.rng.next_float(); bcs = ln.rng.next_float(); }
         V3 wi; float pdf; int flags;
         V3 f = bsdf_sample_f<EXT>(m, ln.v, ln.v.wo, wi, bs1, bs2, bcs, pdf, BX_ALL, flags);
@@ -971,10 +976,10 @@
     else { r.d = ln.dB; ln.vf = (ln.vf & ~BV_QB) | BV_CUR_B; }
     if (ACCEL == RT_ACCEL_GRID) grid_begin(ln.tv, sc, r, false); else trav_begin(ln.tv, sc, r, false);
 }
-template <bool COUNT, int ACCEL, bool EXT>
+template <bool COUNT, int ACCEL, bool EXT, class FX = fixed::Any>
 RT_DEV void advance_pass_byv(const DevScene &sc, const DevFrame &fr, Lane &ln, unsigned gtid, unsigned *c_closest, unsigned *c_any, unsigned *c_bad) {
     constexpr int INTEG = RT_INTEGRATOR_PATH;
-#define RT_BV_BODY(S) stage_body<COUNT, INTEG, false, EXT, S, true>(sc, fr, ln, gtid, c_closest, c_any, c_bad)
+#define RT_BV_BODY(S) stage_body<COUNT, INTEG, false, EXT, S, true, false, FX>(sc, fr, ln, gtid, c_closest, c_any, c_bad)
     const int nLights = int(sc.n_lights);
     if (!ln.has_ray && (ln.stage == ST_VERTEX || ln.stage == ST_ED_DONE)) {
         byv_ray_result<COUNT, EXT>(sc, ln, c_closest, c_any);
@@ -1027,16 +1032,16 @@
     const bool first = stage == ST_VERTEX || stage == ST_DIRECT_NEXT;
     return phase == 0 ? first : !first;
 }
-template <bool COUNT, int INTEG_, bool VOL, bool EXT, bool DEFER = false, bool PARK = false>
+template <bool COUNT, int INTEG_, bool VOL, bool EXT, bool DEFER = false, bool PARK = false, class FX = fixed::Any>
 RT_DEV void advance_pass(const DevScene &sc, const DevFrame &fr, Lane &ln, unsigned gtid,
                          unsigned *c_closest, unsigned *c_any, unsigned *c_bad, int phase) {
     constexpr int INTEG = INTEG_ == RT_INTEG_DIRECT_WEIGHTED ? int(RT_INTEGRATOR_DIRECT) : INTEG_;
 #ifdef RT_PROFILE_STAGES
 #define RT_RUN(S) { const unsigned long long m_ = __ballot(!ln.has_ray && ln.stage == S); if (m_) { const unsigned long long t_ = __builtin_readcyclecounter(); \
-        if (!ln.has_ray && ln.stage == S) stage_body<COUNT, INTEG_, VOL, EXT, S, DEFER, PARK>(sc, fr, ln, gtid, c_closest, c_any, c_bad); \
+        if (!ln.has_ray && ln.stage == S) stage_body<COUNT, INTEG_, VOL, EXT, S, DEFER, PARK, FX>(sc, fr, ln, gtid, c_closest, c_any, c_bad); \
         if (__lane_id() == 0) { atomicAdd(fr.counters + 24 + 2 * S, __builtin_readcyclecounter() - t_); atomicAdd(fr.counters + 24 + 2 * S + 1, (unsigned long long)__popcll(m_) | (1ull << 40)); } } }
 #else
-#define RT_RUN(S) if (!ln.has_ray && ln.stage == S) stage_body<COUNT, INTEG_, VOL, EXT, S, DEFER, PARK>(sc, fr, ln, gtid, c_closest, c_any, c_bad)
+#define RT_RUN(S) if (!ln.has_ray && ln.stage == S) stage_body<COUNT, INTEG_, VOL, EXT, S, DEFER, PARK, FX>(sc, fr, ln, gtid, c_closest, c_any, c_bad)
 #endif
     if constexpr (INTEG_ == RT_INTEGRATOR_DEBUG) {
         RT_RUN(ST_VERTEX);
diff --git a/pbrt-v1_amd/csrc/hip/rt_kernels.hip b/pbrt-v1_amd/csrc/hip/rt_kernels.hip
--- a/pbrt-v1_amd/csrc/hip/rt_kernels.hip
+++ b/pbrt-v1_amd/csrc/hip/rt_kernels.hip
@@ -184,9 +184,14 @@
 static int render_mega(RtScene *s, const RtRenderDesc *rd, DevFrame &fr) {
     int rc = bind_scratch(s, rd, fr, s->n_threads); if (rc) return rc;
     const bool debug = rd->integrator == RT_INTEGRATOR_DEBUG;
-    const int k = debug ? flavour::Debug::index(request_of(s, rd, &fr)) : flavour::Mega::index(request_of(s, rd, &fr));
-    const unsigned grid = debug ? s->grids.debug[k] : s->grids.mega[rd->integrator][k];
-    const RenderKernelFn kernel = debug ? g_render_kernels_debug[k] : (*g_render_kernels[rd->integrator])[k];
+    bool fixed_frame = fixed::qualifies(fixed::Facts{rd->integrator, fr.sampler, rd->integrator == RT_INTEGRATOR_DIRECT && rd->strategy == RT_STRATEGY_WEIGHTED,
+                                                     s->dev.cam.lens_radius, s->dev.cam.type, fr.shard_count, fr.mega_tile, fr.dims_max_n,
+                                                     s->counting, s->has_ext, s->volume.present != 0, fr.high_occupancy != 0});
+    if (const char *e = knob("PBRT_HIP_FIXED_FRAME")) fixed_frame = fixed_frame && std::atoi(e) != 0;
+    const int k = debug ? flavour::Debug::index(request_of(s, rd, &fr)) : fixed_frame ? flavour::Fixed::index(request_of(s, rd, &fr)) : flavour::Mega::index(request_of(s, rd, &fr));
+    const unsigned grid = debug ? s->grids.debug[k] : fixed_frame ? s->grids.fixed[k] : s->grids.mega[rd->integrator][k];
+    const RenderKernelFn kernel = debug ? g_render_kernels_debug[k] : fixed_frame ? g_render_kernels_fixed[k] : (*g_render_kernels[rd->integrator])[k];
+    s->last_fixed = fixed_frame;
     if (grid == 0) return fail(RT_ESTATE, "render kernel variant has no resident grid");
 #ifdef RT_TAIL_PROBE
     static unsigned long long *probe = nullptr;
@@ -540,7 +545,7 @@
     const int k = flavour::Trace::index(rq);
     HIPWARN(hipEventRecord(s->ev0, s->stream));
     hipLaunchKernelGGL(g_pipe_trace[k], dim3(s->grids.trace[k]), dim3(RT_BLOCK), 0, s->stream, (const DevScene *)s->dev_scene, job);
-    HIPWARN(hipEventRecord(s->ev1, s->stream)); HIPWARN(hipEventRecord(s->ev2, s->stream)); s->have_timing = true; s->last_pipeline = false;
+    HIPWARN(hipEventRecord(s->ev1, s->stream)); HIPWARN(hipEventRecord(s->ev2, s->stream)); s->have_timing = true; s->last_pipeline = false; s->last_fixed = false;
     HIPCHK(hipGetLastError());
     HIPCHK(hipMemcpyAsync(host.data(), s->trace_buf + 2 * size_t(n), size_t(n) * sizeof(float4), hipMemcpyDeviceToHost, s->stream));
     HIPCHK(hipStreamSynchronize(s->stream));
@@ -633,6 +638,7 @@
     if (debug) { rc = upload_tex_uv(s); if (rc) return rc; }
     { hipError_t pre = hipGetLastError(); if (pre != hipSuccess) return fail(RT_EDEVICE, std::string("pending HIP error before launch: ") + hipGetErrorString(pre)); }
     s->rendered = true;
+    s->last_fixed = false;
     rc = fr.pipeline ? render_pipeline(s, rd, fr) : bidir ? render_bidir(s, rd, fr) : weighted ? render_weighted(s, rd, fr) : render_mega(s, rd, fr);
     if (rc) return rc;
     s->last_pipeline = fr.pipeline != 0; s->last_weighted = weighted;
@@ -723,6 +729,7 @@
         out->slots = s->pipe_slots;
     } else out->trace_ms = out->render_ms;
     out->bands = s->last_pipeline ? 0 : 1;
+    out->fixed_frame = s->last_fixed ? 1 : 0;
     if (s->last_weighted) {
         out->weighted_points = s->wt_points;
         hipEvent_t seq[6] = {s->ev0, s->wt_ev[0], s->wt_ev[1], s->wt_ev[2], s->wt_ev[3], s->ev1};
diff --git a/pbrt-v1_amd/csrc/hip/rt_mega_f.hip b/pbrt-v1_amd/csrc/hip/rt_mega_f.hip
--- /dev/null
+++ b/pbrt-v1_amd/csrc/hip/rt_mega_f.hip
@@ -0,0 +1,5 @@
+#include "rt_render_kernel.h"
+#include "rt_fixed_frame.h"
+namespace rt {
+RT_FLAVOUR_TABLE(g_render_kernels_fixed, RenderKernelFn, Fixed, Fixed::flavour(K), render_kernel_fixed<f.count, flavour::Fixed::integrator(K), f.accel, f.vol, f.waves, f.ext, fixed::Frame>)
+}
diff --git a/pbrt-v1_amd/csrc/hip/rt_render_body.inc b/pbrt-v1_amd/csrc/hip/rt_render_body.inc
--- /dev/null
+++ b/pbrt-v1_amd/csrc/hip/rt_render_body.inc
@@ -0,0 +1,150 @@
+    __shared__ uint2 lds_stack[RT_STACK_LDS * RT_BLOCK];
+    constexpr bool POOL = MINW < RT_HIGH_OCC_WAVES;
+    constexpr int PN = POOL ? RT_BLOCK : 64;
+    __shared__ unsigned long long pool_key[PN];
+    __shared__ float4 pool_res[PN];
+    __shared__ unsigned pool_head[PN];
+    __shared__ float4 pool_ray[3 * PN];
+    __shared__ float lds_tm_own[POOL ? 1 : RT_STACK_LDS * RT_BLOCK];
+    float RT_L *lds_tm = (float RT_L *)lds_tm_own;
+    const DevScene &sc = *scp;
+    const DevFrame &fr = *frp;
+    const unsigned wave0 = POOL ? (threadIdx.x & ~63u) : 0u;
+    const PoolLds pool = {(unsigned long long RT_L *)pool_key + wave0, (float4 RT_L *)pool_res + wave0, (unsigned RT_L *)pool_head + wave0,
+                          (float4 RT_L *)pool_ray + 3 * wave0};
+    const unsigned gtid = blockIdx.x * RT_BLOCK + threadIdx.x;
+    const int lane = threadIdx.x & 63;
+    constexpr bool BYV = RT_MEGA_BYV != 0 && !POOL && INTEG == RT_INTEGRATOR_PATH && !VOL && !EXT && !COUNT;
+    Lane ln;
+    ln.vf = 0u;
+    ln.stage = ST_FETCH; ln.has_ray = false; ln.fsp = 0; ln.tv.active = false; ln.tv.hit_prim = -1;
+    ln.L = mk3(0.f); ln.thr = mk3(1.f); ln.alpha = 0.f; ln.depth = 0; ln.specular = false;
+    TravCounters tc; tc.nodes = tc.leaf_refs = tc.tris = tc.spills = 0;
+    RT_PFT(tc.c_desc = tc.c_leaf = tc.n_chunks = tc.n_pooled = tc.n_iter = 0;)
+    unsigned c_cam = 0, c_closest = 0, c_any = 0, c_bad = 0;
+
+#ifdef RT_PROFILE
+    unsigned long long pf_shade = 0, pf_trav = 0, pf_outer = 0, pf_inner = 0, pf_rounds = 0, pf_act = 0, pf_rays = 0, pf_t0 = 0;
+#define RT_PF(x) x
+#else
+#define RT_PF(x)
+#endif
+#ifdef RT_TAIL_PROBE
+    const unsigned long long tp_start = __builtin_amdgcn_s_memrealtime();
+    unsigned long long tp_empty = 0, tp_taken = 0;
+#endif
+    unsigned long long w_next = 0, w_end = 0;
+    const unsigned n_bands = fr.xcd_bands ? 8u : 1u, home = fr.xcd_bands ? (blockIdx.x & 7u) : 0u;
+    unsigned band_shift = 0;
+
+    int phase = (INTEG == RT_INTEGRATOR_PATH && fr.phase_sync && !BYV) ? 1 : -1;
+    for (;;) {
+        RT_PF(pf_t0 = __builtin_readcyclecounter(); ++pf_outer;)
+        do {
+            RT_PF(++pf_inner;)
+            if constexpr (BYV) advance_pass_byv<COUNT, ACCEL, EXT, FX>(sc, fr, ln, gtid, &c_closest, &c_any, &c_bad);
+            else advance_pass<COUNT, INTEG, VOL, EXT, false, false, FX>(sc, fr, ln, gtid, &c_closest, &c_any, &c_bad, phase);
+            const unsigned long long want = phase == 0 ? 0ull : __ballot(!ln.has_ray && ln.stage == ST_FETCH);
+            if (want) {
+                const unsigned n_want = unsigned(__popcll(want));
+                const unsigned long long have = w_end - w_next;
+                unsigned long long fresh = 0, fresh_end = 0;
+                if (have < n_want) {
+                    const int leader = __ffsll((long long)want) - 1;
+#pragma unroll 1
+                    while (band_shift < n_bands) {
+                        const unsigned r = (home + band_shift) % n_bands;
+                        const unsigned long long lo = band_lo(fr.total_work, r, n_bands), hi = band_lo(fr.total_work, r + 1u, n_bands);
+                        unsigned long long base = 0;
+                        if (lane == leader) base = atomicAdd(fr.work_counter + 8u * r, (unsigned long long)RT_MEGA_CHUNK);
+                        base = uniform64(__shfl(base, leader));
+                        if (lo + base < hi) { fresh = lo + base; fresh_end = fresh + RT_MEGA_CHUNK < hi ? fresh + RT_MEGA_CHUNK : hi; break; }
+                        ++band_shift;
+                    }
+                }
+                const bool none_left = band_shift >= n_bands;
+#ifdef RT_TAIL_PROBE
+                if (none_left && !tp_empty) tp_empty = __builtin_amdgcn_s_memrealtime();
+#endif
+                const unsigned long long rk = __popcll(want & ((1ull << lane) - 1ull));
+                const unsigned long long w_mine = rk < have ? w_next + rk : fresh + (rk - have);
+                const bool got = rk < have || w_mine < fresh_end;
+                if (have < n_want) {
+                    const unsigned long long took = n_want - have < fresh_end - fresh ? n_want - have : fresh_end - fresh;
+                    w_next = fresh + took; w_end = fresh_end;
+                } else w_next += n_want;
+                if (!ln.has_ray && ln.stage == ST_FETCH && !got) { if (none_left) ln.stage = ST_EXIT; }
+                else if (!ln.has_ray && ln.stage == ST_FETCH) {
+                    const unsigned long long w = w_mine;
+#ifdef RT_TAIL_PROBE
+                    tp_taken += 1;
+#endif
+                    {
+                        unsigned long long pixel; int s;
+                        bool ok;
+                        if (FX::tile_order || fr.mega_tile > 0) { unsigned px; tile_order_to_sample(fr, unsigned(w), px, s); pixel = px; ok = true; }
+                        else ok = work_to_sample(fr, w, pixel, s);
+                        if (ok) {
+                            Ray ray;
+                            setup_sample<FX>(sc, fr, ln, pixel, s, ray);
+                            ln.work = (FX::tile_order || fr.mega_tile > 0) ? uint32_t(pixel * unsigned(fr.spp) + unsigned(s)) : uint32_t(w);
+                            if (INTEG == RT_INTEG_DIRECT_WEIGHTED) ln.ord = fr.weighted_phase == 1 ? 0u : RT_GPTR(const unsigned, fr.wt_base)[ln.work];
+                            ln.L = mk3(0.f); ln.thr = mk3(1.f); ln.alpha = 0.f; ln.depth = 0; ln.fsp = 0;
+                            ln.specular = false;
+                            if (COUNT) ++c_cam;
+                            accel_begin<ACCEL>(ln.tv, sc, ray, false);
+                            if (VOL) vol_store_ray(fr, 0, gtid, ray);
+                            ln.has_ray = true; ln.stage = ST_VERTEX;
+                            if (BYV) ln.vf = BV_B | BV_CUR_B;
+                        }
+                    }
+                }
+            }
+        } while (__any(!ln.has_ray && stage_in_phase(ln.stage, phase)));
+        if (phase >= 0) phase ^= 1;
+        RT_PF({ unsigned long long t1 = __builtin_readcyclecounter(); pf_shade += t1 - pf_t0; pf_t0 = t1; pf_rays += __popcll(__ballot(ln.has_ray && ln.tv.active)); })
+        if (!__any(ln.has_ray)) {
+            if (!__any(ln.stage != ST_EXIT)) break;
+            continue;
+        }
+        for (;;) {
+            if constexpr (BYV) {
+                const bool next = ln.has_ray && !ln.tv.active && (ln.vf & (BV_QM | BV_QB)) != 0u;
+                if (__any(next)) { if (next) byv_ray_advance<COUNT, ACCEL, EXT>(sc, ln, &c_closest, &c_any); }
+            }
+            const bool act = ln.has_ray && ln.tv.active;
+            const unsigned long long am = __ballot(act);
+            if (!am) break;
+            RT_PF(++pf_rounds; pf_act += __popcll(am);)
+            if (fr.exit_thresh > 0 && __popcll(am) <= fr.exit_thresh && __any(!act && ln.stage != ST_EXIT)) break;
+            if (POOL && fr.trav_mode == 3) accel_round_pooled<COUNT, ACCEL, EXT>(ln.tv, ln.has_ray, sc, (uint2 RT_L *)lds_stack, RT_GPTR(uint2, fr.spill), fr.n_threads, gtid, tc, pool);
+            else trace_round<COUNT, ACCEL, EXT, RT_STACK_LDS, !POOL>(ln.tv, ln.has_ray, sc, (uint2 RT_L *)lds_stack, lds_tm, RT_GPTR(uint2, fr.spill), fr.n_threads, gtid, tc, fr.leaf_min);
+        }
+        if (ln.has_ray && !ln.tv.active && !(BYV && (ln.vf & (BV_QM | BV_QB)) != 0u)) ln.has_ray = false;
+        RT_PF(pf_trav += __builtin_readcyclecounter() - pf_t0;)
+    }
+#ifdef RT_PROFILE
+    if (lane == 0) {
+        unsigned long long v[12] = {pf_shade, pf_trav, pf_outer, pf_inner, pf_rounds, pf_act, pf_rays, tc.c_desc, tc.c_leaf, tc.n_chunks, tc.n_pooled, tc.n_iter};
+        for (int k = 0; k < 12; ++k) atomicAdd(fr.counters + 8 + k, v[k]);
+    }
+#endif
+
+#ifdef RT_TAIL_PROBE
+    {
+        for (int off = 32; off > 0; off >>= 1) tp_taken += __shfl_down(tp_taken, off);
+        if (lane == 0 && fr.probe) {
+            unsigned long long *o = fr.probe + size_t(gtid >> 6) * 4u;
+            o[0] = tp_start; o[1] = tp_empty; o[2] = __builtin_amdgcn_s_memrealtime(); o[3] = tp_taken;
+        }
+    }
+#endif
+    if (COUNT && !(INTEG == RT_INTEG_DIRECT_WEIGHTED && fr.weighted_phase != 3)) {
+        unsigned long long v[8] = {c_cam, c_closest, c_any, tc.nodes, tc.leaf_refs, tc.tris, c_bad, tc.spills};
+#pragma unroll
+        for (int k = 0; k < 8; ++k) {
+            unsigned long long x = v[k];
+            for (int off = 32; off > 0; off >>= 1) x += __shfl_down(x, off);
+            if (lane == 0 && x) atomicAdd(fr.counters + k, x);
+        }
+    }
diff --git a/pbrt-v1_amd/csrc/hip/rt_render_kernel.h b/pbrt-v1_amd/csrc/hip/rt_render_kernel.h
--- a/pbrt-v1_amd/csrc/hip/rt_render_kernel.h
+++ b/pbrt-v1_amd/csrc/hip/rt_render_kernel.h
@@ -32,156 +32,12 @@
 template <bool COUNT, int INTEG, int ACCEL, bool VOL, int MINW, bool EXT>
 __global__ __launch_bounds__(RT_BLOCK, (EXT && COUNT && INTEG == RT_INTEGRATOR_PATH && ACCEL == RT_ACCEL_GRID && !VOL && MINW < 3) ? 3 : MINW) void render_kernel(const DevScene *__restrict__ scp,
                                                                        const DevFrame *__restrict__ frp) {
-    __shared__ uint2 lds_stack[RT_STACK_LDS * RT_BLOCK];
-    constexpr bool POOL = MINW < RT_HIGH_OCC_WAVES;
-    constexpr int PN = POOL ? RT_BLOCK : 64;
-    __shared__ unsigned long long pool_key[PN];
-    __shared__ float4 pool_res[PN];
-    __shared__ unsigned pool_head[PN];
-    __shared__ float4 pool_ray[3 * PN];
-    __shared__ float lds_tm_own[POOL ? 1 : RT_STACK_LDS * RT_BLOCK];
-    float RT_L *lds_tm = (float RT_L *)lds_tm_own;
-    const DevScene &sc = *scp;
-    const DevFrame &fr = *frp;
-    const unsigned wave0 = POOL ? (threadIdx.x & ~63u) : 0u;
-    const PoolLds pool = {(unsigned long long RT_L *)pool_key + wave0, (float4 RT_L *)pool_res + wave0, (unsigned RT_L *)pool_head + wave0,
-                          (float4 RT_L *)pool_ray + 3 * wave0};
-    const unsigned gtid = blockIdx.x * RT_BLOCK + threadIdx.x;
-    const int lane = threadIdx.x & 63;
-    constexpr bool BYV = RT_MEGA_BYV != 0 && !POOL && INTEG == RT_INTEGRATOR_PATH && !VOL && !EXT && !COUNT;
-    Lane ln;
-    ln.vf = 0u;
-    ln.stage = ST_FETCH; ln.has_ray = false; ln.fsp = 0; ln.tv.active = false; ln.tv.hit_prim = -1;
-    ln.L = mk3(0.f); ln.thr = mk3(1.f); ln.alpha = 0.f; ln.depth = 0; ln.specular = false;
-    TravCounters tc; tc.nodes = tc.leaf_refs = tc.tris = tc.spills = 0;
-    RT_PFT(tc.c_desc = tc.c_leaf = tc.n_chunks = tc.n_pooled = tc.n_iter = 0;)
-    unsigned c_cam = 0, c_closest = 0, c_any = 0, c_bad = 0;
-
-#ifdef RT_PROFILE
-    unsigned long long pf_shade = 0, pf_trav = 0, pf_outer = 0, pf_inner = 0, pf_rounds = 0, pf_act = 0, pf_rays = 0, pf_t0 = 0;
-#define RT_PF(x) x
-#else
-#define RT_PF(x)
-#endif
-#ifdef RT_TAIL_PROBE
-    const unsigned long long tp_start = __builtin_amdgcn_s_memrealtime();
-    unsigned long long tp_empty = 0, tp_taken = 0;
-#endif
-    unsigned long long w_next = 0, w_end = 0;
-    const unsigned n_bands = fr.xcd_bands ? 8u : 1u, home = fr.xcd_bands ? (blockIdx.x & 7u) : 0u;
-    unsigned band_shift = 0;
-
-    int phase = (INTEG == RT_INTEGRATOR_PATH && fr.phase_sync && !BYV) ? 1 : -1;
-    for (;;) {
-        RT_PF(pf_t0 = __builtin_readcyclecounter(); ++pf_outer;)
-        do {
-            RT_PF(++pf_inner;)
-            if constexpr (BYV) advance_pass_byv<COUNT, ACCEL, EXT>(sc, fr, ln, gtid, &c_closest, &c_any, &c_bad);
-            else advance_pass<COUNT, INTEG, VOL, EXT>(sc, fr, ln, gtid, &c_closest, &c_any, &c_bad, phase);
-            const unsigned long long want = phase == 0 ? 0ull : __ballot(!ln.has_ray && ln.stage == ST_FETCH);
-            if (want) {
-                const unsigned n_want = unsigned(__popcll(want));
-                const unsigned long long have = w_end - w_next;
-                unsigned long long fresh = 0, fresh_end = 0;
-                if (have < n_want) {
-                    const int leader = __ffsll((long long)want) - 1;
-#pragma unroll 1
-                    while (band_shift < n_bands) {
-                        const unsigned r = (home + band_shift) % n_bands;
-                        const unsigned long long lo = band_lo(fr.total_work, r, n_bands), hi = band_lo(fr.total_work, r + 1u, n_bands);
-                        unsigned long long base = 0;
-                        if (lane == leader) base = atomicAdd(fr.work_counter + 8u * r, (unsigned long long)RT_MEGA_CHUNK);
-                        base = uniform64(__shfl(base, leader));
-                        if (lo + base < hi) { fresh = lo + base; fresh_end = fresh + RT_MEGA_CHUNK < hi ? fresh + RT_MEGA_CHUNK : hi; break; }
-                        ++band_shift;
-                    }
-                }
-                const bool none_left = band_shift >= n_bands;
-#ifdef RT_TAIL_PROBE
-                if (none_left && !tp_empty) tp_empty = __builtin_amdgcn_s_memrealtime();
-#endif
-                const unsigned long long rk = __popcll(want & ((1ull << lane) - 1ull));
-                const unsigned long long w_mine = rk < have ? w_next + rk : fresh + (rk - have);
-                const bool got = rk < have || w_mine < fresh_end;
-                if (have < n_want) {
-                    const unsigned long long took = n_want - have < fresh_end - fresh ? n_want - have : fresh_end - fresh;
-                    w_next = fresh + took; w_end = fresh_end;
-                } else w_next += n_want;
-                if (!ln.has_ray && ln.stage == ST_FETCH && !got) { if (none_left) ln.stage = ST_EXIT; }
-                else if (!ln.has_ray && ln.stage == ST_FETCH) {
-                    const unsigned long long w = w_mine;
-#ifdef RT_TAIL_PROBE
-                    tp_taken += 1;
-#endif
-                    {
-                        unsigned long long pixel; int s;
-                        bool ok;
-                        if (fr.mega_tile > 0) { unsigned px; tile_order_to_sample(fr, unsigned(w), px, s); pixel = px; ok = true; }
-                        else ok = work_to_sample(fr, w, pixel, s);
-                        if (ok) {
-                            Ray ray;
-                            setup_sample(sc, fr, ln, pixel, s, ray);
-                            ln.work = fr.mega_tile > 0 ? uint32_t(pixel * unsigned(fr.spp) + unsigned(s)) : uint32_t(w);
-                            if (INTEG == RT_INTEG_DIRECT_WEIGHTED) ln.ord = fr.weighted_phase == 1 ? 0u : RT_GPTR(const unsigned, fr.wt_base)[ln.work];
-                            ln.L = mk3(0.f); ln.thr = mk3(1.f); ln.alpha = 0.f; ln.depth = 0; ln.fsp = 0;
-                            ln.specular = false;
-                            if (COUNT) ++c_cam;
-                            accel_begin<ACCEL>(ln.tv, sc, ray, false);
-                            if (VOL) vol_store_ray(fr, 0, gtid, ray);
-                            ln.has_ray = true; ln.stage = ST_VERTEX;
-                            if (BYV) ln.vf = BV_B | BV_CUR_B;
-                        }
-                    }
-                }
-            }
-        } while (__any(!ln.has_ray && stage_in_phase(ln.stage, phase)));
-        if (phase >= 0) phase ^= 1;
-        RT_PF({ unsigned long long t1 = __builtin_readcyclecounter(); pf_shade += t1 - pf_t0; pf_t0 = t1; pf_rays += __popcll(__ballot(ln.has_ray && ln.tv.active)); })
-        if (!__any(ln.has_ray)) {
-            if (!__any(ln.stage != ST_EXIT)) break;
-            continue;
-        }
-        for (;;) {
-            if constexpr (BYV) {
-                const bool next = ln.has_ray && !ln.tv.active && (ln.vf & (BV_QM | BV_QB)) != 0u;
-                if (__any(next)) { if (next) byv_ray_advance<COUNT, ACCEL, EXT>(sc, ln, &c_closest, &c_any); }
-            }
-            const bool act = ln.has_ray && ln.tv.active;
-            const unsigned long long am = __ballot(act);
-            if (!am) break;
-            RT_PF(++pf_rounds; pf_act += __popcll(am);)
-            if (fr.exit_thresh > 0 && __popcll(am) <= fr.exit_thresh && __any(!act && ln.stage != ST_EXIT)) break;
-            if (POOL && fr.trav_mode == 3) accel_round_pooled<COUNT, ACCEL, EXT>(ln.tv, ln.has_ray, sc, (uint2 RT_L *)lds_stack, RT_GPTR(uint2, fr.spill), fr.n_threads, gtid, tc, pool);
-            else trace_round<COUNT, ACCEL, EXT, RT_STACK_LDS, !POOL>(ln.tv, ln.has_ray, sc, (uint2 RT_L *)lds_stack, lds_tm, RT_GPTR(uint2, fr.spill), fr.n_threads, gtid, tc, fr.leaf_min);
-        }
-        if (ln.has_ray && !ln.tv.active && !(BYV && (ln.vf & (BV_QM | BV_QB)) != 0u)) ln.has_ray = false;
-        RT_PF(pf_trav += __builtin_readcyclecounter() - pf_t0;)
-    }
-#ifdef RT_PROFILE
-    if (lane == 0) {
-        unsigned long long v[12] = {pf_shade, pf_trav, pf_outer, pf_inner, pf_rounds, pf_act, pf_rays, tc.c_desc, tc.c_leaf, tc.n_chunks, tc.n_pooled, tc.n_iter};
-        for (int k = 0; k < 12; ++k) atomicAdd(fr.counters + 8 + k, v[k]);
-    }
-#endif
-
-#ifdef RT_TAIL_PROBE
-    {
-        for (int off = 32; off > 0; off >>= 1) tp_taken += __shfl_down(tp_taken, off);
-        if (lane == 0 && fr.probe) {
-            unsigned long long *o = fr.probe + size_t(gtid >> 6) * 4u;
-            o[0] = tp_start; o[1] = tp_empty; o[2] = __builtin_amdgcn_s_memrealtime(); o[3] = tp_taken;
-        }
-    }
-#endif
-    if (COUNT && !(INTEG == RT_INTEG_DIRECT_WEIGHTED && fr.weighted_phase != 3)) {
-        unsigned long long v[8] = {c_cam, c_closest, c_any, tc.nodes, tc.leaf_refs, tc.tris, c_bad, tc.spills};
-#pragma unroll
-        for (int k = 0; k < 8; ++k) {
-            unsigned long long x = v[k];
-            for (int off = 32; off > 0; off >>= 1) x += __shfl_down(x, off);
-            if (lane == 0 && x) atomicAdd(fr.counters + k, x);
-        }
-    }
+    using FX = fixed::Any;
+#include "rt_render_body.inc"
+}
+template <bool COUNT, int INTEG, int ACCEL, bool VOL, int MINW, bool EXT, class FX>
+__global__ __launch_bounds__(RT_BLOCK, MINW) void render_kernel_fixed(const DevScene *__restrict__ scp, const DevFrame *__restrict__ frp) {
+#include "rt_render_body.inc"
 }
 
 typedef void (*RenderKernelFn)(const DevScene *, const DevFrame *);
diff --git a/pbrt-v1_amd/csrc/hip/rt_scene.hip b/pbrt-v1_amd/csrc/hip/rt_scene.hip
--- a/pbrt-v1_amd/csrc/hip/rt_scene.hip
+++ b/pbrt-v1_amd/csrc/hip/rt_scene.hip
@@ -499,6 +499,12 @@
     };
     ResidentGrids &g = s->grids;
     for (int i = 0; i <= RT_INTEGRATOR_PATH; ++i) if ((rc = resident(*g_render_kernels[i], g.mega[i]))) return rc;
+    {
+        const unsigned others = mx;
+        if ((rc = resident(g_render_kernels_fixed, g.fixed))) return rc;
+        for (int k = 0; k < flavour::Fixed::N; ++k) g.fixed[k] = std::min(g.fixed[k], g.mega[flavour::Fixed::integrator(k)][flavour::Fixed::generic(k)]);
+        mx = others;
+    }
     if ((rc = resident(g_render_kernels_weighted, g.weighted)) || (rc = resident(g_render_kernels_bidir, g.bidir))) return rc;
     s->grid = mx;
     {
```

Result: faster. 3565, median of 6 (+2.2%).
